# vb000/LookOnceToHear

Hardware: AMD Instinct MI355X
Metric: frames_per_sec (5 s 16 kHz binaural clips, 625 STFT frames each, offline forward) (higher is better)
Workload: dtype f32 via f16x3 split (3x fp16 MFMA per product, fp32 accumulate; ~22-bit operands, un-normalised rows scaled by a power of two before the split: any finite fp32 range); 1 GPU; BASELINE configs[2]: 32 x 5 s 16 kHz binaural clips per GPU, offline forward (configs/tsh.json separator, random-init weights); batch_per_gpu=32, global_batch=32, parallelism=utterance-dp1, gemm_mode=f16x3, tune=, batches_in_flight=1

## Files before the change

### include/lookonce_hip.h

```cpp
#ifndef LOOKONCE_HIP_H
#define LOOKONCE_HIP_H

#ifdef __cplusplus
extern "C" {
#endif

typedef void* lh_stream_t;

enum {
    LH_OK = 0,
    LH_ERR_ARG = 1,
    LH_ERR_UNSUPPORTED = 2,
    LH_ERR_LAUNCH = 3,
    LH_ERR_RANGE = 4
};

int lh_range_status(unsigned* range_flag, lh_stream_t stream);
int lh_range_flag_copy(unsigned* range_flag, void* host_pinned, lh_stream_t stream);
int lh_range_flag_clear(unsigned* range_flag, lh_stream_t stream);
int lh_selftest_fp16_subnormal(lh_stream_t stream);

enum { LH_GEMM_F32 = 0, LH_GEMM_F16X3 = 1 };

int lh_abi_version(void);

int lh_set_tuning(int key, int value);

int lh_check_config(int nfft, int hop, int n_mics, int emb_dim, int n_blocks_unused, int lstm_hidden,
                    int n_heads, int attn_window, int n_srcs, int spk_emb_dim);

int lh_stft_conv_in(const float* x, const float* conv_buf_in, float* conv_buf_out, const void* wfb_pk,
                    const void* wconv_pk, const float* bconv, float* z, int B, int T, int n_samples,
                    lh_stream_t stream);

int lh_embed_proj_ln(const float* emb, const float* w, const float* bias, const float* ln_w, const float* ln_b,
                     float* scratch, float* gain, int B, lh_stream_t stream);

int lh_ln_lstm_intra(const float* x, const float* ln_w, const float* ln_b, const void* w_pk, const float* b_sum,
                     float* h_out, int n_frames , int mode, lh_stream_t stream);

int lh_ln_lstm_inter(const float* x, const float* ln_w, const float* ln_b, const void* w_pk, const float* b_sum,
                     const float* h0, const float* c0, float* hN, float* cN, float* h_out, int B, int T, int mode,
                     lh_stream_t stream);

int lh_intra_stream(const float* x, const void* wih_pk, const float* b_sum, const float* whh, float* h_out,
                    int n_frames, lh_stream_t stream);

int lh_inter_matvec(const float* x, const void* wih_pk, const float* b_sum, const float* whh, const void* wlin_pk,
                    const float* blin, const float* h0, const float* c0, float* hN, float* cN, float* out, int B, int T,
                    lh_stream_t stream);

int lh_intra_block(const float* x, const void* w_pk, const float* b_sum, const void* wlin_pk, const float* blin,
                   float* out, int n_frames, lh_stream_t stream);

int lh_inter_block(const float* x, const void* w_pk, const float* b_sum, const void* wlin_pk, const float* blin,
                   const float* h0, const float* c0, float* hN, float* cN, float* out, int B, int T,
                   lh_stream_t stream);

int lh_linear_res(const float* h, const void* w_pk, const float* bias, const float* res, float* out, int rows,
                  int K, lh_stream_t stream);

#define LH_KV_PAD_ROWS 48

int lh_qkv_proj_ln(const float* y, const void* w_pk, const float* bias, const float* slopes, const float* lnq_w,
                   const float* lnq_b, const float* lnk_w, const float* lnk_b, const float* lnv_w,
                   const float* lnv_b, void* q, void* kx, void* vx, const int* ring_pos, int B, int T,
                   lh_stream_t stream);

int lh_local_attn(const void* q, const void* kx, const void* vx, float* merged, int B, int T, lh_stream_t stream);

int lh_ring_pack(const float* k_buf, const float* v_buf, void* kx, void* vx, int B, int T, lh_stream_t stream);
int lh_ring_unpack(const void* kx, const void* vx, float* k_buf, float* v_buf, int B, int T, lh_stream_t stream);
int lh_ring_advance(int* ring_pos, int modulo, lh_stream_t stream);

int lh_proj_ln_res(const float* merged, const void* w_pk, const float* bias, const float* slope,
                   const float* ln_w, const float* ln_b, const float* y2, const float* gain, float* out, int B,
                   int T, lh_stream_t stream);

int lh_deconv_istft(const float* y, const float* deconv_buf_in, float* deconv_buf_out, const float* istft_buf_in,
                    float* istft_buf_out, const void* wdec_pk, const float* bdec, const void* wfb_dec,
                    float* wave_out, unsigned* range_flag, int keep_nonfinite, int B, int T, lh_stream_t stream);

int lh_intra_block_win(const float* x, const void* w_pk, const float* b_sum, const void* wlin_pk, const float* blin,
                       float* out, int B, int T, int t0, int Tc, lh_stream_t stream);
int lh_inter_block_win(const float* x, const void* w_pk, const float* b_sum, const void* wlin_pk, const float* blin,
                       const float* h0, const float* c0, float* hN, float* cN, float* out, int B, int T, int t0, int Tc,
                       int carry, lh_stream_t stream);
int lh_ln_lstm_intra_win(const float* x, const float* ln_w, const float* ln_b, const void* w_pk, const float* b_sum, float* h_out,
                         int B, int T, int t0, int Tc, lh_stream_t stream);
int lh_linear_res_win(const float* h, const void* w_pk, const float* bias, const float* res, float* out, int B, int T, int t0,
                      int Tc, int K, lh_stream_t stream);
int lh_inter_matvec_win(const float* x, const void* wih_pk, const float* b_sum, const float* whh, const void* wlin_pk,
                        const float* blin, const float* h0, const float* c0, float* hN, float* cN, float* out, int B, int T,
                        int t0, int Tc, int carry, lh_stream_t stream);
int lh_qkv_proj_ln_win(const float* y, const void* w_pk, const float* bias, const float* slopes, const float* lnq_w,
                       const float* lnq_b, const float* lnk_w, const float* lnk_b, const float* lnv_w,
                       const float* lnv_b, void* q, void* kx, void* vx, const int* ring_pos, int B, int T, int t0, int Tc,
                       lh_stream_t stream);
int lh_local_attn_win(const void* q, const void* kx, const void* vx, float* merged, int B, int T, int t0, int Tc,
                      lh_stream_t stream);
int lh_proj_ln_res_win(const float* merged, const void* w_pk, const float* bias, const float* slope, const float* ln_w,
                       const float* ln_b, const float* y2, const float* gain, float* out, int B, int T, int t0, int Tc,
                       lh_stream_t stream);

int lh_ref32_stft_conv_in(const float* x, const float* conv_buf_in, float* conv_buf_out, const float* filters,
                          const float* conv_w, const float* conv_b, float* spec_scratch, float* out, int B, int T,
                          int n_samples, lh_stream_t stream);
int lh_ref32_linear(const float* in, const float* w, const float* bias, const float* slope, const float* res, float* out,
                    int rows, int K, int N, lh_stream_t stream);
int lh_ref32_head_ln(const float* pre, int ncol, int col0, int D, const float* ln_w, const float* ln_b, float* dst,
                     int row0, int rows_per_bh, int B, int T, lh_stream_t stream);
int lh_ref32_local_attn(const float* q, const float* kx, const float* vx, float* merged, int B, int T, lh_stream_t stream);
int lh_ref32_proj_ln_res(const float* merged, const float* w, const float* bias, const float* slope, const float* ln_w,
                         const float* ln_b, const float* y2, const float* gain, float* rows_scratch, float* pre_scratch,
                         float* out, int B, int T, lh_stream_t stream);
int lh_ref32_deconv_istft(const float* y, const float* deconv_buf_in, float* deconv_buf_out, const float* istft_buf_in,
                          float* istft_buf_out, const float* deconv_w, const float* deconv_b, const float* filters,
                          float* sx_scratch, float* wave_out, int B, int T, lh_stream_t stream);

int lh_emb_frontend(const float* x, float* inv_std, const float* wfb_pk, const float* wconv_pk, const float* bconv,
                    const float* gn_w, const float* gn_b, double* gn_part, float* z, void* xsplit_next, int B, int T,
                    int n_samples, lh_stream_t stream);

#ifdef LH_LEGACY
int lh_emb_axis(const float* x, const void* wih_pk, const float* bih, const void* whh_pk, const void* wct_pk,
                const float* bct, void* xsplit, float* gx, float* hbuf, float* out, int B, int T, int inter,
                lh_stream_t stream);
#endif

int lh_emb_axis_fused(const float* x, const void* wrec_pk, const float* brec, const void* wct_pk, const float* bct,
                      void* xsplit, void* hsplit, float* out, int B, int T, int inter, int have_xsplit, int emit_split,
                      lh_stream_t stream);

int lh_emb_axis_mv(const float* x, const void* wih_pk, const float* bih, const float* whh, const void* wct_pk,
                   const float* bct, void* xsplit, void* hsplit, float* out, int B, int T, int have_xsplit, int emit_split,
                   lh_stream_t stream);

int lh_emb_attn_block(const float* y2, const void* wqkv_pk, const float* bqkv, const float* slopes,
                      const float* lnq_w, const float* lnq_b, const float* lnk_w, const float* lnk_b,
                      const float* lnv_w, const float* lnv_b, const void* wproj_pk, const float* bproj,
                      const float* slope_p, const float* lnp_w, const float* lnp_b, void* q, void* k, float* v,
                      void* vt, float* sc, void* p, float* merged, float* out, void* xsplit_next, int B, int T,
                      lh_stream_t stream);

int lh_emb_head(const float* z, const void* w_pk, const float* bias, const float* ln_w, const float* ln_b,
                float* part, float* emb, int B, int T, lh_stream_t stream);

int lh_render_binaural(const float* src, const float* rir, const float* gain, const int* tgt_idx, float* events,
                       unsigned* peak, float* mixture, float* target, int B, int S1, int N, int Lh, lh_stream_t stream);

int lh_metric_sums(const float* outputs, const float* target, const float* mixture, const float* emb,
                   const float* emb_gt, double* scratch, float* rows, double* sums, int B, int n_samples,
                   int emb_dim, lh_stream_t stream);

int lh_binaural_cues(const float* est, const float* gt, double* scratch, double* rows, double* sums, int B, int n_samples,
                     int sr, int frame, double rms_threshold, lh_stream_t stream);

typedef struct { void* base; unsigned long long bytes; } lh_span_t;
enum { LH_SESSION_RESET = 1, LH_SESSION_OPEN = 2, LH_SESSION_CLOSE = 4, LH_SESSION_GEN_SHIFT = 8, LH_SESSION_MAX_SPANS = 32,
       LH_SESSION_MAX_END_SPANS = 8 };
int lh_session_begin(const lh_span_t* spans, int n_spans, const float* chunk_in, float* chunk, const unsigned* cmd,
                     const unsigned* active, int S, lh_stream_t stream);
int lh_session_end(const lh_span_t* spans, int n_spans, const float* chunk_in, float* out, unsigned* cmd, unsigned* active,
                   unsigned* fault, int S, lh_stream_t stream);

int lh_session_move(const lh_span_t* spans, int n_spans, const int* from, unsigned* cmd, unsigned* active, int n_rows, int S,
                    lh_stream_t stream);
int lh_session_begin_rows(const lh_span_t* spans, int n_spans, const float* chunk_in, float* chunk, const unsigned* cmd,
                          const unsigned* active, const int* slot_of, int n_rows, int S, lh_stream_t stream);
int lh_session_end_rows(const lh_span_t* spans, int n_spans, const float* chunk_in, const float* out_rows, float* out,
                        unsigned* cmd, unsigned* active, unsigned* fault, const int* slot_of, const int* row_of, int* from,
                        int n_rows, int S, lh_stream_t stream);

enum { LH_ENROLL_ARM = 1, LH_ENROLL_CANCEL = 2, LH_ENROLL_GEN_SHIFT = 8, LH_ENROLL_FAULT = 0x80000000u };
int lh_session_capture(const float* chunk_in, float* enroll, unsigned* ecmd, unsigned* estate, unsigned* edone, int n_chunks,
                       int S, lh_stream_t stream);

int lh_comm_unique_id(void* id128);
int lh_comm_init(const void* id128, int n_ranks, int rank, void** comm);
int lh_allreduce_f64(void* comm, double* buf, int count, lh_stream_t stream);
int lh_comm_destroy(void* comm);

#ifdef __cplusplus
}
#endif
#endif
```

### lookoncetohear_amd/_cabi.py

```python
from __future__ import annotations

import ctypes
import os
from ctypes import c_double, c_int, c_void_p

_PKG = os.path.dirname(os.path.abspath(__file__))
HIP_LIB_PATH = os.path.join(_PKG, "_lookonce_hip.so")
ABI_VERSION = 18

_P, _I = c_void_p, c_int
SIGNATURES = {
    "lh_abi_version": [],
    "lh_check_config": [_I] * 10,
    "lh_stft_conv_in": [_P] * 7 + [_I] * 3 + [_P],
    "lh_embed_proj_ln": [_P] * 7 + [_I, _P],
    "lh_set_tuning": [_I, _I],
    "lh_ln_lstm_intra": [_P] * 6 + [_I, _I, _P],
    "lh_ln_lstm_inter": [_P] * 10 + [_I, _I, _I, _P],
    "lh_intra_stream": [_P] * 5 + [_I, _P],
    "lh_inter_matvec": [_P] * 11 + [_I, _I, _P],
    "lh_intra_block": [_P] * 6 + [_I, _P],
    "lh_inter_block": [_P] * 10 + [_I, _I, _P],
    "lh_linear_res": [_P] * 5 + [_I, _I, _P],
    "lh_qkv_proj_ln": [_P] * 14 + [_I, _I, _P],
    "lh_local_attn": [_P] * 4 + [_I, _I, _P],
    "lh_ring_pack": [_P] * 4 + [_I, _I, _P],
    "lh_ring_unpack": [_P] * 4 + [_I, _I, _P],
    "lh_ring_advance": [_P, _I, _P],
    "lh_session_begin": [_P, _I, _P, _P, _P, _P, _I, _P],
    "lh_session_end": [_P, _I, _P, _P, _P, _P, _P, _I, _P],
    "lh_session_capture": [_P] * 5 + [_I, _I, _P],
    "lh_session_move": [_P, _I, _P, _P, _P, _I, _I, _P],
    "lh_session_begin_rows": [_P, _I, _P, _P, _P, _P, _P, _I, _I, _P],
    "lh_session_end_rows": [_P, _I] + [_P] * 9 + [_I, _I, _P],
    "lh_proj_ln_res": [_P] * 9 + [_I, _I, _P],
    "lh_deconv_istft": [_P] * 10 + [_I, _I, _I, _P],
    "lh_intra_block_win": [_P] * 6 + [_I, _I, _I, _I, _P],
    "lh_inter_block_win": [_P] * 10 + [_I, _I, _I, _I, _I, _P],
    "lh_ln_lstm_intra_win": [_P] * 6 + [_I, _I, _I, _I, _P],
    "lh_linear_res_win": [_P] * 5 + [_I, _I, _I, _I, _I, _P],
    "lh_inter_matvec_win": [_P] * 11 + [_I, _I, _I, _I, _I, _P],
    "lh_qkv_proj_ln_win": [_P] * 14 + [_I, _I, _I, _I, _P],
    "lh_local_attn_win": [_P] * 4 + [_I, _I, _I, _I, _P],
    "lh_proj_ln_res_win": [_P] * 9 + [_I, _I, _I, _I, _P],
    "lh_emb_frontend": [_P] * 10 + [_I, _I, _I, _P],
    "lh_emb_axis_fused": [_P] * 8 + [_I, _I, _I, _I, _I, _P],
    "lh_emb_axis_mv": [_P] * 9 + [_I, _I, _I, _I, _P],
    "lh_emb_attn_block": [_P] * 24 + [_I, _I, _P],
    "lh_emb_head": [_P] * 7 + [_I, _I, _P],
    "lh_render_binaural": [_P] * 8 + [_I, _I, _I, _I, _P],
    "lh_metric_sums": [_P] * 8 + [_I, _I, _I, _P],
    "lh_binaural_cues": [_P] * 5 + [_I, _I, _I, _I, c_double, _P],
    "lh_range_status": [_P, _P],
    "lh_range_flag_copy": [_P, _P, _P],
    "lh_range_flag_clear": [_P, _P],
    "lh_selftest_fp16_subnormal": [_P],
    "lh_comm_unique_id": [_P],
    "lh_comm_init": [_P, _I, _I, _P],
    "lh_allreduce_f64": [_P, _P, _I, _P],
    "lh_comm_destroy": [_P],
    "lh_ref32_stft_conv_in": [_P] * 8 + [_I, _I, _I, _P],
    "lh_ref32_linear": [_P] * 6 + [_I, _I, _I, _P],
    "lh_ref32_head_ln": [_P, _I, _I, _I, _P, _P, _P, _I, _I, _I, _I, _P],
    "lh_ref32_local_attn": [_P] * 4 + [_I, _I, _P],
    "lh_ref32_proj_ln_res": [_P] * 11 + [_I, _I, _P],
    "lh_ref32_deconv_istft": [_P] * 10 + [_I, _I, _P],
}
LEGACY_SIGNATURES = {
    "lh_emb_axis": [_P] * 10 + [_I, _I, _I, _P],
}
ERRORS = {1: "LH_ERR_ARG", 2: "LH_ERR_UNSUPPORTED", 3: "LH_ERR_LAUNCH", 4: "LH_ERR_RANGE"}


class Lib:

    def __init__(self, path: str):
        if not os.path.exists(path):
            raise RuntimeError(
                f"{path} not found: the HIP extension is not built. Run `python -m lookoncetohear_amd.build` "
                "(hipcc --offload-arch=gfx950). There is no CPU fallback for the product path.")
        self.path = path
        import torch
        self._dll = ctypes.CDLL(path)
        for name, argtypes in SIGNATURES.items():
            fn = getattr(self._dll, name)
            fn.argtypes = argtypes
            fn.restype = c_int
        for name, argtypes in LEGACY_SIGNATURES.items():
            fn = getattr(self._dll, name, None)
            if fn is not None:
                fn.argtypes = argtypes
                fn.restype = c_int
        v = self._dll.lh_abi_version()
        if v != ABI_VERSION:
            raise RuntimeError(f"{path}: ABI version {v}, expected {ABI_VERSION}")

    def call(self, name: str, *args) -> None:
        rc = getattr(self._dll, name)(*args)
        if rc != 0:
            raise RuntimeError(f"{name} failed: {ERRORS.get(rc, rc)}")

    def raw(self, name: str):
        return getattr(self._dll, name)


def device_of(t):
    import torch
    return torch.cuda.device(t.device)


_hip_lib = None
_selftested = set()


class HipHost:
    _host_name = "this module"

    def _lib(self, t) -> "Lib":
        if not t.is_cuda:
            raise RuntimeError(f"lookoncetohear_amd.{self._host_name} runs on an MI355X (ROCm device tensors); there is no "
                               "CPU path. Move the module and its inputs to cuda.")
        lib = load()
        import torch
        selftest_device(lib, t.device.index if t.device.index is not None else torch.cuda.current_device())
        return lib

    def _stream(self, device) -> int:
        import torch
        return torch.cuda.current_stream(device).cuda_stream

    def _device_ctx(self, t):
        return device_of(t)

    def _flag_words(self, device):
        return self._host_words(2, device)

    def _host_words(self, n, device):
        import torch
        return torch.zeros(n, dtype=torch.int32).pin_memory()


def selftest_device(lib: "Lib", device_index: int) -> None:
    if device_index in _selftested:
        return
    import torch
    with torch.cuda.device(device_index):
        rc = lib.raw("lh_selftest_fp16_subnormal")(torch.cuda.current_stream(device_index).cuda_stream)
    if rc != 0:
        raise RuntimeError(f"lh_selftest_fp16_subnormal failed on cuda:{device_index} ({ERRORS.get(rc, rc)}): fp16 subnormal "
                           "MFMA operands are flushed; the split-precision kernels would lose precision silently")
    _selftested.add(device_index)


def load() -> Lib:
    global _hip_lib
    if _hip_lib is None:
        _hip_lib = Lib(os.environ.get("LOOKONCE_HIP_LIB", HIP_LIB_PATH))
        for kv in filter(None, os.environ.get("LOOKONCE_TUNE", "").split(",")):
            k, v = kv.split("=")
            _hip_lib.call("lh_set_tuning", int(k), int(v))
    return _hip_lib
```

### lookoncetohear_amd/csrc/lh_frontend.hip

```cpp
#include "lh_split.h"

namespace lh {

constexpr int FE_NTH = 512;
constexpr int FE_TT = 14;
constexpr int FE_NJ = 16;
constexpr int FE_AP = NFFT + 8;
constexpr int FE_SP = 68;
constexpr int FE_NT = (NK + 15) / 16;
constexpr int FE_KS = NFFT / 32;
constexpr int FE_OP = C + 4;

__global__ void __launch_bounds__(FE_NTH, 1) k_stft_conv_in(const float* __restrict__ x, const float* __restrict__ cbuf_in,
                                                            float* __restrict__ cbuf_out, const _Float16* __restrict__ wfb_pk,
                                                            const _Float16* __restrict__ wc_pk, const float* __restrict__ bc,
                                                            float* __restrict__ z, int B, int T, int n_samples) {
    __shared__ __attribute__((aligned(16))) _Float16 ahi[NMIC * FE_NJ * FE_AP];
    __shared__ __attribute__((aligned(16))) _Float16 alo[NMIC * FE_NJ * FE_AP];
    __shared__ __attribute__((aligned(16))) _Float16 sth[(NF + 2) * FE_SP];
    __shared__ __attribute__((aligned(16))) _Float16 stl[(NF + 2) * FE_SP];
    __shared__ __attribute__((aligned(16))) float outs[2][NF * FE_OP];
    __shared__ float tmax[FE_NTH / 64];
    const int tid = threadIdx.x, lane = tid & 63, wave = wave_id(tid), g4 = lane >> 4, l15 = lane & 15;

    f16x8 wfh[2][FE_KS], wfl[2][FE_KS];
#pragma unroll
    for (int i = 0; i < 2; ++i) load_w<FE_KS>(wfb_pk, min(wave + 8 * i, FE_NT - 1), lane, wfh[i], wfl[i]);
    f16x8 wch[2], wcl[2];
    const int cnt = wave & 3;
    load_w<2>(wc_pk, cnt, lane, wch, wcl);
    const float cbias = bc[cnt * 16 + l15];

    static_assert(((NF + 2) * FE_SP) % 4 == 0, "8-byte zero fill");
    for (int i = tid; i < (NF + 2) * FE_SP / 4; i += FE_NTH) {
        *reinterpret_cast<f16x4*>(&sth[i * 4]) = f16x4{0, 0, 0, 0};
        *reinterpret_cast<f16x4*>(&stl[i * 4]) = f16x4{0, 0, 0, 0};
    }

    const int tiles_per_b = (T + FE_TT - 1) / FE_TT;
    for (int tile = blockIdx.x; tile < B * tiles_per_b; tile += gridDim.x) {
        const int b = tile / tiles_per_b;
        const int t0 = (tile % tiles_per_b) * FE_TT;
        const int nt_out = min(FE_TT, T - t0);
        __syncthreads();
        float tsc, tinv;

        {
            constexpr int NLD = NMIC * FE_NJ * 48 / FE_NTH;
            float4 stg[NLD];
#pragma unroll
            for (int i = 0; i < NLD; ++i) {
                const int e = tid + FE_NTH * i;
                const int m = e / (FE_NJ * 48), j = (e / 48) % FE_NJ, c4 = e % 48;
                const int t = t0 - 2 + j;
                stg[i] = make_float4(0.f, 0.f, 0.f, 0.f);
                if (t >= 0 && t < T)
                    stg[i] = *reinterpret_cast<const float4*>(&x[((long)b * NMIC + m) * n_samples + (long)t * HOP + c4 * 4]);
            }
            float tm = 0.f;
#pragma unroll
            for (int i = 0; i < NLD; ++i) tm = fmaxf(tm, absmax4(stg[i]));
            if (t0 == 0)
                for (int i = tid; i < 4 * 2 * NF; i += FE_NTH) tm = fmaxf(tm, fabsf(cbuf_in[(long)b * 4 * 2 * NF + i]) * (1.0f / 32.0f));
            tm = wave_max(tm);
            if (lane == 0) tmax[wave] = tm;
            __syncthreads();
#pragma unroll
            for (int w = 0; w < FE_NTH / 64; ++w) tm = fmaxf(tm, tmax[w]);
            pow2_scale<9>(tm, tsc, tinv);
#pragma unroll
            for (int i = 0; i < NLD; ++i) {
                const int e = tid + FE_NTH * i;
                const int m = e / (FE_NJ * 48), j = (e / 48) % FE_NJ, c4 = e % 48;
                const float v[4] = {stg[i].x * tsc, stg[i].y * tsc, stg[i].z * tsc, stg[i].w * tsc};
                f16x2_t h01, l01, h23, l23;
                split_pair(v[0], v[1], h01, l01);
                split_pair(v[2], v[3], h23, l23);
                const f16x4 h4 = f16x4{h01[0], h01[1], h23[0], h23[1]}, l4 = f16x4{l01[0], l01[1], l23[0], l23[1]};
                const int idx = (m * FE_NJ + j) * FE_AP + c4 * 4;
                *reinterpret_cast<f16x4*>(&ahi[idx]) = h4;
                *reinterpret_cast<f16x4*>(&alo[idx]) = l4;
            }
        }
        __syncthreads();

#pragma unroll 1
        for (int m = 0; m < NMIC; ++m) {
            f32x4 am[2], ac[2];
#pragma unroll
            for (int i = 0; i < 2; ++i) { am[i] = f32x4{0.f, 0.f, 0.f, 0.f}; ac[i] = f32x4{0.f, 0.f, 0.f, 0.f}; }
            const bool second = wave + 8 < FE_NT;
#pragma unroll
            for (int ks = 0; ks < FE_KS; ++ks) {
                const int idx = (m * FE_NJ + l15) * FE_AP + ks * 32 + g4 * 8;
                const f16x8 fah = *reinterpret_cast<const f16x8*>(&ahi[idx]);
                const f16x8 fal = *reinterpret_cast<const f16x8*>(&alo[idx]);
#pragma unroll
                for (int i = 0; i < 2; ++i) {
                    if (i == 0 || second) {
                        am[i] = __builtin_amdgcn_mfma_f32_16x16x32_f16(fah, wfh[i][ks], am[i], 0, 0, 0);
                        ac[i] = __builtin_amdgcn_mfma_f32_16x16x32_f16(fah, wfl[i][ks], ac[i], 0, 0, 0);
                        ac[i] = __builtin_amdgcn_mfma_f32_16x16x32_f16(fal, wfh[i][ks], ac[i], 0, 0, 0);
                    }
                }
            }
#pragma unroll
            for (int i = 0; i < 2; ++i) {
                const int nt = wave + 8 * i;
                const int k = nt * 16 + l15;
                if (nt < FE_NT && k < NK) {
                    const int ch = (k / NF) * NMIC + m, f = k % NF;
#pragma unroll
                    for (int r = 0; r < 4; ++r) {
                        const int j = g4 * 4 + r, t = t0 - 2 + j;
                        float v = am[i][r] + ac[i][r];
                        if (t < 0) v = cbuf_in[(((long)b * 4 + ch) * 2 + (t + 2)) * NF + f] * tsc;
                        if (t >= T) v = 0.0f;
                        _Float16 h, l;
                        split_hl(v, h, l);
                        sth[(f + 1) * FE_SP + j * 4 + ch] = h;
                        stl[(f + 1) * FE_SP + j * 4 + ch] = l;
                        if (t >= T - 2 && t < T) cbuf_out[(((long)b * 4 + ch) * 2 + (t - (T - 2))) * NF + f] = v * tinv;
                    }
                }
            }
        }
        __syncthreads();

        const int mt0 = wave >> 2;
        const int kf0 = g4 >> 1, cofs = (g4 & 1) * 8;
        for (int jt = 0; jt < nt_out; ++jt) {
            float* ob = outs[jt & 1];
#pragma unroll
            for (int i = 0; i < 4; ++i) {
                const int mt = mt0 + 2 * i;
                if (mt < 7) {
                    const int f = min(mt * 16 + l15, NF - 1);
                    const int a0 = (f + kf0) * FE_SP + jt * 4 + cofs, a1 = (f + 2) * FE_SP + jt * 4 + cofs;
                    f16x8 ah[2], al[2];
                    auto rd8 = [&](const _Float16* base, int idx) -> f16x8 {
                        const f16x4 u = *reinterpret_cast<const f16x4*>(&base[idx]);
                        const f16x4 w = *reinterpret_cast<const f16x4*>(&base[idx + 4]);
                        return f16x8{u[0], u[1], u[2], u[3], w[0], w[1], w[2], w[3]};
                    };
                    ah[0] = rd8(sth, a0); al[0] = rd8(stl, a0);
                    ah[1] = rd8(sth, a1); al[1] = rd8(stl, a1);
                    f32x4 am = f32x4{0.f, 0.f, 0.f, 0.f}, ac = f32x4{0.f, 0.f, 0.f, 0.f};
#pragma unroll
                    for (int ks = 0; ks < 2; ++ks) {
                        am = __builtin_amdgcn_mfma_f32_16x16x32_f16(ah[ks], wch[ks], am, 0, 0, 0);
                        ac = __builtin_amdgcn_mfma_f32_16x16x32_f16(ah[ks], wcl[ks], ac, 0, 0, 0);
                        ac = __builtin_amdgcn_mfma_f32_16x16x32_f16(al[ks], wch[ks], ac, 0, 0, 0);
                    }
#pragma unroll
                    for (int r = 0; r < 4; ++r) {
                        const int fo = mt * 16 + g4 * 4 + r;
                        if (fo < NF) ob[fo * FE_OP + cnt * 16 + l15] = fmaf(am[r] + ac[r], tinv, cbias);
                    }
                }
            }
            __syncthreads();
            float* dst = z + (((long)b * T + t0 + jt) * NF) * C;
            for (int e = tid; e < NF * 16; e += FE_NTH)
                *reinterpret_cast<float4*>(&dst[e * 4]) = *reinterpret_cast<const float4*>(&ob[(e >> 4) * FE_OP + (e & 15) * 4]);
        }
    }
}

constexpr int EP_ROWS = 32, EP_NB = 8;
__global__ void __launch_bounds__(256) k_embed_proj(const float* __restrict__ emb, const float* __restrict__ w,
                                                     const float* __restrict__ bias, float* __restrict__ raw, int B) {
    constexpr int N = C * NF;
    __shared__ __attribute__((aligned(16))) float es[EP_NB][SPK];
    const int tid = threadIdx.x, lane = tid & 63, wave = wave_id(tid);
    const int b0 = blockIdx.y * EP_NB;
    for (int i = tid; i < EP_NB * SPK; i += 256) {
        const int bb = min(b0 + i / SPK, B - 1);
        es[i / SPK][i % SPK] = emb[(long)bb * SPK + (i % SPK)];
    }
    __syncthreads();
    constexpr int RW = EP_ROWS / 4;
    float4 w4[RW];
    float bz[RW];
#pragma unroll
    for (int q = 0; q < RW; ++q) {
        const int r = min((int)blockIdx.x * EP_ROWS + wave + q * 4, N - 1);
        w4[q] = *reinterpret_cast<const float4*>(&w[(long)r * SPK + lane * 4]);
        bz[q] = bias[r];
    }
#pragma unroll
    for (int q = 0; q < RW; ++q) {
        const int r = blockIdx.x * EP_ROWS + wave + q * 4;
        if (r >= N) break;
#pragma unroll
        for (int j = 0; j < EP_NB; ++j) {
            const float4 e4 = *reinterpret_cast<const float4*>(&es[j][lane * 4]);
            float s = wave_sum(w4[q].x * e4.x + w4[q].y * e4.y + w4[q].z * e4.z + w4[q].w * e4.w);
            if (lane == 0 && b0 + j < B) raw[(long)(b0 + j) * N + r] = s + bz[q];
        }
    }
}

__global__ void __launch_bounds__(256) k_embed_ln(const float* __restrict__ raw, const float* __restrict__ lnw,
                                                   const float* __restrict__ lnb, float* __restrict__ gain) {
    constexpr int N = C * NF;
    __shared__ float vals[N];
    __shared__ float red[4];
    const int tid = threadIdx.x;
    const int b = blockIdx.x;
    float s = 0.0f;
    for (int i = tid; i < N; i += 256) { const float v = raw[(long)b * N + i]; vals[i] = v; s += v; }
    const float mean = block_sum_256(s, red) * (1.0f / N);
    float v = 0.0f;
    for (int i = tid; i < N; i += 256) { float d = vals[i] - mean; v += d * d; }
    const float rstd = rsqrtf(block_sum_256(v, red) * (1.0f / N) + LN_EPS);
    for (int oidx = tid; oidx < N; oidx += 256) {
        const int f = oidx / C, c = oidx % C;
        const int i = c * NF + f;
        gain[(long)b * N + oidx] = (vals[i] - mean) * rstd * lnw[i] + lnb[i];
    }
}

}

extern "C" int lh_stft_conv_in(const float* x, const float* conv_buf_in, float* conv_buf_out, const void* wfb_pk,
                               const void* wconv_pk, const float* bconv, float* z, int B, int T, int n_samples,
                               lh_stream_t stream) {
    using namespace lh;
    if (!x || !conv_buf_in || !conv_buf_out || !wfb_pk || !wconv_pk || !bconv || !z || B <= 0 || T <= 0) return LH_ERR_ARG;
    if (conv_buf_in == conv_buf_out || n_samples != T * HOP + (NFFT - HOP)) return LH_ERR_ARG;
    const int tiles = B * ((T + FE_TT - 1) / FE_TT);
    hipLaunchKernelGGL(k_stft_conv_in, dim3(tiles < 256 ? tiles : 256), dim3(FE_NTH), 0, (hipStream_t)stream, x,
                       conv_buf_in, conv_buf_out, (const _Float16*)wfb_pk, (const _Float16*)wconv_pk, bconv, z, B, T,
                       n_samples);
    return check_launch();
}

extern "C" int lh_embed_proj_ln(const float* emb, const float* w, const float* bias, const float* ln_w,
                                const float* ln_b, float* scratch, float* gain, int B, lh_stream_t stream) {
    using namespace lh;
    if (!emb || !w || !bias || !ln_w || !ln_b || !scratch || !gain || B <= 0 || scratch == gain) return LH_ERR_ARG;
    hipLaunchKernelGGL(k_embed_proj, dim3((C * NF + EP_ROWS - 1) / EP_ROWS, (B + EP_NB - 1) / EP_NB), dim3(256), 0,
                       (hipStream_t)stream, emb, w, bias, scratch, B);
    hipLaunchKernelGGL(k_embed_ln, dim3(B), dim3(256), 0, (hipStream_t)stream, scratch, ln_w, ln_b, gain);
    return check_launch();
}

extern "C" int lh_abi_version(void) { return 18; }

extern "C" int lh_check_config(int nfft, int hop, int n_mics, int emb_dim, int n_blocks_unused, int lstm_hidden,
                               int n_heads, int attn_window, int n_srcs, int spk_emb_dim) {
    using namespace lh;
    (void)n_blocks_unused;
    if (nfft != NFFT || hop != HOP || n_mics != NMIC || emb_dim != C || lstm_hidden != H || n_heads != NH ||
        attn_window != WIN || n_srcs != NSRC || spk_emb_dim != SPK)
        return LH_ERR_UNSUPPORTED;
    return LH_OK;
}
```

### lookoncetohear_amd/csrc/lh_lstm.hip

```cpp
#include <type_traits>

#include "lh_common.h"

namespace lh {

constexpr int LS_PAD = 36;

template <int MT>
__global__ void __launch_bounds__(256) k_ln_lstm(const float* __restrict__ x, const float* __restrict__ lnw,
                                                 const float* __restrict__ lnb, const float* __restrict__ w_pk,
                                                 const float* __restrict__ b_sum, const float* __restrict__ h0,
                                                 const float* __restrict__ c0, float* __restrict__ hN,
                                                 float* __restrict__ cN, float* __restrict__ h_out, int nseq,
                                                 int nstep, int sdiv, int so, int si, int ps, int ldh) {
    constexpr int NS = 16 * MT;
    __shared__ __attribute__((aligned(16))) float abuf[2 * 4 * NS * LS_PAD];
    const int tid = threadIdx.x, lane = tid & 63, wave = wave_id(tid);
    const int dir = blockIdx.y;
    const int s0 = blockIdx.x * NS;
    const int g4 = lane >> 4, l15 = lane & 15;

    auto A = [&](int buf, int chunk, int row, int j) -> float* {
        return &abuf[((buf * 4 + chunk) * NS + row) * LS_PAD + j];
    };
// ... 598 lines not shown
    if (nstep >= 2) store_rows(nstep - 2, (nstep - 1) & 1, rr);
    load_base(nstep - 1, rr);
    lin_tile(nstep & 1, nstep & 1);
    __syncthreads();
    store_rows(nstep - 1, nstep & 1, rr);
}

#endif

__global__ void __launch_bounds__(512, 1) k_lstm_lin8p(const float* __restrict__ x, const _Float16* __restrict__ w_pk,
                                                       const float* __restrict__ b_sum, const _Float16* __restrict__ wlin_pk,
                                                       const float* __restrict__ blin, const float* __restrict__ h0,
                                                       const float* __restrict__ c0, float* __restrict__ hN,
                                                       float* __restrict__ cN, float* out, int nseq, int nstep, int sdiv,
                                                       int so, int si, int ps, int dir, int accumulate) {
    constexpr int NS = 16;
    constexpr int LSP = C + 4;
    __shared__ __attribute__((aligned(16))) _Float16 ahi[2 * NS * LH_AP];
    __shared__ __attribute__((aligned(16))) _Float16 alo[2 * NS * LH_AP];
    __shared__ __attribute__((aligned(16))) float ls[2 * NS * LSP];
    __shared__ __attribute__((aligned(16))) float hf[NS * LSP];
    const int tid = threadIdx.x, lane = tid & 63;
    const int wave = __builtin_amdgcn_readfirstlane(tid >> 6);
    const int s0 = blockIdx.x * NS;
    const int g4 = lane >> 4, l15 = lane & 15;
    const bool lin_wave = wave < 4;
    const int q = tid & 15, rrow = (tid & 255) >> 4;
    const int unit0 = 8 * wave + 2 * g4;

    auto row_of0 = [&](int s) -> long { return (long)(s / sdiv) * so + (long)(s % sdiv) * si; };
    const long wg_row0 = row_of0(min(s0, nseq - 1));
    const unsigned voff = (unsigned)((row_of0(min(s0 + rrow, nseq - 1)) - wg_row0) * (C * 4) + q * 16);
    const char* xb = reinterpret_cast<const char*>(x) + wg_row0 * (C * 4);
    char* ob = reinterpret_cast<char*>(out) + wg_row0 * (C * 4);
    const char* bsrc = reinterpret_cast<const char*>(
        accumulate ? reinterpret_cast<unsigned long long>(ob) : reinterpret_cast<unsigned long long>(xb));
    const long step_bytes = (long)ps * (C * 4);
    auto step_pos = [&](int it) -> int { it = min(max(it, 0), nstep - 1); return dir ? (nstep - 1 - it) : it; };

    f16x8 wh[2][4], wl[2][4];
    {
        const _Float16* wp = w_pk + ((long)(dir * 8 + wave) * 8 * 64 + lane) * 16;
#pragma unroll
        for (int m = 0; m < 2; ++m)
#pragma unroll
            for (int ks = 0; ks < 4; ++ks) {
                wh[m][ks] = *reinterpret_cast<const f16x8*>(wp + (long)(m * 4 + ks) * 64 * 16);
                wl[m][ks] = *reinterpret_cast<const f16x8*>(wp + (long)(m * 4 + ks) * 64 * 16 + 8);
            }
    }
    f16x8 lwh[2], lwl[2];
    float lbias = 0.0f;
    if (lin_wave) {
#pragma unroll
        for (int ks = 0; ks < 2; ++ks) {
            lwh[ks] = *reinterpret_cast<const f16x8*>(&wlin_pk[((wave * 2 + ks) * 64 + lane) * 16]);
            lwl[ks] = *reinterpret_cast<const f16x8*>(&wlin_pk[((wave * 2 + ks) * 64 + lane) * 16 + 8]);
        }
        if (!accumulate) lbias = blin[wave * 16 + l15];
    } else {
#pragma unroll
        for (int ks = 0; ks < 2; ++ks) lwh[ks] = lwl[ks] = f16x8{0, 0, 0, 0, 0, 0, 0, 0};
    }
    float bias[2][4];
#pragma unroll
    for (int m = 0; m < 2; ++m)
#pragma unroll
        for (int g = 0; g < 4; ++g) bias[m][g] = b_sum[dir * 256 + g * 64 + unit0 + m];

    const int a_frag = l15 * LH_AP + g4 * 8;
    const int a_cell = l15 * LH_AP + C + unit0;
    const int a_row = rrow * LH_AP + q * 4;
    const int l_row = rrow * LSP + q * 4;
    const int l_lin = (g4 * 4) * LSP + wave * 16 + l15;

    auto store_split4 = [&](int idx, float a, float b, float c, float d) {
        f16x4 h4, l4;
        _Float16 th, tl;
        split_f16(a, th, tl); h4[0] = th; l4[0] = tl;
        split_f16(b, th, tl); h4[1] = th; l4[1] = tl;
        split_f16(c, th, tl); h4[2] = th; l4[2] = tl;
        split_f16(d, th, tl); h4[3] = th; l4[3] = tl;
        *reinterpret_cast<f16x4*>(&ahi[idx]) = h4;
        *reinterpret_cast<f16x4*>(&alo[idx]) = l4;
    };
    auto norm_store_x = [&](int buf, float4 v) {
        const float mean = group16_sum(v.x + v.y + v.z + v.w) * (1.0f / C);
        v.x -= mean; v.y -= mean; v.z -= mean; v.w -= mean;
        const float var = group16_sum(v.x * v.x + v.y * v.y + v.z * v.z + v.w * v.w) * (1.0f / C);
        const float rstd = __builtin_amdgcn_rsqf(var + LN_EPS);
        store_split4(buf * NS * LH_AP + a_row, v.x * rstd, v.y * rstd, v.z * rstd, v.w * rstd);
    };
    auto load_row = [&](const char* base, int it) -> float4 {
        return *reinterpret_cast<const float4*>(base + step_pos(it) * step_bytes + voff);
    };
    auto x_half = [&](int buf, f32x4 (&g)[2]) {
#pragma unroll
        for (int m = 0; m < 2; ++m) g[m] = f32x4{bias[m][0], bias[m][1], bias[m][2], bias[m][3]};
#pragma unroll
        for (int ks = 0; ks < 2; ++ks) {
            const f16x8 xh = *reinterpret_cast<const f16x8*>(&ahi[buf * NS * LH_AP + a_frag + ks * 32]);
            const f16x8 xl = *reinterpret_cast<const f16x8*>(&alo[buf * NS * LH_AP + a_frag + ks * 32]);
#pragma unroll
            for (int m = 0; m < 2; ++m) g[m] = __builtin_amdgcn_mfma_f32_16x16x32_f16(wh[m][ks], xh, g[m], 0, 0, 0);
#pragma unroll
            for (int m = 0; m < 2; ++m) g[m] = __builtin_amdgcn_mfma_f32_16x16x32_f16(wh[m][ks], xl, g[m], 0, 0, 0);
#pragma unroll
            for (int m = 0; m < 2; ++m) g[m] = __builtin_amdgcn_mfma_f32_16x16x32_f16(wl[m][ks], xh, g[m], 0, 0, 0);
        }
    };

    float creg[2], hreg[2];
    float4 carry = make_float4(0.f, 0.f, 0.f, 0.f);
    if (!lin_wave) {
        norm_store_x(0, load_row(xb, 0));
        norm_store_x(1, load_row(xb, 1));
        carry = load_row(xb, 2);
    } else {
        const int s = min(s0 + rrow, nseq - 1);
        float4 hv = make_float4(0.f, 0.f, 0.f, 0.f);
        if (h0) hv = *reinterpret_cast<const float4*>(&h0[(long)s * H + q * 4]);
        store_split4(a_row + C, hv.x, hv.y, hv.z, hv.w);
    }
    {
        const int s = min(s0 + l15, nseq - 1);
#pragma unroll
        for (int m = 0; m < 2; ++m) {
            creg[m] = c0 ? c0[(long)s * H + unit0 + m] : 0.0f;
            hreg[m] = 0.0f;
        }
    }
    __syncthreads();
    f32x4 gx[2];
    x_half(0, gx);
    __syncthreads();

    auto step = [&](int it, auto cur_tag, auto lin_tag) __attribute__((always_inline)) {
        constexpr int cur = decltype(cur_tag)::value, nxt = cur ^ 1;
        constexpr bool LIN = decltype(lin_tag)::value;
        f16x8 bh[2], bl[2];
#pragma unroll
        for (int ks = 0; ks < 2; ++ks) {
            bh[ks] = *reinterpret_cast<const f16x8*>(&ahi[cur * NS * LH_AP + a_frag + (2 + ks) * 32]);
            bl[ks] = *reinterpret_cast<const f16x8*>(&alo[cur * NS * LH_AP + a_frag + (2 + ks) * 32]);
        }
        f32x4 acc[2] = {gx[0], gx[1]};
#pragma unroll
        for (int ks = 0; ks < 2; ++ks) {
#pragma unroll
            for (int m = 0; m < 2; ++m) acc[m] = __builtin_amdgcn_mfma_f32_16x16x32_f16(wh[m][2 + ks], bh[ks], acc[m], 0, 0, 0);
#pragma unroll
            for (int m = 0; m < 2; ++m) acc[m] = __builtin_amdgcn_mfma_f32_16x16x32_f16(wh[m][2 + ks], bl[ks], acc[m], 0, 0, 0);
#pragma unroll
            for (int m = 0; m < 2; ++m) acc[m] = __builtin_amdgcn_mfma_f32_16x16x32_f16(wl[m][2 + ks], bh[ks], acc[m], 0, 0, 0);
        }
        pin_here(carry);
        if (LIN) {
            const float4 pv = *reinterpret_cast<const float4*>(&ls[nxt * NS * LSP + l_row]);
            const float4 done = make_float4(carry.x + pv.x, carry.y + pv.y, carry.z + pv.z, carry.w + pv.w);
            if (it >= 2) *reinterpret_cast<float4*>(ob + step_pos(it - 2) * step_bytes + voff) = done;
            carry = load_row(bsrc, it - 1);
        } else {
            norm_store_x(cur, carry);
            carry = load_row(xb, it + 3);
        }
        __builtin_amdgcn_sched_barrier(0);
        auto cells = [&]() {
#pragma unroll
            for (int m = 0; m < 2; ++m) {
                lstm_cell_pre(acc[m][0], acc[m][1], acc[m][2], acc[m][3], creg[m], hreg[m]);
                _Float16 th, tl;
                split_f16(hreg[m], th, tl);
                ahi[nxt * NS * LH_AP + a_cell + m] = th;
                alo[nxt * NS * LH_AP + a_cell + m] = tl;
            }
        };
        if (LIN) {
            x_half(nxt, gx);
            f32x4 am = f32x4{lbias, lbias, lbias, lbias};
#pragma unroll
            for (int ks = 0; ks < 2; ++ks) {
                am = __builtin_amdgcn_mfma_f32_16x16x32_f16(bh[ks], lwh[ks], am, 0, 0, 0);
                am = __builtin_amdgcn_mfma_f32_16x16x32_f16(bh[ks], lwl[ks], am, 0, 0, 0);
                am = __builtin_amdgcn_mfma_f32_16x16x32_f16(bl[ks], lwh[ks], am, 0, 0, 0);
            }
            __builtin_amdgcn_sched_barrier(0);
            cells();
#pragma unroll
            for (int r = 0; r < 4; ++r) ls[cur * NS * LSP + r * LSP + l_lin] = am[r];
        } else {
            __builtin_amdgcn_sched_barrier(0);
            cells();
            __builtin_amdgcn_sched_barrier(0);
            x_half(nxt, gx);
        }
        __builtin_amdgcn_sched_barrier(0);
        __syncthreads();
    };
    auto run = [&](auto lin_tag) __attribute__((always_inline)) {
        int it = 0;
        for (; it + 1 < nstep; it += 2) {
            step(it, std::integral_constant<int, 0>{}, lin_tag);
            step(it + 1, std::integral_constant<int, 1>{}, lin_tag);
        }
        if (it < nstep) step(it, std::integral_constant<int, 0>{}, lin_tag);
    };
    if (lin_wave) run(std::true_type{});
    else run(std::false_type{});

    const int lastb = nstep & 1;
    if (lin_wave) {
        if (nstep >= 2) {
            const float4 pv = *reinterpret_cast<const float4*>(&ls[(lastb ^ 1) * NS * LSP + l_row]);
            *reinterpret_cast<float4*>(ob + step_pos(nstep - 2) * step_bytes + voff) =
                make_float4(carry.x + pv.x, carry.y + pv.y, carry.z + pv.z, carry.w + pv.w);
        }
        carry = load_row(bsrc, nstep - 1);
        f32x4 am = f32x4{lbias, lbias, lbias, lbias};
#pragma unroll
        for (int ks = 0; ks < 2; ++ks) {
            const f16x8 ah = *reinterpret_cast<const f16x8*>(&ahi[lastb * NS * LH_AP + a_frag + (2 + ks) * 32]);
            const f16x8 al = *reinterpret_cast<const f16x8*>(&alo[lastb * NS * LH_AP + a_frag + (2 + ks) * 32]);
            am = __builtin_amdgcn_mfma_f32_16x16x32_f16(ah, lwh[ks], am, 0, 0, 0);
            am = __builtin_amdgcn_mfma_f32_16x16x32_f16(ah, lwl[ks], am, 0, 0, 0);
            am = __builtin_amdgcn_mfma_f32_16x16x32_f16(al, lwh[ks], am, 0, 0, 0);
        }
#pragma unroll
        for (int r = 0; r < 4; ++r) ls[lastb * NS * LSP + r * LSP + l_lin] = am[r];
    }
    if (hN) {
#pragma unroll
        for (int m = 0; m < 2; ++m) hf[l15 * LSP + unit0 + m] = hreg[m];
    }
    __syncthreads();
    if (lin_wave) {
        const float4 pv = *reinterpret_cast<const float4*>(&ls[lastb * NS * LSP + l_row]);
        *reinterpret_cast<float4*>(ob + step_pos(nstep - 1) * step_bytes + voff) =
            make_float4(carry.x + pv.x, carry.y + pv.y, carry.z + pv.z, carry.w + pv.w);
    } else if (hN && s0 + rrow < nseq) {
        *reinterpret_cast<float4*>(&hN[(long)(s0 + rrow) * H + q * 4]) = *reinterpret_cast<const float4*>(&hf[l_row]);
    }
    if (cN && s0 + l15 < nseq) {
#pragma unroll
        for (int m = 0; m < 2; ++m) cN[(long)(s0 + l15) * H + unit0 + m] = creg[m];
    }
}

#if defined(LH_LEGACY)
static int g_dephase = 1;
template <int MT>
static int launch_lstm_lin(const float* x, const void* w_pk, const float* b_sum, const void* wlin_pk, const float* blin,
                           const float* h0, const float* c0, float* hN, float* cN, float* out, int nseq, int nstep,
                           int sdiv, int so, int si, int ps, int dir, int accumulate, hipStream_t st) {
    constexpr int NS = 16 * MT;
    if (h0 || c0 || hN || cN) return LH_ERR_ARG;
    hipLaunchKernelGGL((k_ln_lstm_lin<MT>), dim3((nseq + NS - 1) / NS), dim3(256), 0, st, x, (const _Float16*)w_pk, b_sum,
                       (const _Float16*)wlin_pk, blin, h0, c0, hN, cN, out, nseq, nstep, sdiv, so, si, ps, dir, accumulate,
                       g_dephase);
    return check_launch();
}

#endif
template <int MT>
static int launch_lstm_h3(const float* x, const float* lnw, const float* lnb, const void* w_pk, const float* b_sum,
                          const float* h0, const float* c0, float* hN, float* cN, float* h_out, int nseq, int nstep,
                          int ndir, int sdiv, int so, int si, int ps, int ldh, hipStream_t st) {
    constexpr int NS = 16 * MT;
    hipLaunchKernelGGL((k_ln_lstm_h3<MT>), dim3((nseq + NS - 1) / NS, ndir), dim3(256), 0, st, x, lnw, lnb,
                       (const _Float16*)w_pk, b_sum, h0, c0, hN, cN, h_out, nseq, nstep, sdiv, so, si, ps, ldh);
    return check_launch();
}

template <int MT>
static int launch_lstm(const float* x, const float* lnw, const float* lnb, const float* w_pk, const float* b_sum,
                       const float* h0, const float* c0, float* hN, float* cN, float* h_out, int nseq, int nstep,
                       int ndir, int sdiv, int so, int si, int ps, int ldh, hipStream_t st) {
    constexpr int NS = 16 * MT;
    hipLaunchKernelGGL((k_ln_lstm<MT>), dim3((nseq + NS - 1) / NS, ndir), dim3(256), 0, st, x, lnw, lnb, w_pk, b_sum,
                       h0, c0, hN, cN, h_out, nseq, nstep, sdiv, so, si, ps, ldh);
    return check_launch();
}

}

namespace lh {
static int cu_count() {
    static int n = 0;
    if (n == 0) {
        int dev = 0, v = 0;
        if (hipGetDevice(&dev) == hipSuccess &&
            hipDeviceGetAttribute(&v, hipDeviceAttributeMultiprocessorCount, dev) == hipSuccess && v > 0)
            n = v;
        else
            n = 256;
    }
    return n;
}
int emb_set(int key, int value);
static int g_tune[8] = {0, 0, 0, 0, 0, 0, 0, 0};
}
namespace lh { int attn_set_mq(int v); }
namespace lh {
int launch_intra_xp(const float* x, const void* w_pk, const float* b_sum, const void* wlin_pk, const float* blin, float* out,
                    int nseq, int nstep, int sdiv, int so, int si, int ps, int dir, int accumulate, hipStream_t st);
int xp_set(int key, int v);
int launch_inter_xp(const float* x, const void* w_pk, const float* b_sum, const void* wlin_pk, const float* blin,
                    const float* h0, const float* c0, float* hN, float* cN, float* out, int nseq, int nstep, int sdiv, int so,
                    int si, int ps, hipStream_t st, int cflags = 0);
}
namespace lh { int backend_set_runs(int v); }
#if defined(LH_PROBE_TRACE)
extern "C" int lh_probe_trace_read(unsigned long long* host_dst) {
    return hipMemcpyFromSymbol(host_dst, HIP_SYMBOL(lh::lh_trace_buf), sizeof(lh::lh_trace_buf)) == hipSuccess ? 0 : 1;
}
#endif
extern "C" int lh_set_tuning(int key, int value) {
    if (key == 4) return lh::attn_set_mq(value);
    if (key == 6) return lh::backend_set_runs(value);
    if (key >= 7 && key < 16) return lh::xp_set(key, value);
    if (key == 16 || key == 17) return lh::emb_set(key, value);
    if (key < 0 || key >= 8) return LH_ERR_ARG;
#if defined(LH_LEGACY)
    if (key == 3) lh::g_dephase = value;
#else
    if (key == 2 && value == 2) return LH_ERR_UNSUPPORTED;
#endif
    lh::g_tune[key] = value;
    return LH_OK;
}

extern "C" int lh_ln_lstm_intra(const float* x, const float* ln_w, const float* ln_b, const void* w_pk,
                                const float* b_sum, float* h_out, int n_frames, int mode, lh_stream_t stream) {
    using namespace lh;
    if (!x || !ln_w || !ln_b || !w_pk || !b_sum || !h_out || n_frames <= 0) return LH_ERR_ARG;
    const int mt = g_tune[0] ? g_tune[0] : (mode == LH_GEMM_F16X3 ? 0 : (n_frames >= 8192 ? 2 : 1));
    if (mode == LH_GEMM_F16X3) {
        hipStream_t st = (hipStream_t)stream;
        if (mt == 2)
            return launch_lstm_h3<2>(x, ln_w, ln_b, w_pk, b_sum, nullptr, nullptr, nullptr, nullptr, h_out, n_frames, NF,
                                     2, 1, NF, 0, 1, 2 * H, st);
        if (mt == 1)
            return launch_lstm_h3<1>(x, ln_w, ln_b, w_pk, b_sum, nullptr, nullptr, nullptr, nullptr, h_out, n_frames, NF,
                                     2, 1, NF, 0, 1, 2 * H, st);
        const int slots = 2 * cu_count();
        const int tiles2 = (n_frames / 32) * 2 / slots * slots / 2;
        const int f2 = tiles2 * 32;
        int rc = LH_OK;
        if (f2 > 0)
            rc = launch_lstm_h3<2>(x, ln_w, ln_b, w_pk, b_sum, nullptr, nullptr, nullptr, nullptr, h_out, f2, NF, 2, 1, NF,
                                   0, 1, 2 * H, st);
        if (rc == LH_OK && n_frames > f2)
            rc = launch_lstm_h3<1>(x + (long)f2 * NF * C, ln_w, ln_b, w_pk, b_sum, nullptr, nullptr, nullptr, nullptr,
                                   h_out + (long)f2 * NF * 2 * H, n_frames - f2, NF, 2, 1, NF, 0, 1, 2 * H, st);
        return rc;
    }
    if (mode != LH_GEMM_F32) return LH_ERR_UNSUPPORTED;
    const float* w_f32 = (const float*)w_pk;
    if (mt == 2)
        return launch_lstm<2>(x, ln_w, ln_b, w_f32, b_sum, nullptr, nullptr, nullptr, nullptr, h_out, n_frames, NF, 2, 1,
                              NF, 0, 1, 2 * H, (hipStream_t)stream);
    return launch_lstm<1>(x, ln_w, ln_b, w_f32, b_sum, nullptr, nullptr, nullptr, nullptr, h_out, n_frames, NF, 2, 1, NF,
                          0, 1, 2 * H, (hipStream_t)stream);
}

extern "C" int lh_ln_lstm_intra_win(const float* x, const float* ln_w, const float* ln_b, const void* w_pk, const float* b_sum,
                                    float* h_out, int B, int T, int t0, int Tc, lh_stream_t stream) {
    using namespace lh;
    if (!x || !ln_w || !ln_b || !w_pk || !b_sum || !h_out || B <= 0 || T <= 0 || t0 < 0 || Tc <= 0 || t0 + Tc > T) return LH_ERR_ARG;
    const long off = (long)t0 * NF;
    return launch_lstm_h3<1>(x + off * C, ln_w, ln_b, w_pk, b_sum, nullptr, nullptr, nullptr, nullptr, h_out + off * 2 * H, B * Tc,
                             NF, 2, Tc, T * NF, NF, 1, 2 * H, (hipStream_t)stream);
}

extern "C" int lh_ln_lstm_inter(const float* x, const float* ln_w, const float* ln_b, const void* w_pk,
                                const float* b_sum, const float* h0, const float* c0, float* hN, float* cN,
                                float* h_out, int B, int T, int mode, lh_stream_t stream) {
    using namespace lh;
    if (!x || !ln_w || !ln_b || !w_pk || !b_sum || !h0 || !c0 || !hN || !cN || !h_out || B <= 0 || T <= 0)
        return LH_ERR_ARG;
    if (h0 == hN || c0 == cN) return LH_ERR_ARG;
    const int nseq = B * NF;
    const int mt = g_tune[1] == 2 ? 2 : 1;
    if (mode == LH_GEMM_F16X3) {
        if (mt == 2)
            return launch_lstm_h3<2>(x, ln_w, ln_b, w_pk, b_sum, h0, c0, hN, cN, h_out, nseq, T, 1, NF, T * NF, 1, NF, H,
                                     (hipStream_t)stream);
        return launch_lstm_h3<1>(x, ln_w, ln_b, w_pk, b_sum, h0, c0, hN, cN, h_out, nseq, T, 1, NF, T * NF, 1, NF, H,
                                 (hipStream_t)stream);
    }
    if (mode != LH_GEMM_F32) return LH_ERR_UNSUPPORTED;
    const float* w_f32 = (const float*)w_pk;
    if (mt == 2)
        return launch_lstm<2>(x, ln_w, ln_b, w_f32, b_sum, h0, c0, hN, cN, h_out, nseq, T, 1, NF, T * NF, 1, NF, H,
                              (hipStream_t)stream);
    return launch_lstm<1>(x, ln_w, ln_b, w_f32, b_sum, h0, c0, hN, cN, h_out, nseq, T, 1, NF, T * NF, 1, NF, H,
                          (hipStream_t)stream);
}

extern "C" int lh_intra_block(const float* x, const void* w_pk, const float* b_sum, const void* wlin_pk,
                              const float* blin, float* out, int n_frames, lh_stream_t stream) {
    using namespace lh;
    if (!x || !w_pk || !b_sum || !wlin_pk || !blin || !out || n_frames <= 0 || x == out) return LH_ERR_ARG;
    hipStream_t st = (hipStream_t)stream;
    int rc = LH_OK;
    for (int dir = 0; dir < 2 && rc == LH_OK; ++dir)
#if defined(LH_LEGACY)
        if (g_tune[2] == 2)
            rc = launch_lstm_lin<1>(x, w_pk, b_sum, (const _Float16*)wlin_pk + (long)dir * 4 * 2 * 64 * 16, blin, nullptr, nullptr,
                                    nullptr, nullptr, out, n_frames, NF, 1, NF, 0, 1, dir, dir, st);
        else
#endif
            rc = launch_intra_xp(x, w_pk, b_sum, (const _Float16*)wlin_pk + (long)dir * 4 * 2 * 64 * 16, blin, out, n_frames,
                                 NF, 1, NF, 0, 1, dir, dir, st);
    return rc;
}

extern "C" int lh_intra_block_win(const float* x, const void* w_pk, const float* b_sum, const void* wlin_pk,
                                  const float* blin, float* out, int B, int T, int t0, int Tc, lh_stream_t stream) {
    using namespace lh;
    if (!x || !w_pk || !b_sum || !wlin_pk || !blin || !out || B <= 0 || T <= 0 || x == out || t0 < 0 || Tc <= 0 || t0 + Tc > T)
        return LH_ERR_ARG;
    const long off = (long)t0 * NF * C;
    int rc = LH_OK;
    for (int dir = 0; dir < 2 && rc == LH_OK; ++dir)
        rc = launch_intra_xp(x + off, w_pk, b_sum, (const _Float16*)wlin_pk + (long)dir * 4 * 2 * 64 * 16, blin, out + off,
                             B * Tc, NF, Tc, T * NF, NF, 1, dir, dir, (hipStream_t)stream);
    return rc;
}

extern "C" int lh_inter_block_win(const float* x, const void* w_pk, const float* b_sum, const void* wlin_pk,
                                  const float* blin, const float* h0, const float* c0, float* hN, float* cN, float* out,
                                  int B, int T, int t0, int Tc, int carry, lh_stream_t stream) {
    using namespace lh;
    if (!x || !w_pk || !b_sum || !wlin_pk || !blin || !h0 || !c0 || !hN || !cN || !out || B <= 0 || T <= 0) return LH_ERR_ARG;
    if (h0 == hN || c0 == cN || x == out || t0 < 0 || Tc < 2 || t0 + Tc > T || (carry & ~3)) return LH_ERR_ARG;
    const long off = (long)t0 * NF * C;
    return launch_inter_xp(x + off, w_pk, b_sum, wlin_pk, blin, h0, c0, hN, cN, out + off, B * NF, Tc, NF, T * NF, 1, NF,
                           (hipStream_t)stream, carry);
}

extern "C" int lh_inter_block(const float* x, const void* w_pk, const float* b_sum, const void* wlin_pk,
                              const float* blin, const float* h0, const float* c0, float* hN, float* cN, float* out,
                              int B, int T, lh_stream_t stream) {
    using namespace lh;
    if (!x || !w_pk || !b_sum || !wlin_pk || !blin || !h0 || !c0 || !hN || !cN || !out || B <= 0 || T <= 0) return LH_ERR_ARG;
    if (h0 == hN || c0 == cN || x == out) return LH_ERR_ARG;
    const int nseq = B * NF;
    if (g_tune[5] != 2 && T >= 2)
        return launch_inter_xp(x, w_pk, b_sum, wlin_pk, blin, h0, c0, hN, cN, out, nseq, T, NF, T * NF, 1, NF,
                               (hipStream_t)stream);
    hipLaunchKernelGGL(k_lstm_lin8p, dim3((nseq + 15) / 16), dim3(512), 0, (hipStream_t)stream, x, (const _Float16*)w_pk,
                           b_sum, (const _Float16*)wlin_pk, blin, h0, c0, hN, cN, out, nseq, T, NF, T * NF, 1, NF, 0, 0);
    return check_launch();
}
```

### lookoncetohear_amd/csrc/lh_recur.hip

```cpp
#include <tuple>
#include <type_traits>
#include <utility>

#include "lh_common.h"

namespace lh {

typedef _Float16 xp_f16x8 __attribute__((ext_vector_type(8)));
typedef _Float16 xp_f16x4 __attribute__((ext_vector_type(4)));
constexpr int XP_AP = 144;
constexpr int XP_LSP = 68;
constexpr float XP_K2 = -2.0f * LOG2E;

template <int NSLOT, class MF, class Ops>
__device__ __forceinline__ void xp_zip(MF& mf, Ops& ops) {
    constexpr int NOPS = (int)std::tuple_size<Ops>::value;
    xp_for<NSLOT>([&](auto s_) {
        constexpr int i = decltype(s_)::value;
        mf(s_);
        constexpr int a = i * NOPS / NSLOT, b = (i + 1) * NOPS / NSLOT;
        xp_for<b - a>([&](auto k_) { std::get<a + decltype(k_)::value>(ops)(); });
#if !defined(XP_NO_FENCE)
        __builtin_amdgcn_sched_barrier(0);
#endif
    });
}

#if defined(XP_X2)
constexpr int XP_XN = 8;
#else
constexpr int XP_XN = 12;
#endif

#if defined(XP_PF1)
constexpr int XP_PF = 1;
#else
constexpr int XP_PF = 2;
#endif

#if defined(XP_TRACE)
__device__ unsigned long long xp_trace_buf[2 * 128 * 4];
__device__ unsigned long long xp_wg_log[4096 * 4];
__device__ unsigned long long xp_trace_inter[2 * 128 * 4];
#define XP_STAMP(k) do { if (tr_on) tr[(it & 127) * 4 + (k)] = __builtin_amdgcn_s_memtime(); } while (0)
#else
#define XP_STAMP(k) do { } while (0)
#endif

__device__ __forceinline__ float xp_exp2(float v) {
#if defined(XP_PROBE_NOTRANS)
    return __builtin_fmaf(v, 0.25f, 0.5f);
#else
    return __builtin_amdgcn_exp2f(v);
#endif
}
__device__ __forceinline__ float xp_rcp(float v) {
#if defined(XP_PROBE_NOTRANS)
    return __builtin_fmaf(v, -0.25f, 1.0f);
#else
    return __builtin_amdgcn_rcpf(v);
#endif
}
#if defined(XP_PROBE_HIHI)
constexpr int XP_NP = 1;
#else
constexpr int XP_NP = 3;
#endif

__global__ void __launch_bounds__(256, 2) k_intra_xp(const float* __restrict__ x, const _Float16* __restrict__ w_pk,
                                                     const float* __restrict__ b_sum, const _Float16* __restrict__ wlin_pk,
                                                     const float* __restrict__ blin, float* out, int nseq, int nstep,
                                                     int sdiv, int so, int si, int ps, int dir, int accumulate, int prio) {
    constexpr int NS = 16;
    __shared__ __attribute__((aligned(16))) _Float16 ahi[2 * NS * XP_AP];
    __shared__ __attribute__((aligned(16))) _Float16 alo[2 * NS * XP_AP];
    __shared__ __attribute__((aligned(16))) float ls[2 * NS * XP_LSP];
    const int tid = threadIdx.x, lane = tid & 63, wave = wave_id(tid);
#if defined(XP_TRACE)
    __shared__ unsigned long long tr[128 * 4];
    const int tr_slot = blockIdx.x == 7 ? 0 : (blockIdx.x == gridDim.x / 2 + 3 ? 1 : -1);
    const bool tr_on = tr_slot >= 0 && threadIdx.x == 0 && dir == 0;
    const unsigned long long wg_t0 = __builtin_amdgcn_s_memtime();
#endif
    if (prio == 1) {
        const unsigned hw_id = __builtin_amdgcn_s_getreg((4 - 1) << 11 | 0 << 6 | 4);
        if (hw_id & 1) __builtin_amdgcn_s_setprio(2);
    }
#if defined(LH_PROBE_INTRA1)
    const int nt1 = (nseq + NS - 1) / NS;
    dir = (int)blockIdx.x >= nt1;
    accumulate = dir;
    wlin_pk += (long)dir * 4 * 2 * 64 * 16;
    const int s0 = ((int)blockIdx.x - dir * nt1) * NS;
#else
    const int s0 = blockIdx.x * NS;
#endif
    const int g4 = lane >> 4, l15 = lane & 15;
    const int q = tid & 15;
    const int unit = wave * 16 + l15;

    auto row_of0 = [&](int s) -> long { return (long)(s / sdiv) * so + (long)(s % sdiv) * si; };
    const long wg_row0 = row_of0(min(s0, nseq - 1));
    const int srow = min(s0 + (tid >> 4), nseq - 1);
    const unsigned voff = (unsigned)((row_of0(srow) - wg_row0) * (C * 4) + q * 16);
    const char* xb = reinterpret_cast<const char*>(x) + wg_row0 * (C * 4);
    char* ob = reinterpret_cast<char*>(out) + wg_row0 * (C * 4);
    const char* bsrc = reinterpret_cast<const char*>(
        accumulate ? reinterpret_cast<unsigned long long>(ob) : reinterpret_cast<unsigned long long>(xb));
    const long step_bytes = (long)ps * (C * 4);
    auto step_pos = [&](int it) -> int { it = min(max(it, 0), nstep - 1); return dir ? (nstep - 1 - it) : it; };

    xp_f16x8 wh[4][4], wl[4][4];
    {
        const _Float16* wp = w_pk + ((long)(dir * 4 + wave) * 16 * 64 + lane) * 16;
#pragma unroll
        for (int g = 0; g < 4; ++g)
#pragma unroll
            for (int ks = 0; ks < 4; ++ks) {
                wh[g][ks] = *reinterpret_cast<const xp_f16x8*>(wp + (long)(g * 4 + ks) * 64 * 16);
                wl[g][ks] = *reinterpret_cast<const xp_f16x8*>(wp + (long)(g * 4 + ks) * 64 * 16 + 8);
            }
    }
    xp_f16x8 lwh[2], lwl[2];
#pragma unroll
    for (int ks = 0; ks < 2; ++ks) {
        lwh[ks] = *reinterpret_cast<const xp_f16x8*>(&wlin_pk[((wave * 2 + ks) * 64 + lane) * 16]);
        lwl[ks] = *reinterpret_cast<const xp_f16x8*>(&wlin_pk[((wave * 2 + ks) * 64 + lane) * 16 + 8]);
    }
    float eb[4];
#pragma unroll
    for (int g = 0; g < 4; ++g)
        eb[g] = __builtin_amdgcn_exp2f(fminf(fmaxf(b_sum[dir * 256 + g * 64 + unit], -100.0f), 100.0f));
    const float lbias = accumulate ? 0.0f : blin[unit];

    const int a_row = (tid >> 4) * XP_AP + q * 4;
    const int l_row = (tid >> 4) * XP_LSP + q * 4;
    const int a_frag = l15 * XP_AP + g4 * 8;
    const int a_cell = (g4 * 4) * XP_AP + C + unit;
    const int l_cell = (g4 * 4) * XP_LSP + unit;

    auto load_x = [&](int it) -> float4 { return *reinterpret_cast<const float4*>(xb + step_pos(it) * step_bytes + voff); };
    auto load_base = [&](int it) -> float4 { return *reinterpret_cast<const float4*>(bsrc + step_pos(it) * step_bytes + voff); };
    auto store_split4 = [&](int idx, float a, float b, float c, float d) {
        f16x2_t h01, l01, h23, l23;
        split_pair(a, b, h01, l01);
        split_pair(c, d, h23, l23);
        const xp_f16x4 h4 = xp_f16x4{h01[0], h01[1], h23[0], h23[1]}, l4 = xp_f16x4{l01[0], l01[1], l23[0], l23[1]};
        *reinterpret_cast<xp_f16x4*>(&ahi[idx]) = h4;
        *reinterpret_cast<xp_f16x4*>(&alo[idx]) = l4;
    };
    auto norm_store_x = [&](int buf, float4 v) {
        const float mean = group16_sum(v.x + v.y + v.z + v.w) * (1.0f / C);
        v.x -= mean; v.y -= mean; v.z -= mean; v.w -= mean;
        const float var = group16_sum(v.x * v.x + v.y * v.y + v.z * v.z + v.w * v.w) * (1.0f / C);
        const float rstd = __builtin_amdgcn_rsqf(var + LN_EPS);
        store_split4(buf * NS * XP_AP + a_row, v.x * rstd, v.y * rstd, v.z * rstd, v.w * rstd);
    };
    auto x_half = [&](int buf, f32x4 (&g)[4]) __attribute__((always_inline)) {
        xp_f16x8 xh[2], xl[2];
#pragma unroll
        for (int ks = 0; ks < 2; ++ks) {
            xh[ks] = *reinterpret_cast<const xp_f16x8*>(&ahi[buf * NS * XP_AP + a_frag + ks * 32]);
            xl[ks] = *reinterpret_cast<const xp_f16x8*>(&alo[buf * NS * XP_AP + a_frag + ks * 32]);
        }
#pragma unroll
        for (int gg = 0; gg < 4; ++gg) g[gg] = f32x4{0.f, 0.f, 0.f, 0.f};
#pragma unroll
        for (int ks = 0; ks < 2; ++ks) {
#pragma unroll
            for (int gg = 0; gg < 4; ++gg) g[gg] = __builtin_amdgcn_mfma_f32_16x16x32_f16(xh[ks], wh[gg][ks], g[gg], 0, 0, 0);
#pragma unroll
            for (int gg = 0; gg < 4; ++gg) g[gg] = __builtin_amdgcn_mfma_f32_16x16x32_f16(xh[ks], wl[gg][ks], g[gg], 0, 0, 0);
#pragma unroll
            for (int gg = 0; gg < 4; ++gg) g[gg] = __builtin_amdgcn_mfma_f32_16x16x32_f16(xl[ks], wh[gg][ks], g[gg], 0, 0, 0);
        }
    };

    float creg[4] = {0.f, 0.f, 0.f, 0.f};
    float4 xr, rr = make_float4(0.f, 0.f, 0.f, 0.f);
    norm_store_x(0, load_x(0));
    norm_store_x(1, load_x(1));
    xr = load_x(2);
    store_split4(a_row + C, 0.f, 0.f, 0.f, 0.f);
    __syncthreads();
    f32x4 gx[4];
    x_half(0, gx);
    __syncthreads();

    auto step = [&](int it, auto cur_tag, auto store_tag) __attribute__((always_inline)) {
        constexpr int cur = decltype(cur_tag)::value, nxt = cur ^ 1;
        constexpr bool STORE = decltype(store_tag)::value;
        if (prio == 2) __builtin_amdgcn_s_setprio(3);
        if (prio == 3) __builtin_amdgcn_s_setprio(0);
        XP_STAMP(0);
        xp_f16x8 hh[2], hl[2];
#pragma unroll
        for (int ks = 0; ks < 2; ++ks) {
            hh[ks] = *reinterpret_cast<const xp_f16x8*>(&ahi[cur * NS * XP_AP + a_frag + (2 + ks) * 32]);
            hl[ks] = *reinterpret_cast<const xp_f16x8*>(&alo[cur * NS * XP_AP + a_frag + (2 + ks) * 32]);
        }
        f32x4 acc[4] = {gx[0], gx[1], gx[2], gx[3]};
        auto h_mfma = [&](auto idx) __attribute__((always_inline)) {
            constexpr int i = decltype(idx)::value, ks = i / 12, p = (i % 12) / 4, g = i % 4;
            if constexpr (p < XP_NP)
            acc[g] = __builtin_amdgcn_mfma_f32_16x16x32_f16(p == 2 ? hl[ks] : hh[ks], p == 1 ? wl[g][2 + ks] : wh[g][2 + ks],
                                                            acc[g], 0, 0, 0);
        };
        float4 v, pv, done, y;
        float s, t, qa, qb, rstd;
        xp_f16x4 h4, l4;
        auto h_ops = std::make_tuple(
            [&] { v = xr; s = v.x + v.y; t = v.z + v.w; },
            [&] { s += t; pv = *reinterpret_cast<const float4*>(&ls[nxt * NS * XP_LSP + l_row]); },
            [&] { s = row_ror_add<8>(s); },
            [&] { s = row_ror_add<4>(s); },
            [&] { s = row_ror_add<2>(s); },
            [&] { s = row_ror_add<1>(s); },
            [&] { v.x = __builtin_fmaf(s, -1.0f / C, v.x); v.y = __builtin_fmaf(s, -1.0f / C, v.y); },
            [&] { v.z = __builtin_fmaf(s, -1.0f / C, v.z); v.w = __builtin_fmaf(s, -1.0f / C, v.w); },
            [&] { qa = v.x * v.x; qb = v.z * v.z; },
            [&] { qa = __builtin_fmaf(v.y, v.y, qa); qb = __builtin_fmaf(v.w, v.w, qb); },
            [&] { qa += qb; done.x = rr.x + pv.x; },
            [&] { qa = row_ror_add<8>(qa); done.y = rr.y + pv.y; },
            [&] { qa = row_ror_add<4>(qa); done.z = rr.z + pv.z; },
            [&] { qa = row_ror_add<2>(qa); done.w = rr.w + pv.w; },
            [&] { qa = row_ror_add<1>(qa); },
            [&] {
                rstd = __builtin_amdgcn_rsqf(__builtin_fmaf(qa, 1.0f / C, LN_EPS));
#if defined(XP_PROBE_NOGLOBAL)
                if (STORE && done.x == 1.2345e30f) *reinterpret_cast<float4*>(ob + step_pos(it - 2) * step_bytes + voff) = done;
#else
                if (STORE) *reinterpret_cast<float4*>(ob + step_pos(it - 2) * step_bytes + voff) = done;
#endif
            },
#if defined(XP_PROBE_NOGLOBAL)
            [&] { if (!STORE) rr = load_base(it - 1); },
#else
            [&] { rr = load_base(it - 1); },
#endif
            [&] { y.x = v.x * rstd; y.y = v.y * rstd; },
            [&] { y.z = v.z * rstd; y.w = v.w * rstd; },
            [&] { f16x2_t a_, b_; split_pair(y.x, y.y, a_, b_); h4[0] = a_[0]; h4[1] = a_[1]; l4[0] = b_[0]; l4[1] = b_[1]; },
            [&] { },
            [&] { f16x2_t a_, b_; split_pair(y.z, y.w, a_, b_); h4[2] = a_[0]; h4[3] = a_[1]; l4[2] = b_[0]; l4[3] = b_[1]; },
            [&] {
                *reinterpret_cast<xp_f16x4*>(&ahi[cur * NS * XP_AP + a_row]) = h4;
                *reinterpret_cast<xp_f16x4*>(&alo[cur * NS * XP_AP + a_row]) = l4;
            },
#if defined(XP_PROBE_NOGLOBAL)
            [&] { if (!STORE) xr = load_x(it + 3); });
#else
            [&] { xr = load_x(it + 3); });
#endif
        xp_zip<24>(h_mfma, h_ops);
        XP_STAMP(1);
        if (prio == 2) __builtin_amdgcn_s_setprio(0);
        if (prio == 3) __builtin_amdgcn_s_setprio(3);
        xp_f16x8 xh[2], xl[2];
        f32x4 am = f32x4{lbias, lbias, lbias, lbias};
        auto c_mfma = [&](auto idx) __attribute__((always_inline)) {
            constexpr int i = decltype(idx)::value;
            if constexpr (i < 6) {
                constexpr int ks = i / 3, p = i % 3;
                if constexpr (p < XP_NP)
                am = __builtin_amdgcn_mfma_f32_16x16x32_f16(p == 2 ? hl[ks] : hh[ks], p == 1 ? lwl[ks] : lwh[ks], am, 0, 0, 0);
            } else {
                constexpr int j = i - 6, ks = j / XP_XN, p = (j % XP_XN) / 4, g = j % 4;
                const f32x4 c0 = j < 4 ? f32x4{0.f, 0.f, 0.f, 0.f} : gx[g];
                if constexpr (p < XP_NP)
                gx[g] = __builtin_amdgcn_mfma_f32_16x16x32_f16(p == 2 ? xl[ks] : xh[ks], p == 1 ? wl[g][ks] : wh[g][ks], c0, 0, 0, 0);
            }
        };
        float tc[4];
        auto cA = [&](auto r_) { constexpr int r = decltype(r_)::value; acc[0][r] = xp_exp2(acc[0][r]); acc[1][r] = xp_exp2(acc[1][r]); };
        auto cB = [&](auto r_) { constexpr int r = decltype(r_)::value; acc[2][r] = xp_exp2(acc[2][r]); acc[3][r] = xp_exp2(acc[3][r]); };
        auto cC = [&](auto r_) {
            constexpr int r = decltype(r_)::value;
#pragma unroll
            for (int g = 0; g < 4; ++g) acc[g][r] = __builtin_fmaf(acc[g][r], eb[g], 1.0f);
        };
        auto cD = [&](auto r_) { constexpr int r = decltype(r_)::value; acc[0][r] = xp_rcp(acc[0][r]); acc[1][r] = xp_rcp(acc[1][r]); };
        auto cE = [&](auto r_) { constexpr int r = decltype(r_)::value; acc[2][r] = xp_rcp(acc[2][r]); acc[3][r] = xp_rcp(acc[3][r]); };
        auto cF = [&](auto r_) {
            constexpr int r = decltype(r_)::value;
            const float g2 = __builtin_fmaf(2.0f * XP_K2, acc[2][r], -XP_K2);
            creg[r] = __builtin_fmaf(acc[1][r], creg[r], acc[0][r] * g2);
        };
        auto cG = [&](auto r_) { constexpr int r = decltype(r_)::value; tc[r] = 1.0f + xp_exp2(creg[r]); };
        auto cH = [&](auto r_) { constexpr int r = decltype(r_)::value; tc[r] = xp_rcp(tc[r]); };
        auto cI = [&](auto r_) {
            constexpr int r = decltype(r_)::value;
            const float hv = acc[3][r] * __builtin_fmaf(2.0f, tc[r], -1.0f);
            _Float16 th, tl;
            split_hl(hv, th, tl);
            ahi[(nxt * NS + r) * XP_AP + a_cell] = th;
            alo[(nxt * NS + r) * XP_AP + a_cell] = tl;
        };
        using R0 = std::integral_constant<int, 0>;
        using R1 = std::integral_constant<int, 1>;
        using R2 = std::integral_constant<int, 2>;
        using R3 = std::integral_constant<int, 3>;
        auto c_ops = std::make_tuple(
            [&] {
                xh[0] = *reinterpret_cast<const xp_f16x8*>(&ahi[nxt * NS * XP_AP + a_frag]);
                xl[0] = *reinterpret_cast<const xp_f16x8*>(&alo[nxt * NS * XP_AP + a_frag]);
            },
            [&] {
                xh[1] = *reinterpret_cast<const xp_f16x8*>(&ahi[nxt * NS * XP_AP + a_frag + 32]);
                xl[1] = *reinterpret_cast<const xp_f16x8*>(&alo[nxt * NS * XP_AP + a_frag + 32]);
            },
            [&] { cA(R0{}); }, [&] { cA(R1{}); }, [&] { cB(R0{}); }, [&] { cB(R1{}); }, [&] { cC(R0{}); }, [&] { cC(R1{}); },
            [&] { cD(R0{}); }, [&] { cD(R1{}); },
            [&] {
#pragma unroll
                for (int r = 0; r < 4; ++r) ls[(cur * NS + r) * XP_LSP + l_cell] = am[r];
            },
            [&] { cE(R0{}); }, [&] { cE(R1{}); }, [&] { cF(R0{}); }, [&] { cF(R1{}); }, [&] { cG(R0{}); }, [&] { cG(R1{}); },
            [&] { cH(R0{}); }, [&] { cH(R1{}); }, [&] { cI(R0{}); }, [&] { cI(R1{}); },
            [&] { cA(R2{}); }, [&] { cA(R3{}); }, [&] { cB(R2{}); }, [&] { cB(R3{}); }, [&] { cC(R2{}); }, [&] { cC(R3{}); },
            [&] { cD(R2{}); }, [&] { cD(R3{}); }, [&] { cE(R2{}); }, [&] { cE(R3{}); }, [&] { cF(R2{}); }, [&] { cF(R3{}); },
            [&] { cG(R2{}); }, [&] { cG(R3{}); }, [&] { cH(R2{}); }, [&] { cH(R3{}); }, [&] { cI(R2{}); }, [&] { cI(R3{}); });
        xp_zip<6 + 2 * XP_XN>(c_mfma, c_ops);
        XP_STAMP(2);
        __syncthreads();
        __builtin_amdgcn_sched_barrier(0);
    };
    {
        using B0 = std::integral_constant<int, 0>;
        using B1 = std::integral_constant<int, 1>;
        step(0, B0{}, std::false_type{});
        if (nstep > 1) step(1, B1{}, std::false_type{});
        int it = 2;
        for (; it + 1 < nstep; it += 2) {
            step(it, B0{}, std::true_type{});
            step(it + 1, B1{}, std::true_type{});
        }
        if (it < nstep) step(it, B0{}, std::true_type{});
    }

#if defined(XP_TRACE)
    if (tr_slot >= 0 && dir == 0 && threadIdx.x < 64)
        for (int i = threadIdx.x; i < 128 * 4; i += 64) xp_trace_buf[tr_slot * 512 + i] = tr[i];
    if (threadIdx.x == 0 && dir == 0 && blockIdx.x < 4096) {
        xp_wg_log[blockIdx.x * 4 + 0] = wg_t0;
        xp_wg_log[blockIdx.x * 4 + 1] = __builtin_amdgcn_s_memtime();
        xp_wg_log[blockIdx.x * 4 + 2] = __builtin_amdgcn_s_getreg((32 - 1) << 11 | 0 << 6 | 4);
        xp_wg_log[blockIdx.x * 4 + 3] = __builtin_amdgcn_s_getreg((32 - 1) << 11 | 0 << 6 | 20);
    }
#endif
    const int lastb = nstep & 1;
    if (nstep >= 2) {
        const float4 pv = *reinterpret_cast<const float4*>(&ls[(lastb ^ 1) * NS * XP_LSP + l_row]);
        *reinterpret_cast<float4*>(ob + step_pos(nstep - 2) * step_bytes + voff) =
            make_float4(rr.x + pv.x, rr.y + pv.y, rr.z + pv.z, rr.w + pv.w);
    }
    rr = load_base(nstep - 1);
    {
        f32x4 am = f32x4{lbias, lbias, lbias, lbias};
#pragma unroll
        for (int ks = 0; ks < 2; ++ks) {
            const xp_f16x8 ah = *reinterpret_cast<const xp_f16x8*>(&ahi[lastb * NS * XP_AP + a_frag + (2 + ks) * 32]);
            const xp_f16x8 al = *reinterpret_cast<const xp_f16x8*>(&alo[lastb * NS * XP_AP + a_frag + (2 + ks) * 32]);
            am = __builtin_amdgcn_mfma_f32_16x16x32_f16(ah, lwh[ks], am, 0, 0, 0);
            am = __builtin_amdgcn_mfma_f32_16x16x32_f16(ah, lwl[ks], am, 0, 0, 0);
            am = __builtin_amdgcn_mfma_f32_16x16x32_f16(al, lwh[ks], am, 0, 0, 0);
        }
#pragma unroll
        for (int r = 0; r < 4; ++r) ls[(lastb * NS + r) * XP_LSP + l_cell] = am[r];
    }
    __syncthreads();
    {
        const float4 pv = *reinterpret_cast<const float4*>(&ls[lastb * NS * XP_LSP + l_row]);
        *reinterpret_cast<float4*>(ob + step_pos(nstep - 1) * step_bytes + voff) =
            make_float4(rr.x + pv.x, rr.y + pv.y, rr.z + pv.z, rr.w + pv.w);
    }
}

template <bool LIN>
struct xp_tag { static constexpr bool value = LIN; };

__global__ void __launch_bounds__(512, 1) k_inter_xp(const float* __restrict__ x, const _Float16* __restrict__ w_pk,
                                                     const float* __restrict__ b_sum, const _Float16* __restrict__ wlin_pk,
                                                     const float* __restrict__ blin, const float* __restrict__ h0,
                                                     const float* __restrict__ c0, float* __restrict__ hN,
                                                     float* __restrict__ cN, float* out, int nseq, int nstep, int sdiv,
                                                     int so, int si, int ps, int dir, int accumulate, int prio, int cflags) {
    constexpr int NS = 16;
    __shared__ __attribute__((aligned(16))) _Float16 ahi[2 * NS * XP_AP];
    __shared__ __attribute__((aligned(16))) _Float16 alo[2 * NS * XP_AP];
    __shared__ __attribute__((aligned(16))) float ls[2 * NS * XP_LSP];
    __shared__ __attribute__((aligned(16))) float hf[NS * XP_LSP];
    const int tid = threadIdx.x, lane = tid & 63;
    const int wave = __builtin_amdgcn_readfirstlane(tid >> 6);
    const bool role_swap = (prio & 16) != 0;
    prio &= 15;
    const bool lin_wave = (wave < 4) != role_swap;
    const int rw = wave & 3;
    if ((prio == 1 && !lin_wave) || (prio == 2 && lin_wave)) __builtin_amdgcn_s_setprio(3);
#if defined(XP_TRACE)
    __shared__ unsigned long long tr_all[2 * 128 * 4];
    const bool tr_on = blockIdx.x == 3 && (threadIdx.x & 255) == 0;
    unsigned long long* const tr = tr_all + (threadIdx.x >> 8) * 512;
#endif
    const int s0 = blockIdx.x * NS;
    const int g4 = lane >> 4, l15 = lane & 15;
    const int q = tid & 15, rrow = (tid & 255) >> 4;
    const int unit0 = 8 * wave + 2 * g4;

    auto row_of0 = [&](int s) -> long { return (long)(s / sdiv) * so + (long)(s % sdiv) * si; };
    const long wg_row0 = row_of0(min(s0, nseq - 1));
    const unsigned voff = (unsigned)((row_of0(min(s0 + rrow, nseq - 1)) - wg_row0) * (C * 4) + q * 16);
    const char* xb = reinterpret_cast<const char*>(x) + wg_row0 * (C * 4);
    char* ob = reinterpret_cast<char*>(out) + wg_row0 * (C * 4);
    const char* bsrc = reinterpret_cast<const char*>(
        accumulate ? reinterpret_cast<unsigned long long>(ob) : reinterpret_cast<unsigned long long>(xb));
    const long step_bytes = (long)ps * (C * 4);
    auto step_pos = [&](int it) -> int { it = min(max(it, 0), nstep - 1); return dir ? (nstep - 1 - it) : it; };

    xp_f16x8 wh[2][4], wl[2][4];
    {
        const _Float16* wp = w_pk + ((long)(dir * 8 + wave) * 8 * 64 + lane) * 16;
#pragma unroll
        for (int m = 0; m < 2; ++m)
#pragma unroll
            for (int ks = 0; ks < 4; ++ks) {
                wh[m][ks] = *reinterpret_cast<const xp_f16x8*>(wp + (long)(m * 4 + ks) * 64 * 16);
                wl[m][ks] = *reinterpret_cast<const xp_f16x8*>(wp + (long)(m * 4 + ks) * 64 * 16 + 8);
            }
    }
    xp_f16x8 lwh[2], lwl[2];
    float lbias = 0.0f;
    if (lin_wave) {
#pragma unroll
        for (int ks = 0; ks < 2; ++ks) {
            lwh[ks] = *reinterpret_cast<const xp_f16x8*>(&wlin_pk[((rw * 2 + ks) * 64 + lane) * 16]);
            lwl[ks] = *reinterpret_cast<const xp_f16x8*>(&wlin_pk[((rw * 2 + ks) * 64 + lane) * 16 + 8]);
        }
        if (!accumulate) lbias = blin[rw * 16 + l15];
    } else {
#pragma unroll
        for (int ks = 0; ks < 2; ++ks) lwh[ks] = lwl[ks] = xp_f16x8{0, 0, 0, 0, 0, 0, 0, 0};
    }
    float eb[2][4];
#pragma unroll
    for (int m = 0; m < 2; ++m)
#pragma unroll
        for (int g = 0; g < 4; ++g)
            eb[m][g] = __builtin_amdgcn_exp2f(fminf(fmaxf(b_sum[dir * 256 + g * 64 + unit0 + m], -100.0f), 100.0f));

    const int a_frag = l15 * XP_AP + g4 * 8;
    const int a_cell = l15 * XP_AP + C + unit0;
    const int a_row = rrow * XP_AP + q * 4;
    const int l_row = rrow * XP_LSP + q * 4;
    const int l_lin = (g4 * 4) * XP_LSP + rw * 16 + l15;

    auto store_split4 = [&](int idx, float a, float b, float c, float d) {
        f16x2_t h01, l01, h23, l23;
        split_pair(a, b, h01, l01);
        split_pair(c, d, h23, l23);
        const xp_f16x4 h4 = xp_f16x4{h01[0], h01[1], h23[0], h23[1]}, l4 = xp_f16x4{l01[0], l01[1], l23[0], l23[1]};
        *reinterpret_cast<xp_f16x4*>(&ahi[idx]) = h4;
        *reinterpret_cast<xp_f16x4*>(&alo[idx]) = l4;
    };
    auto norm_store_x = [&](int buf, float4 v) {
        float s = v.x + v.y, t = v.z + v.w;
        s += t;
        s = group16_sum(s);
        v.x = __builtin_fmaf(s, -1.0f / C, v.x); v.y = __builtin_fmaf(s, -1.0f / C, v.y);
        v.z = __builtin_fmaf(s, -1.0f / C, v.z); v.w = __builtin_fmaf(s, -1.0f / C, v.w);
        float qa = v.x * v.x, qb = v.z * v.z;
        qa = __builtin_fmaf(v.y, v.y, qa); qb = __builtin_fmaf(v.w, v.w, qb);
        qa += qb;
        qa = group16_sum(qa);
        const float rstd = __builtin_amdgcn_rsqf(__builtin_fmaf(qa, 1.0f / C, LN_EPS));
        store_split4(buf * NS * XP_AP + a_row, v.x * rstd, v.y * rstd, v.z * rstd, v.w * rstd);
    };
    auto load_row = [&](const char* base, int it) -> float4 {
        return *reinterpret_cast<const float4*>(base + step_pos(it) * step_bytes + voff);
    };
    auto x_half = [&](int buf, f32x4 (&g)[2]) {
#pragma unroll
        for (int m = 0; m < 2; ++m) g[m] = f32x4{0.f, 0.f, 0.f, 0.f};
#pragma unroll
        for (int ks = 0; ks < 2; ++ks) {
            const xp_f16x8 xh = *reinterpret_cast<const xp_f16x8*>(&ahi[buf * NS * XP_AP + a_frag + ks * 32]);
            const xp_f16x8 xl = *reinterpret_cast<const xp_f16x8*>(&alo[buf * NS * XP_AP + a_frag + ks * 32]);
#pragma unroll
            for (int m = 0; m < 2; ++m) g[m] = __builtin_amdgcn_mfma_f32_16x16x32_f16(wh[m][ks], xh, g[m], 0, 0, 0);
#pragma unroll
            for (int m = 0; m < 2; ++m) g[m] = __builtin_amdgcn_mfma_f32_16x16x32_f16(wh[m][ks], xl, g[m], 0, 0, 0);
#pragma unroll
            for (int m = 0; m < 2; ++m) g[m] = __builtin_amdgcn_mfma_f32_16x16x32_f16(wl[m][ks], xh, g[m], 0, 0, 0);
        }
    };

    float creg[2], hreg[2];
    float4 carryq[2] = {make_float4(0.f, 0.f, 0.f, 0.f), make_float4(0.f, 0.f, 0.f, 0.f)};
    if (!lin_wave) {
        norm_store_x(0, load_row(xb, 0));
        norm_store_x(1, load_row(xb, 1));
        carryq[0] = load_row(xb, 2);
        if (XP_PF == 2) carryq[1] = load_row(xb, 3);
    } else {
        const int s = min(s0 + rrow, nseq - 1);
        float4 hv = make_float4(0.f, 0.f, 0.f, 0.f);
        if (h0) hv = *reinterpret_cast<const float4*>(&h0[(long)s * H + q * 4]);
        store_split4(a_row + C, hv.x, hv.y, hv.z, hv.w);
    }
    {
        const int s = min(s0 + l15, nseq - 1);
#pragma unroll
        for (int m = 0; m < 2; ++m) {
            creg[m] = c0 ? ((cflags & 1) ? 1.0f : XP_K2) * c0[(long)s * H + unit0 + m] : 0.0f;
            hreg[m] = 0.0f;
        }
    }
    __syncthreads();
    f32x4 gx[2];
    x_half(0, gx);
    __syncthreads();

    auto step = [&](int it, auto cur_tag, auto lin_tag, auto store_tag) __attribute__((always_inline)) {
        constexpr int cur = decltype(cur_tag)::value, nxt = cur ^ 1;
        constexpr bool LIN = decltype(lin_tag)::value;
        constexpr bool STORE = decltype(store_tag)::value;
        float4& carry = carryq[XP_PF == 2 ? cur : 0];
        if (prio == 3) __builtin_amdgcn_s_setprio(3);
        if (prio == 4) __builtin_amdgcn_s_setprio(0);
        XP_STAMP(0);
        xp_f16x8 bh[2], bl[2];
#pragma unroll
        for (int ks = 0; ks < 2; ++ks) {
            bh[ks] = *reinterpret_cast<const xp_f16x8*>(&ahi[cur * NS * XP_AP + a_frag + (2 + ks) * 32]);
            bl[ks] = *reinterpret_cast<const xp_f16x8*>(&alo[cur * NS * XP_AP + a_frag + (2 + ks) * 32]);
        }
        f32x4 acc[2] = {gx[0], gx[1]};
        xp_f16x8 xh[2], xl[2];
        auto h_mfma = [&](auto idx) __attribute__((always_inline)) {
            constexpr int i = decltype(idx)::value, ks = i / 6, p = (i % 6) / 2, m = i % 2;
            acc[m] = __builtin_amdgcn_mfma_f32_16x16x32_f16(p == 2 ? wl[m][2 + ks] : wh[m][2 + ks], p == 1 ? bl[ks] : bh[ks],
                                                            acc[m], 0, 0, 0);
        };
        if constexpr (LIN) {
            float4 pv, done;
            auto h_ops = std::make_tuple(
                [&] { pv = *reinterpret_cast<const float4*>(&ls[nxt * NS * XP_LSP + l_row]); },
                [&] {}, [&] {}, [&] {},
                [&] { done.x = carry.x + pv.x; done.y = carry.y + pv.y; },
                [&] { done.z = carry.z + pv.z; done.w = carry.w + pv.w; },
                [&] { if (STORE) *reinterpret_cast<float4*>(ob + step_pos(it - 2) * step_bytes + voff) = done; },
                [&] { carry = load_row(bsrc, it + XP_PF - 2); });
            xp_zip<12>(h_mfma, h_ops);
        } else {
            float4 v, y;
            float s, t, qa, qb, rstd;
            xp_f16x4 h4, l4;
            auto h_ops = std::make_tuple(
                [&] { v = carry; s = v.x + v.y; t = v.z + v.w; },
                [&] { s += t; },
                [&] { s = row_ror_add<8>(s); },
                [&] { s = row_ror_add<4>(s); },
                [&] { s = row_ror_add<2>(s); },
                [&] { s = row_ror_add<1>(s); },
                [&] { v.x = __builtin_fmaf(s, -1.0f / C, v.x); v.y = __builtin_fmaf(s, -1.0f / C, v.y); },
                [&] { v.z = __builtin_fmaf(s, -1.0f / C, v.z); v.w = __builtin_fmaf(s, -1.0f / C, v.w); },
                [&] { qa = v.x * v.x; qb = v.z * v.z; },
                [&] { qa = __builtin_fmaf(v.y, v.y, qa); qb = __builtin_fmaf(v.w, v.w, qb); },
                [&] { qa += qb; },
                [&] { qa = row_ror_add<8>(qa); },
                [&] { qa = row_ror_add<4>(qa); },
                [&] { qa = row_ror_add<2>(qa); },
                [&] { qa = row_ror_add<1>(qa); },
                [&] { rstd = __builtin_amdgcn_rsqf(__builtin_fmaf(qa, 1.0f / C, LN_EPS)); },
                [&] { y.x = v.x * rstd; y.y = v.y * rstd; },
                [&] { y.z = v.z * rstd; y.w = v.w * rstd; },
                [&] { carry = load_row(xb, it + 2 + XP_PF); },
                [&] { f16x2_t a_, b_; split_pair(y.x, y.y, a_, b_); h4[0] = a_[0]; h4[1] = a_[1]; l4[0] = b_[0]; l4[1] = b_[1]; },
                [&] { },
                [&] { f16x2_t a_, b_; split_pair(y.z, y.w, a_, b_); h4[2] = a_[0]; h4[3] = a_[1]; l4[2] = b_[0]; l4[3] = b_[1]; },
                [&] {
                    *reinterpret_cast<xp_f16x4*>(&ahi[cur * NS * XP_AP + a_row]) = h4;
                    *reinterpret_cast<xp_f16x4*>(&alo[cur * NS * XP_AP + a_row]) = l4;
                },
                [&] {
                    xh[0] = *reinterpret_cast<const xp_f16x8*>(&ahi[nxt * NS * XP_AP + a_frag]);
                    xl[0] = *reinterpret_cast<const xp_f16x8*>(&alo[nxt * NS * XP_AP + a_frag]);
                    xh[1] = *reinterpret_cast<const xp_f16x8*>(&ahi[nxt * NS * XP_AP + a_frag + 32]);
                    xl[1] = *reinterpret_cast<const xp_f16x8*>(&alo[nxt * NS * XP_AP + a_frag + 32]);
                });
            xp_zip<12>(h_mfma, h_ops);
        }
        XP_STAMP(1);
        if (prio == 3) __builtin_amdgcn_s_setprio(0);
        if (prio == 4) __builtin_amdgcn_s_setprio(3);
        f32x4 am = f32x4{lbias, lbias, lbias, lbias};
        constexpr int NL = LIN ? 6 : 0;
        auto c_mfma = [&](auto idx) __attribute__((always_inline)) {
            constexpr int i = decltype(idx)::value;
            if constexpr (i < NL) {
                constexpr int ks = i / 3, p = i % 3;
                am = __builtin_amdgcn_mfma_f32_16x16x32_f16(p == 2 ? bl[ks] : bh[ks], p == 1 ? lwl[ks] : lwh[ks], am, 0, 0, 0);
            } else {
                constexpr int j = i - NL, ks = j / 6, p = (j % 6) / 2, m = j % 2;
                const f32x4 c0v = j < 2 ? f32x4{0.f, 0.f, 0.f, 0.f} : gx[m];
                gx[m] = __builtin_amdgcn_mfma_f32_16x16x32_f16(p == 2 ? wl[m][ks] : wh[m][ks], p == 1 ? xl[ks] : xh[ks], c0v, 0, 0, 0);
            }
        };
        float tc[2];
        auto cA = [&](auto m_) { constexpr int m = decltype(m_)::value; acc[m][0] = __builtin_amdgcn_exp2f(acc[m][0]); acc[m][1] = __builtin_amdgcn_exp2f(acc[m][1]); };
        auto cB = [&](auto m_) { constexpr int m = decltype(m_)::value; acc[m][2] = __builtin_amdgcn_exp2f(acc[m][2]); acc[m][3] = __builtin_amdgcn_exp2f(acc[m][3]); };
        auto cC = [&](auto m_) {
            constexpr int m = decltype(m_)::value;
#pragma unroll
            for (int g = 0; g < 4; ++g) acc[m][g] = __builtin_fmaf(acc[m][g], eb[m][g], 1.0f);
        };
        auto cD = [&](auto m_) { constexpr int m = decltype(m_)::value; acc[m][0] = __builtin_amdgcn_rcpf(acc[m][0]); acc[m][1] = __builtin_amdgcn_rcpf(acc[m][1]); };
        auto cE = [&](auto m_) { constexpr int m = decltype(m_)::value; acc[m][2] = __builtin_amdgcn_rcpf(acc[m][2]); acc[m][3] = __builtin_amdgcn_rcpf(acc[m][3]); };
        auto cF = [&](auto m_) {
            constexpr int m = decltype(m_)::value;
            const float g2 = __builtin_fmaf(2.0f * XP_K2, acc[m][2], -XP_K2);
            creg[m] = __builtin_fmaf(acc[m][1], creg[m], acc[m][0] * g2);
        };
        auto cG = [&](auto m_) { constexpr int m = decltype(m_)::value; tc[m] = 1.0f + __builtin_amdgcn_exp2f(creg[m]); };
        auto cH = [&](auto m_) { constexpr int m = decltype(m_)::value; tc[m] = __builtin_amdgcn_rcpf(tc[m]); };
        auto cI = [&](auto m_) {
            constexpr int m = decltype(m_)::value;
            hreg[m] = acc[m][3] * __builtin_fmaf(2.0f, tc[m], -1.0f);
            if constexpr (m == 1) {
                f16x2_t th2, tl2;
                split_pair(hreg[0], hreg[1], th2, tl2);
                *reinterpret_cast<f16x2_t*>(&ahi[nxt * NS * XP_AP + a_cell]) = th2;
                *reinterpret_cast<f16x2_t*>(&alo[nxt * NS * XP_AP + a_cell]) = tl2;
            }
        };
        using M0 = std::integral_constant<int, 0>;
        using M1 = std::integral_constant<int, 1>;
        auto c_ops = std::make_tuple(
            [&] {
                if constexpr (LIN) {
                    xh[0] = *reinterpret_cast<const xp_f16x8*>(&ahi[nxt * NS * XP_AP + a_frag]);
                    xl[0] = *reinterpret_cast<const xp_f16x8*>(&alo[nxt * NS * XP_AP + a_frag]);
                }
            },
            [&] {
                if constexpr (LIN) {
                    xh[1] = *reinterpret_cast<const xp_f16x8*>(&ahi[nxt * NS * XP_AP + a_frag + 32]);
                    xl[1] = *reinterpret_cast<const xp_f16x8*>(&alo[nxt * NS * XP_AP + a_frag + 32]);
                }
            },
            [&] { cA(M0{}); }, [&] { cA(M1{}); }, [&] { cB(M0{}); }, [&] { cB(M1{}); }, [&] { cC(M0{}); }, [&] { cC(M1{}); },
            [&] { cD(M0{}); }, [&] { cD(M1{}); }, [&] { cE(M0{}); }, [&] { cE(M1{}); },
            [&] {
                if constexpr (LIN) {
#pragma unroll
                    for (int r = 0; r < 4; ++r) ls[cur * NS * XP_LSP + r * XP_LSP + l_lin] = am[r];
                }
            },
            [&] { cF(M0{}); }, [&] { cF(M1{}); }, [&] { cG(M0{}); }, [&] { cG(M1{}); }, [&] { cH(M0{}); }, [&] { cH(M1{}); },
            [&] { cI(M0{}); }, [&] { cI(M1{}); });
        xp_zip<12 + NL>(c_mfma, c_ops);
        XP_STAMP(2);
        __syncthreads();
        XP_STAMP(3);
        __builtin_amdgcn_sched_barrier(0);
    };
    auto run = [&](auto lin_tag) __attribute__((always_inline)) {
        using B0 = std::integral_constant<int, 0>;
        using B1 = std::integral_constant<int, 1>;
        step(0, B0{}, lin_tag, std::false_type{});
        step(1, B1{}, lin_tag, std::false_type{});
        int it = 2;
        for (; it + 1 < nstep; it += 2) {
            step(it, B0{}, lin_tag, std::true_type{});
            step(it + 1, B1{}, lin_tag, std::true_type{});
        }
        if (it < nstep) step(it, B0{}, lin_tag, std::true_type{});
    };
    if (lin_wave) run(std::true_type{});
    else run(std::false_type{});

#if defined(XP_TRACE)
    __syncthreads();
    if (blockIdx.x == 3)
        for (int i = threadIdx.x; i < 2 * 128 * 4; i += 512) xp_trace_inter[i] = tr_all[i];
#endif
    const int lastb = nstep & 1;
    float4 carry = XP_PF == 2 ? (lastb ? carryq[1] : carryq[0]) : carryq[0];
    if (lin_wave) {
        if (nstep >= 2) {
            const float4 pv = *reinterpret_cast<const float4*>(&ls[(lastb ^ 1) * NS * XP_LSP + l_row]);
            *reinterpret_cast<float4*>(ob + step_pos(nstep - 2) * step_bytes + voff) =
                make_float4(carry.x + pv.x, carry.y + pv.y, carry.z + pv.z, carry.w + pv.w);
        }
        carry = XP_PF == 2 ? (lastb ? carryq[0] : carryq[1]) : load_row(bsrc, nstep - 1);
        f32x4 am = f32x4{lbias, lbias, lbias, lbias};
#pragma unroll
        for (int ks = 0; ks < 2; ++ks) {
            const xp_f16x8 ah = *reinterpret_cast<const xp_f16x8*>(&ahi[lastb * NS * XP_AP + a_frag + (2 + ks) * 32]);
            const xp_f16x8 al = *reinterpret_cast<const xp_f16x8*>(&alo[lastb * NS * XP_AP + a_frag + (2 + ks) * 32]);
            am = __builtin_amdgcn_mfma_f32_16x16x32_f16(ah, lwh[ks], am, 0, 0, 0);
            am = __builtin_amdgcn_mfma_f32_16x16x32_f16(ah, lwl[ks], am, 0, 0, 0);
            am = __builtin_amdgcn_mfma_f32_16x16x32_f16(al, lwh[ks], am, 0, 0, 0);
        }
#pragma unroll
        for (int r = 0; r < 4; ++r) ls[lastb * NS * XP_LSP + r * XP_LSP + l_lin] = am[r];
    }
    if (hN) {
#pragma unroll
        for (int m = 0; m < 2; ++m) hf[l15 * XP_LSP + unit0 + m] = hreg[m];
    }
    __syncthreads();
    if (lin_wave) {
        const float4 pv = *reinterpret_cast<const float4*>(&ls[lastb * NS * XP_LSP + l_row]);
        *reinterpret_cast<float4*>(ob + step_pos(nstep - 1) * step_bytes + voff) =
            make_float4(carry.x + pv.x, carry.y + pv.y, carry.z + pv.z, carry.w + pv.w);
    } else if (hN && s0 + rrow < nseq) {
        *reinterpret_cast<float4*>(&hN[(long)(s0 + rrow) * H + q * 4]) = *reinterpret_cast<const float4*>(&hf[l_row]);
    }
    if (cN && s0 + l15 < nseq) {
#pragma unroll
        for (int m = 0; m < 2; ++m) cN[(long)(s0 + l15) * H + unit0 + m] = creg[m] * ((cflags & 2) ? 1.0f : 1.0f / XP_K2);
    }
}

static int g_xp_lds_pad = 0;
static int g_xp_prio = 1;
static int g_xp_prio_inter = 3;

int launch_inter_xp(const float* x, const void* w_pk, const float* b_sum, const void* wlin_pk, const float* blin,
                    const float* h0, const float* c0, float* hN, float* cN, float* out, int nseq, int nstep, int sdiv, int so,
                    int si, int ps, hipStream_t st, int cflags) {
    if (nstep < 2) return LH_ERR_ARG;
    hipLaunchKernelGGL(k_inter_xp, dim3((nseq + 15) / 16), dim3(512), 0, st, x, (const _Float16*)w_pk, b_sum,
                       (const _Float16*)wlin_pk, blin, h0, c0, hN, cN, out, nseq, nstep, sdiv, so, si, ps, 0, 0, g_xp_prio_inter,
                       cflags);
    return check_launch();
}
int xp_set(int key, int v) {
    if (key == 7) g_xp_lds_pad = v < 0 ? 0 : v;
    if (key == 8) g_xp_prio = v;
    if (key == 9) g_xp_prio_inter = v;
    return LH_OK;
}

int launch_intra_xp(const float* x, const void* w_pk, const float* b_sum, const void* wlin_pk, const float* blin, float* out,
                    int nseq, int nstep, int sdiv, int so, int si, int ps, int dir, int accumulate, hipStream_t st) {
#if defined(LH_PROBE_INTRA1)
    if (dir == 1) return LH_OK;
    hipLaunchKernelGGL(k_intra_xp, dim3(2 * ((nseq + 15) / 16)), dim3(256), g_xp_lds_pad, st, x, (const _Float16*)w_pk, b_sum,
                       (const _Float16*)wlin_pk, blin, out, nseq, nstep, sdiv, so, si, ps, dir, accumulate, g_xp_prio);
    return check_launch();
#endif
    hipLaunchKernelGGL(k_intra_xp, dim3((nseq + 15) / 16), dim3(256), g_xp_lds_pad, st, x, (const _Float16*)w_pk, b_sum,
                       (const _Float16*)wlin_pk, blin, out, nseq, nstep, sdiv, so, si, ps, dir, accumulate, g_xp_prio);
    return check_launch();
}

}

#if defined(XP_TRACE)
extern "C" int lh_probe_xp_trace_inter_read(unsigned long long* host_dst) {
    return hipMemcpyFromSymbol(host_dst, HIP_SYMBOL(lh::xp_trace_inter), sizeof(lh::xp_trace_inter)) == hipSuccess ? 0 : 1;
}
extern "C" int lh_probe_xp_trace_read(unsigned long long* host_dst) {
    return hipMemcpyFromSymbol(host_dst, HIP_SYMBOL(lh::xp_trace_buf), sizeof(lh::xp_trace_buf)) == hipSuccess ? 0 : 1;
}
extern "C" int lh_probe_xp_wglog_read(unsigned long long* host_dst) {
    return hipMemcpyFromSymbol(host_dst, HIP_SYMBOL(lh::xp_wg_log), sizeof(lh::xp_wg_log)) == hipSuccess ? 0 : 1;
}
#endif
```

### lookoncetohear_amd/net.py

```python
from __future__ import annotations

import ctypes
import math
import os
from typing import Dict, Optional, Tuple

import numpy as np
import torch
import torch.nn as nn
import torch.nn.functional as F

from . import _cabi
from .weights import KV_PAD_ROWS, QK_PAD, pack_all, unsplit_qk, unsplit_v


def mod_pad(x: torch.Tensor, chunk_size: int, pad: Tuple[int, int]):
    mod = 0
    if x.shape[-1] % chunk_size != 0:
        mod = chunk_size - (x.shape[-1] % chunk_size)
    if mod or pad[0] or pad[1]:
        x = F.pad(x, (pad[0], mod + pad[1]))
    return x, mod


def stft_filterbank(n_fft: int, hop: int) -> torch.Tensor:
    nbin = n_fft // 2 + 1
    n = np.arange(n_fft)
    window = np.sqrt(0.5 - 0.5 * np.cos(2 * np.pi * n / n_fft))
    ang = 2 * np.pi * np.arange(nbin)[:, None] * n[None, :] / n_fft
    re, im = np.cos(ang), -np.sin(ang)
    re[0] /= np.sqrt(2)
    re[n_fft // 2] /= np.sqrt(2)
    rows = np.vstack([re, im]) * window[None, :] / (0.5 * np.sqrt(n_fft * n_fft / hop))
    return torch.from_numpy(rows).float().unsqueeze(1)


class _FilterBank(nn.Module):
    def __init__(self, n_fft, hop):
        super().__init__()
        self.register_buffer("_filters", stft_filterbank(n_fft, hop))


class _Coder(nn.Module):
    def __init__(self, n_fft, hop):
        super().__init__()
        self.filterbank = _FilterBank(n_fft, hop)


class _Norm(nn.Module):
    def __init__(self, n, eps):
        super().__init__()
        self.norm = nn.LayerNorm(n, eps=eps)


def _proj(n_in, n_out, n_norm, eps):
    return nn.Sequential(nn.Linear(n_in, n_out), nn.PReLU(), nn.Identity(), _Norm(n_norm, eps))


class _GridNetBlockParams(nn.Module):

    def __init__(self, emb_dim, n_freqs, hidden, n_head, eps):
        super().__init__()
        E = math.ceil(512 * 1.0 / n_freqs)
        self.intra_norm = _Norm(emb_dim, eps)
        self.intra_rnn = nn.LSTM(emb_dim, hidden, 1, batch_first=True, bidirectional=True)
        self.intra_linear = nn.Linear(hidden * 2, emb_dim)
        self.inter_norm = _Norm(emb_dim, eps)
        self.inter_rnn = nn.LSTM(emb_dim, hidden, 1, batch_first=True, bidirectional=False)
        self.inter_linear = nn.Linear(hidden, emb_dim)
        self.attn_conv_Q = _proj(emb_dim, E * n_head, n_freqs * E, eps)
        self.attn_conv_K = _proj(emb_dim, E * n_head, n_freqs * E, eps)
        self.attn_conv_V = _proj(emb_dim, (emb_dim // n_head) * n_head, n_freqs * (emb_dim // n_head), eps)
        self.attn_concat_proj = _proj(emb_dim, emb_dim, n_freqs * emb_dim, eps)


class _TFGridNetParams(nn.Module):

    def __init__(self, n_fft, stride, n_imics, n_srcs, emb_dim, n_layers, hidden, n_head, spk_emb_dim, eps=1.0e-5):
        super().__init__()
        n_freqs = n_fft // 2 + 1
        self.enc = _Coder(n_fft, stride)
        self.dec = _Coder(n_fft, stride)
        self.conv = nn.Sequential(nn.Conv2d(2 * n_imics, emb_dim, (3, 3), padding=(0, 1)))
        self.blocks = nn.ModuleList(
            [_GridNetBlockParams(emb_dim, n_freqs, hidden, n_head, eps) for _ in range(n_layers)])
        self.embed_to_feats_proj = nn.Sequential(nn.Linear(spk_emb_dim, emb_dim * n_freqs),
                                                 nn.LayerNorm(emb_dim * n_freqs))
        self.deconv = nn.ConvTranspose2d(emb_dim, n_srcs * 2, (3, 3), padding=(2, 1))


class _Lanes:
    serial = False

    def __init__(self, dev, side_streams):
        self.dev = dev
        self.main = torch.cuda.current_stream(dev)
        self.streams = [self.main] + list(side_streams)

    def fork(self):
        ev = torch.cuda.Event()
        ev.record(self.main)
        for s_ in self.streams[1:]:
            s_.wait_event(ev)

    def on(self, k):
        return torch.cuda.stream(self.streams[k])

    def signal(self, k):
        ev = torch.cuda.Event()
        ev.record(self.streams[k])
        return ev

    def wait(self, k, ev):
        self.streams[k].wait_event(ev)

    def join(self):
        for s_ in self.streams[1:]:
            self.main.wait_stream(s_)


class _EnrollSide:

    def __init__(self, dev, low_priority: bool = False):
        self.dev = dev
        self._hip, self._raw = None, None
        if low_priority:
            hip = self._hip = _cabi.load()._dll
            least, greatest, raw = ctypes.c_int(0), ctypes.c_int(0), ctypes.c_void_p()
            with torch.cuda.device(dev):
                if (hip.hipDeviceGetStreamPriorityRange(ctypes.byref(least), ctypes.byref(greatest)) != 0 or
                        hip.hipStreamCreateWithPriority(ctypes.byref(raw), 1, least.value) != 0):
                    raise RuntimeError("could not create a low-priority HIP stream")
            self._raw = raw
            self.stream = torch.cuda.ExternalStream(raw.value, device=dev)
        else:
            self.stream = torch.cuda.Stream(device=dev)

    def __del__(self):
        if self._raw is not None:
            self._hip.hipStreamDestroy(self._raw)

    def run(self, fn):
        ev = torch.cuda.Event()
        ev.record(torch.cuda.current_stream(self.dev))
        self.stream.wait_event(ev)
        with torch.cuda.stream(self.stream):
            out = fn()
        done = torch.cuda.Event()
        done.record(self.stream)
        return out, done

    def finished(self, done) -> bool:
        return done.query()

    def hand_over(self, done, out: torch.Tensor):
        main = torch.cuda.current_stream(self.dev)
        main.wait_event(done)
        out.record_stream(main)


class Net(_cabi.HipHost, nn.Module):
    _host_name = "Net"
    enroll_low_priority = False

    def __init__(self, stft_chunk_size=160, stft_pad_size=120, embed_dim=256,
                 num_ch=2, D=64, B=6, I=1, J=1, L=0, H=128,
                 use_attn=False, lookahead=True, local_atten_len=100,
                 chunk_causal=False, num_src=2):
        super().__init__()
        self.ctor_params = dict(stft_chunk_size=stft_chunk_size, stft_pad_size=stft_pad_size, embed_dim=embed_dim,
                                num_ch=num_ch, D=D, B=B, I=I, J=J, L=L, H=H, use_attn=use_attn, lookahead=lookahead,
                                local_atten_len=local_atten_len, chunk_causal=chunk_causal, num_src=num_src)
        self.stft_chunk_size = stft_chunk_size
        self.stft_pad_size = stft_pad_size
        self.num_ch = num_ch
        self.lookahead = lookahead
        self.nfft = stft_chunk_size + stft_pad_size
        self.n_blocks, self.emb_dim, self.hidden, self.n_head = B, D, H, L
        self.n_freqs = self.nfft // 2 + 1
        self.local_atten_len = local_atten_len
        self.n_srcs = num_src
        self.spk_emb_dim = embed_dim
        if not (use_attn and chunk_causal):
            raise NotImplementedError("only the chunk-causal attention mode of configs/tsh.json is implemented")
        shape = (self.nfft, stft_chunk_size, num_ch, D, H, L, local_atten_len, num_src, embed_dim)
        if shape != (192, 128, 2, 64, 64, 4, 50, 2, 256):
            raise NotImplementedError(
                f"the gfx950 kernels are specialised on the configs/tsh.json shapes; got (nfft, hop, mics, D, H, L, "
                f"window, srcs, embed_dim) = {shape}")
        self.E = math.ceil(512 * 1.0 / self.n_freqs)
        self.V_dim = D // L
        self.tfgridnet = _TFGridNetParams(self.nfft, stft_chunk_size, num_ch, num_src, D, B, H, L, embed_dim)
        self.gemm_mode = os.environ.get("LOOKONCE_GEMM", "f16x3")
        self._check_gemm_mode()
        rc = os.environ.get("LOOKONCE_RANGE_CHECK", "1")
        self.range_check = False if rc == "0" else ("sync" if rc == "sync" else True)
        self._range_flags: Dict[str, torch.Tensor] = {}
        self.fuse_linear = os.environ.get("LOOKONCE_FUSE", "1") != "0"
        self.fuse_intra_min_frames = int(os.environ.get("LOOKONCE_FUSE_INTRA_MIN_FRAMES", "6000"))
        self.inter_matvec_max_seqs = int(os.environ.get("LOOKONCE_MATVEC_MAX_SEQS", "256"))
        self.stream_intra_max_frames = 128
        self.n_cus = 256
        self.time_chunks = int(os.environ.get("LOOKONCE_TIME_CHUNKS", "0"))
        self.time_chunks_small = int(os.environ.get("LOOKONCE_TIME_CHUNKS_SMALL", "0"))
        self.chunk_min_frames = 64
        self._chunk_streams: Dict[str, list] = {}
        self._pack_key = None
        self._packed = None
        self._ws: Dict[tuple, dict] = {}
        self._zeros: Dict[tuple, dict] = {}
        self._blob = None
        self._debug_taps: Optional[dict] = None
        self._prof: Optional[list] = None
        self._prof_only: Optional[set] = None
        self._prof_stride: int = 1
        self._prof_count: dict = {}
        self._register_load_state_dict_pre_hook(self._drop_foreign_filterbank_keys)

    @staticmethod
    def _drop_foreign_filterbank_keys(state_dict, prefix, *_):
        for k in [k for k in state_dict if k.startswith(prefix) and ".filterbank." in k and not k.endswith("._filters")]:
            state_dict.pop(k)

    def init_buffers(self, batch_size, device):
        z = lambda *s: torch.zeros(*s, device=device)
        F_, C_, L_ = self.n_freqs, self.emb_dim, self.local_atten_len
        bufs = {}
        for i in range(self.n_blocks):
            bufs[f"buf{i}"] = dict(K_buf=z(batch_size * self.n_head, L_ - 1, self.E * F_),
                                   V_buf=z(batch_size * self.n_head, L_ - 1, self.V_dim * F_),
                                   c0=z(1, batch_size * F_, self.hidden),
                                   h0=z(1, batch_size * F_, self.hidden))
        return dict(conv_buf=z(batch_size, self.num_ch * 2, 2, F_), deconv_buf=z(batch_size, C_, 2, F_),
                    istft_buf=z(batch_size, self.n_srcs, F_ * 2, 1), gridnet_bufs=bufs)

    def predict(self, x, embed, input_state, pad=True, want_state=True):
        mod = 0
        if pad:
            pad_size = (0, self.stft_pad_size) if self.lookahead else (0, 0)
            x, mod = mod_pad(x, chunk_size=self.stft_chunk_size, pad=pad_size)
        x, next_state = self._separate(x, embed, input_state, want_state)
        if mod != 0:
            x = x[:, :, :-mod]
        return x, next_state

    def forward(self, x, embeds, input_state=None, pad=True):
        embeds = embeds[:, 0]
        x, next_state = self.predict(x, embeds, input_state, pad, want_state=input_state is not None)
        return x

    def make_streamer(self, batch_size: int, device, use_graph: bool = True):
        return Streamer(self, batch_size, device, use_graph)

    def make_session_streamer(self, n_slots: int, device, use_graph: bool = True, enroll_chunks: int = 0,
                              compact: bool = False, row_buckets=None):
        return SessionStreamer(self, n_slots, device, use_graph, enroll_chunks, compact, row_buckets)

    def _enroll_side(self, dev) -> _EnrollSide:
        return _EnrollSide(dev, self.enroll_low_priority)

    @classmethod
    def from_packed(cls, path: str, device) -> "Net":
        from . import checkpoint
        meta, flat = checkpoint.import_packed(path, device)
        if meta["model"] != "separator":
            raise ValueError(f"{path}: holds a {meta['model']!r} blob")
        if meta["abi_version"] != _cabi.ABI_VERSION:
            raise ValueError(f"{path}: packed for ABI v{meta['abi_version']}, library is v{_cabi.ABI_VERSION}")
        net = cls(**meta["params"]).eval()
        net.tfgridnet = None
        tree: dict = {"blocks": [dict() for _ in range(net.n_blocks)]}
        for name, t in flat.items():
            if name.startswith("blocks."):
                _, i, key = name.split(".", 2)
                tree["blocks"][int(i)][key] = t
            else:
                tree[name] = t
        net._blob = (next(iter(flat.values())).device, tree)
        return net

    def _weights(self, device) -> dict:
        if self._blob is not None:
            if torch.device(device) != self._blob[0]:
                raise RuntimeError(f"packed weights live on {self._blob[0]}, input on {device}")
            return self._blob[1]
        tensors = list(self.parameters()) + list(self.buffers())
        key = (str(device),) + tuple((t.data_ptr(), t._version) for t in tensors)
        if key != self._pack_key:
            sd = {k: v for k, v in self.state_dict(keep_vars=True).items()}
            for k, v in sd.items():
                if v.device != device:
                    raise RuntimeError(f"parameter {k} lives on {v.device}, input on {device}")
            with torch.no_grad():
                self._packed = pack_all(sd, self.n_blocks)
            self._pack_key = key
        return self._packed

    def _workspace(self, B, T, device) -> dict:
        key = (B, T, str(device))
        ws = self._ws.get(key)
        if ws is None:
            if len(self._ws) > 4:
                self._ws.clear()
            F_, C_, nh = self.n_freqs, self.emb_dim, self.n_head
            e = lambda *s: torch.empty(*s, device=device, dtype=torch.float32)
            hist = self.local_atten_len - 1
            z16 = lambda *s: torch.zeros(*s, device=device, dtype=torch.float16)
            ws = dict(xa=e(B, T, F_, C_), xb=e(B, T, F_, C_), xc=e(B, T, F_, C_), hbuf=e(B * T * F_, 2 * self.hidden),
                      q=z16(B * nh, T, 2 * QK_PAD), kx=z16(B * nh, T + hist + KV_PAD_ROWS, 2 * QK_PAD),
                      vx=z16(B * nh, T + hist + KV_PAD_ROWS, 2 * self.V_dim * F_), gain=e(B, F_, C_),
                      gain_raw=e(B, F_ * C_), hist_dirty=False)
            self._ws[key] = ws
        return ws

    @staticmethod
    def _dev_key(device) -> str:
        dev = torch.device(device)
        if dev.type == "cuda" and dev.index is None:
            dev = torch.device("cuda", torch.cuda.current_device())
        return str(dev)

    def _range_flag(self, device) -> torch.Tensor:
        key = self._dev_key(device)
        if key not in self._range_flags:
            self._range_flags[key] = self._flag_words(torch.device(key))
        return self._range_flags[key]

    def range_status(self, device=None) -> bool:
        if device is None:
            keys = list(self._range_flags)
        else:
            keys = [self._dev_key(device)]
        bad = False
        for key in keys:
            dev = torch.device(key)
            flag = self._range_flag(dev)
            self._sync(dev)
            if int(flag[0]) != 0:
                flag.zero_()
                bad = True
        return bad

    def _sync(self, dev):
        torch.cuda.current_stream(dev).synchronize()

    _RANGE_MSG = ("LH_ERR_RANGE: {} produced non-finite samples. The frame kernels scale every row by a power of "
                  "two before the fp16 hi + lo split, so this means inf / NaN in the input or the state, or an activation "
                  "beyond the fp32 range itself (include/lookonce_hip.h, range contract).")

    def _zero_state(self, B, device) -> dict:
        key = (B, str(device))
        if key not in self._zeros:
            if len(self._zeros) > 4:
                self._zeros.clear()
            self._zeros[key] = self.init_buffers(B, device)
        return self._zeros[key]

    def _separate(self, x: torch.Tensor, embed: torch.Tensor, state: Optional[dict], want_state: bool = True):
        if self.training and torch.is_grad_enabled():
            raise RuntimeError("lookoncetohear_amd.Net is an inference-only drop-in (forward kernels, no autograd): call "
                               ".eval() and/or run under torch.no_grad(); training stays on the reference model")
        self._check_gemm_mode()
        if self.gemm_mode == "f32all":
            return self._separate_ref32(x, embed, state, want_state)
        lib = self._lib(x)
        dev = x.device
        if self.range_check and int(self._range_flag(dev)[0]) != 0:
            self._range_flag(dev).zero_()
            raise RuntimeError(self._RANGE_MSG.format("an earlier forward of this Net"))
        hop, nfft = self.stft_chunk_size, self.nfft
        assert x.dim() == 3 and x.shape[1] == self.num_ch, "input must be [B, num_ch, N]"
        Bn, _, n = x.shape
        from_zero = state is None and not want_state
        if state is None:
            state = self._zero_state(Bn, dev) if from_zero else self.init_buffers(Bn, dev)
        T = (n - nfft) // hop + 1
        if T < 1:
            raise ValueError(f"need at least {nfft} samples, got {n}")
        ns = (T - 1) * hop + nfft
        x = x[..., :ns].contiguous().float()
        embed = embed.contiguous().float()
        F_, C_, nh, H_ = self.n_freqs, self.emb_dim, self.n_head, self.hidden
        hist = self.local_atten_len - 1
        with torch.no_grad(), self._device_ctx(x):
            pk = self._weights(dev)
            ws = self._workspace(Bn, T, dev)
            st = self._stream(dev)
            P = lambda t: t.data_ptr()
            new = lambda t: torch.empty_like(t, dtype=torch.float32)
            c32 = lambda t: t.contiguous().float()
            taps = self._debug_taps
            xa, xb, xc, hbuf = ws["xa"], ws["xb"], ws["xc"], ws["hbuf"]
            prof = self._prof
            only = self._prof_only
            stride, count = self._prof_stride, self._prof_count

            class _Timed:
                @staticmethod
                def call(fn, *args):
                    name = fn[:-4] if fn.endswith("_win") else fn
                    if prof is None or (only is not None and name not in only):
                        return lib_.call(fn, *args)
                    if stride > 1:
                        n = count.get(name, 0)
                        count[name] = n + 1
                        if n % stride:
                            return lib_.call(fn, *args)
                    e0, e1 = torch.cuda.Event(enable_timing=True), torch.cuda.Event(enable_timing=True)
                    e0.record()
                    lib_.call(fn, *args)
                    e1.record()
                    prof.append((name, e0, e1))

            lib_, lib = lib, _Timed

            conv_in = c32(state["conv_buf"]); conv_out = new(conv_in)
            lib.call("lh_stft_conv_in", P(x), P(conv_in), P(conv_out), P(pk["wfb_t"]), P(pk["conv_w"]),
                     P(pk["conv_b"]), P(xa), Bn, T, ns, st)
            lib.call("lh_embed_proj_ln", P(embed), P(pk["emb_w"]), P(pk["emb_b"]), P(pk["emb_ln_w"]),
                     P(pk["emb_ln_b"]), P(ws["gain_raw"]), P(ws["gain"]), Bn, st)
            if taps is not None:
                taps["Z0"], taps["G"] = xa.clone(), ws["gain"].clone()

            rows = Bn * T * F_
            mode = 1 if self.gemm_mode == "f16x3" else 0
            wkey, bkey = ("_w16", "_b16") if mode else ("_w", "_b")
            K = self._n_time_chunks(Bn, T, mode)
            if K > 1:
                self._blocks_chunked(lib, pk, ws, state, Bn, T, dev, from_zero, want_state, K)
            for i in range(self.n_blocks if K == 1 else 0):
                bp = pk["blocks"][i]
                bs = state["gridnet_bufs"][f"buf{i}"]
                h0, c0 = c32(bs["h0"]), c32(bs["c0"])
                hN, cN = new(h0), new(c0)
                fuse = mode == 1 and self.fuse_linear
                if fuse and Bn * T >= self.fuse_intra_min_frames:
                    lib.call("lh_intra_block", P(xa), P(bp["intra_w16"]), P(bp["intra_b16"]), P(bp["intra_lin_w2"]),
                             P(bp["intra_lin_b"]), P(xb), Bn * T, st)
                elif mode == 1 and Bn * T <= self.stream_intra_max_frames:
                    lib.call("lh_intra_stream", P(xa), P(bp["intra_s_wih"]), P(bp["intra_s_b"]), P(bp["intra_s_whh"]),
                             P(hbuf), Bn * T, st)
                    lib.call("lh_linear_res", P(hbuf), P(bp["intra_lin_w"]), P(bp["intra_lin_b"]), P(xa), P(xb), rows,
                             2 * H_, st)
                else:
                    lib.call("lh_ln_lstm_intra", P(xa), P(bp["intra_ln_w"]), P(bp["intra_ln_b"]), P(bp["intra" + wkey]),
                             P(bp["intra" + bkey]), P(hbuf), Bn * T, mode, st)
                    lib.call("lh_linear_res", P(hbuf), P(bp["intra_lin_w"]), P(bp["intra_lin_b"]), P(xa), P(xb), rows,
                             2 * H_, st)
                if fuse and Bn * F_ <= self.inter_matvec_max_seqs and T >= 32:
                    lib.call("lh_inter_matvec", P(xb), P(bp["inter_s_wih"]), P(bp["inter_s_b"]), P(bp["inter_s_whh"]),
                             P(bp["inter_lin_w"]), P(bp["inter_lin_b"]), P(h0), P(c0), P(hN), P(cN), P(xc), Bn, T, st)
                elif fuse:
                    lib.call("lh_inter_block", P(xb), P(bp["inter_w8"]), P(bp["inter_b16"]), P(bp["inter_lin_wu"]),
                             P(bp["inter_lin_b"]), P(h0), P(c0), P(hN), P(cN), P(xc), Bn, T, st)
                else:
                    lib.call("lh_ln_lstm_inter", P(xb), P(bp["inter_ln_w"]), P(bp["inter_ln_b"]), P(bp["inter" + wkey]),
                             P(bp["inter" + bkey]), P(h0), P(c0), P(hN), P(cN), P(hbuf), Bn, T, mode, st)
                    lib.call("lh_linear_res", P(hbuf), P(bp["inter_lin_w"]), P(bp["inter_lin_b"]), P(xb), P(xc), rows,
                             H_, st)
                if not from_zero:
                    lib.call("lh_ring_pack", P(c32(bs["K_buf"])), P(c32(bs["V_buf"])), P(ws["kx"]), P(ws["vx"]), Bn, T, st)
                    ws["hist_dirty"] = True
                elif ws["hist_dirty"]:
                    ws["kx"][:, :hist].zero_()
                    ws["vx"][:, :hist].zero_()
                    ws["hist_dirty"] = False
                lib.call("lh_qkv_proj_ln", P(xc), P(bp["qkv_w"]), P(bp["qkv_b"]), P(bp["qkv_slopes"]), P(bp["lnq_w"]),
                         P(bp["lnq_b"]), P(bp["lnk_w"]), P(bp["lnk_b"]), P(bp["lnv_w"]), P(bp["lnv_b"]), P(ws["q"]),
                         P(ws["kx"]), P(ws["vx"]), None, Bn, T, st)
                lib.call("lh_local_attn", P(ws["q"]), P(ws["kx"]), P(ws["vx"]), P(xb), Bn, T, st)
                if taps is not None:
                    taps[f"blocks.{i}.attn"] = xb.clone()
                gain = ws["gain"] if (i == 0 and self.n_blocks > 1) else None
                lib.call("lh_proj_ln_res", P(xb), P(bp["proj_w"]), P(bp["proj_b"]), P(bp["proj_slope"]),
                         P(bp["proj_ln_w"]), P(bp["proj_ln_b"]), P(xc), P(gain) if gain is not None else None, P(xa),
                         Bn, T, st)
                if want_state:
                    bs["h0"], bs["c0"] = hN, cN
                    bs["K_buf"] = torch.empty(Bn * nh, hist, self.E * F_, device=dev, dtype=torch.float32)
                    bs["V_buf"] = torch.empty(Bn * nh, hist, self.V_dim * F_, device=dev, dtype=torch.float32)
                    lib.call("lh_ring_unpack", P(ws["kx"]), P(ws["vx"]), P(bs["K_buf"]), P(bs["V_buf"]), Bn, T, st)
                if taps is not None:
                    taps[f"blocks.{i}.Y2"] = xc.clone()
                    taps[f"blocks.{i}.Q"] = unsplit_qk(ws["q"], self.E * F_)
                    taps[f"blocks.{i}.K"] = unsplit_qk(ws["kx"][:, hist:hist + T], self.E * F_)
                    taps[f"blocks.{i}.V"] = unsplit_v(ws["vx"][:, hist:hist + T])
                    taps[f"blocks.{i}.out"] = xa.clone()

            dec_in, ist_in = c32(state["deconv_buf"]), c32(state["istft_buf"])
            dec_out, ist_out = new(dec_in), new(ist_in)
            y = torch.empty(Bn, self.n_srcs, hop * T, device=dev, dtype=torch.float32)
            flag = self._range_flag(dev)
            lib.call("lh_deconv_istft", P(xa), P(dec_in), P(dec_out), P(ist_in), P(ist_out), P(pk["deconv_w"]),
                     P(pk["deconv_b"]), P(pk["wfb_dec"]), P(y), P(flag), 1, Bn, T, st)
            if want_state:
                state["conv_buf"], state["deconv_buf"], state["istft_buf"] = conv_out, dec_out, ist_out
            if self.range_check == "sync" and not self._capturing():
                if self.range_status(dev):
                    raise RuntimeError(self._RANGE_MSG.format("this forward"))
        return y, (state if want_state else None)

    def _n_time_chunks(self, Bn: int, T: int, mode: int) -> int:
        if mode != 1 or not self.fuse_linear or self._debug_taps is not None:
            return 1
        if Bn * self.n_freqs <= self.inter_matvec_max_seqs and T < 32:
            return 1
        if Bn * T < self.fuse_intra_min_frames:
            if Bn * T <= self.stream_intra_max_frames:
                return 1
            K = int(self.time_chunks_small)
            if K == 0:
                nseq = Bn * self.n_freqs
                K = 3
                if nseq <= self.inter_matvec_max_seqs:
                    tail = nseq % self.n_cus or self.n_cus
                    K = 1 if tail >= 0.6 * self.n_cus else (2 if nseq <= self.n_cus else 3)
        else:
            K = int(self.time_chunks)
            if K == 0:
                tiles = (Bn * self.n_freqs + 15) // 16
                K = 2 if tiles < 0.7 * self.n_cus else 1
            while K > 1 and Bn * (T // K) < self.fuse_intra_min_frames // 2:
                K -= 1
        return max(min(K, T // max(self.chunk_min_frames, 1)), 1)

    def _window_bounds(self, Bn: int, T: int, K: int) -> list:
        bh8 = (Bn * self.n_head + 7) // 8 * 8
        align = 40 if bh8 * ((T + 31) // 32) > 512 else 32
        if Bn * self.n_freqs <= self.inter_matvec_max_seqs:
            align = 64
        cuts = [(k * T) // K for k in range(K + 1)]
        if T // K >= 2 * align or (align == 64 and T // K >= 64):
            cuts = [0] + [int(round(k * T / K / align)) * align for k in range(1, K)] + [T]
        return cuts

    def _lanes(self, dev, K) -> _Lanes:
        pool = self._chunk_streams.setdefault(str(dev), [])
        while len(pool) < K - 1:
            pool.append(torch.cuda.Stream(device=dev))
        if self.chunk_min_frames < self.local_atten_len - 1:
            raise ValueError("chunk_min_frames must cover the attention history (49 frames) on concurrent streams")
        return _Lanes(dev, pool[:K - 1])

    def _blocks_chunked(self, lib, pk, ws, state, Bn, T, dev, from_zero, want_state, K):
        F_, nh, hist = self.n_freqs, self.n_head, self.local_atten_len - 1
        P = lambda t: t.data_ptr()
        c32 = lambda t: t.contiguous().float()
        xa, xb, xc = ws["xa"], ws["xb"], ws["xc"]
        lanes = self._lanes(dev, K)
        unfused_intra = Bn * T < self.fuse_intra_min_frames
        matvec_inter = Bn * F_ <= self.inter_matvec_max_seqs
        if "kxb" not in ws:
            z16 = lambda *s_: torch.zeros(*s_, device=dev, dtype=torch.float16)
            ws["kxb"] = [ws["kx"]] + [z16(*ws["kx"].shape) for _ in range(self.n_blocks - 1)]
            ws["vxb"] = [ws["vx"]] + [z16(*ws["vx"].shape) for _ in range(self.n_blocks - 1)]
            ws["hist_dirty_b"] = [False] * self.n_blocks
        bounds = self._window_bounds(Bn, T, K)
        hs, cs = [], []
        for i in range(self.n_blocks):
            bs = state["gridnet_bufs"][f"buf{i}"]
            h0, c0 = c32(bs["h0"]).reshape(-1, self.hidden), c32(bs["c0"]).reshape(-1, self.hidden)
            hs.append([h0] + [torch.empty_like(h0) for _ in range(K)])
            cs.append([c0] + [torch.empty_like(c0) for _ in range(K)])
            kx, vx = ws["kxb"][i], ws["vxb"][i]
            if not from_zero:
                lib.call("lh_ring_pack", P(c32(bs["K_buf"])), P(c32(bs["V_buf"])), P(kx), P(vx), Bn, T, self._stream(dev))
                ws["hist_dirty_b"][i] = True
                if i == 0:
                    ws["hist_dirty"] = True
            elif ws["hist_dirty_b"][i] or (i == 0 and ws["hist_dirty"]):
                kx[:, :hist].zero_()
                vx[:, :hist].zero_()
                ws["hist_dirty_b"][i] = False
                if i == 0:
                    ws["hist_dirty"] = False
        lanes.fork()
        for i in range(self.n_blocks):
            bp = pk["blocks"][i]
            kx, vx = ws["kxb"][i], ws["vxb"][i]
            gain = ws["gain"] if (i == 0 and self.n_blocks > 1) else None
            ev_r = ev_q = None
            for k in range(K):
                t0, Tc = bounds[k], bounds[k + 1] - bounds[k]
                carry = (1 if k > 0 else 0) | (2 if k + 1 < K else 0)
                with lanes.on(k):
                    st = self._stream(dev)
                    if unfused_intra:
                        lib.call("lh_ln_lstm_intra_win", P(xa), P(bp["intra_ln_w"]), P(bp["intra_ln_b"]), P(bp["intra_w16"]),
                                 P(bp["intra_b16"]), P(ws["hbuf"]), Bn, T, t0, Tc, st)
                        lib.call("lh_linear_res_win", P(ws["hbuf"]), P(bp["intra_lin_w"]), P(bp["intra_lin_b"]), P(xa), P(xb),
                                 Bn, T, t0, Tc, 2 * self.hidden, st)
                    else:
                        lib.call("lh_intra_block_win", P(xa), P(bp["intra_w16"]), P(bp["intra_b16"]), P(bp["intra_lin_w2"]),
                                 P(bp["intra_lin_b"]), P(xb), Bn, T, t0, Tc, st)
                    if k > 0:
                        lanes.wait(k, ev_r)
                    if matvec_inter:
                        lib.call("lh_inter_matvec_win", P(xb), P(bp["inter_s_wih"]), P(bp["inter_s_b"]), P(bp["inter_s_whh"]),
                                 P(bp["inter_lin_w"]), P(bp["inter_lin_b"]), P(hs[i][k]), P(cs[i][k]), P(hs[i][k + 1]),
                                 P(cs[i][k + 1]), P(xc), Bn, T, t0, Tc, carry, st)
                    else:
                        lib.call("lh_inter_block_win", P(xb), P(bp["inter_w8"]), P(bp["inter_b16"]), P(bp["inter_lin_wu"]),
                                 P(bp["inter_lin_b"]), P(hs[i][k]), P(cs[i][k]), P(hs[i][k + 1]), P(cs[i][k + 1]), P(xc), Bn, T,
                                 t0, Tc, carry, st)
                    if k + 1 < K:
                        ev_r = lanes.signal(k)
                    lib.call("lh_qkv_proj_ln_win", P(xc), P(bp["qkv_w"]), P(bp["qkv_b"]), P(bp["qkv_slopes"]), P(bp["lnq_w"]),
                             P(bp["lnq_b"]), P(bp["lnk_w"]), P(bp["lnk_b"]), P(bp["lnv_w"]), P(bp["lnv_b"]), P(ws["q"]),
                             P(kx), P(vx), None, Bn, T, t0, Tc, st)
                    ev_prev = ev_q
                    if k + 1 < K:
                        ev_q = lanes.signal(k)
                    if k > 0:
                        lanes.wait(k, ev_prev)
                    lib.call("lh_local_attn_win", P(ws["q"]), P(kx), P(vx), P(xb), Bn, T, t0, Tc, st)
                    lib.call("lh_proj_ln_res_win", P(xb), P(bp["proj_w"]), P(bp["proj_b"]), P(bp["proj_slope"]),
                             P(bp["proj_ln_w"]), P(bp["proj_ln_b"]), P(xc), P(gain) if gain is not None else None, P(xa),
                             Bn, T, t0, Tc, st)
        lanes.join()
        if want_state:
            for i in range(self.n_blocks):
                bs = state["gridnet_bufs"][f"buf{i}"]
                bs["h0"], bs["c0"] = hs[i][K].reshape(1, -1, self.hidden), cs[i][K].reshape(1, -1, self.hidden)
                bs["K_buf"] = torch.empty(Bn * nh, hist, self.E * F_, device=dev, dtype=torch.float32)
                bs["V_buf"] = torch.empty(Bn * nh, hist, self.V_dim * F_, device=dev, dtype=torch.float32)
                lib.call("lh_ring_unpack", P(ws["kxb"][i]), P(ws["vxb"][i]), P(bs["K_buf"]), P(bs["V_buf"]), Bn, T,
                         self._stream(dev))

    def _check_gemm_mode(self):
        if self.gemm_mode not in ("f32rec", "f32all", "f16x3"):
            raise ValueError(f"gemm_mode / LOOKONCE_GEMM must be 'f16x3', 'f32rec' or 'f32all', got {self.gemm_mode!r}"
                             + (" ('f32' was the pre-round-5 spelling of 'f32rec')" if self.gemm_mode == "f32" else ""))

    def _capturing(self) -> bool:
        return torch.cuda.is_current_stream_capturing()

    def _separate_ref32(self, x: torch.Tensor, embed: torch.Tensor, state: Optional[dict], want_state: bool = True):
        if self._blob is not None:
            raise RuntimeError("gemm_mode='f32all' reads the parameter tree; a `from_packed` Net has none")
        lib = self._lib(x)
        dev = x.device
        hop, nfft = self.stft_chunk_size, self.nfft
        assert x.dim() == 3 and x.shape[1] == self.num_ch, "input must be [B, num_ch, N]"
        Bn, _, n = x.shape
        if state is None:
            state = self.init_buffers(Bn, dev)
        T = (n - nfft) // hop + 1
        if T < 1:
            raise ValueError(f"need at least {nfft} samples, got {n}")
        ns = (T - 1) * hop + nfft
        x = x[..., :ns].contiguous().float()
        embed = embed.contiguous().float()
        F_, C_, nh, H_ = self.n_freqs, self.emb_dim, self.n_head, self.hidden
        hist = self.local_atten_len - 1
        rows = Bn * T * F_
        with torch.no_grad(), self._device_ctx(x):
            pk = self._weights(dev)
            sd = {k: v.detach().float().contiguous() for k, v in self.tfgridnet.state_dict().items()}
            st = self._stream(dev)
            P = lambda t: t.data_ptr()
            e = lambda *s: torch.empty(*s, device=dev, dtype=torch.float32)
            c32 = lambda t: t.contiguous().float()
            xa, xb, xc, hbuf = e(Bn, T, F_, C_), e(Bn, T, F_, C_), e(Bn, T, F_, C_), e(rows, 2 * H_)
            gain_raw, gain = e(Bn, F_ * C_), e(Bn, F_, C_)
            conv_in = c32(state["conv_buf"]); conv_out = torch.empty_like(conv_in)
            spec_s, sx_s = e(Bn, 2 * self.num_ch, T + 2, F_), e(Bn, self.n_srcs, T + 1, 2 * F_)
            lib.call("lh_ref32_stft_conv_in", P(x), P(conv_in), P(conv_out), P(sd["enc.filterbank._filters"]),
                     P(sd["conv.0.weight"]), P(sd["conv.0.bias"]), P(spec_s), P(xa), Bn, T, ns, st)
            lib.call("lh_embed_proj_ln", P(embed), P(pk["emb_w"]), P(pk["emb_b"]), P(pk["emb_ln_w"]), P(pk["emb_ln_b"]),
                     P(gain_raw), P(gain), Bn, st)
            taps = self._debug_taps
            if taps is not None:
                taps["Z0"], taps["G"] = xa.clone(), gain.clone()
            pre, rows_s, pre_s = e(rows, 112), e(rows, C_), e(rows, C_)
            q = e(Bn * nh, T, self.E * F_)
            for i in range(self.n_blocks):
                bp, bs, g = pk["blocks"][i], state["gridnet_bufs"][f"buf{i}"], f"blocks.{i}."
                h0, c0 = c32(bs["h0"]), c32(bs["c0"])
                hN, cN = torch.empty_like(h0), torch.empty_like(c0)
                lib.call("lh_ln_lstm_intra", P(xa), P(bp["intra_ln_w"]), P(bp["intra_ln_b"]), P(bp["intra_w"]), P(bp["intra_b"]),
                         P(hbuf), Bn * T, 0, st)
                lib.call("lh_ref32_linear", P(hbuf), P(sd[g + "intra_linear.weight"]), P(sd[g + "intra_linear.bias"]), None,
                         P(xa), P(xb), rows, 2 * H_, C_, st)
                lib.call("lh_ln_lstm_inter", P(xb), P(bp["inter_ln_w"]), P(bp["inter_ln_b"]), P(bp["inter_w"]), P(bp["inter_b"]),
                         P(h0), P(c0), P(hN), P(cN), P(hbuf), Bn, T, 0, st)
                lib.call("lh_ref32_linear", P(hbuf), P(sd[g + "inter_linear.weight"]), P(sd[g + "inter_linear.bias"]), None,
                         P(xb), P(xc), rows, H_, C_, st)
                kx, vx = e(Bn * nh, T + hist, self.E * F_), e(Bn * nh, T + hist, self.V_dim * F_)
                kx[:, :hist] = bs["K_buf"].float()
                vx[:, :hist] = bs["V_buf"].float()
                for nm, D, dst, row0, rpb in (("Q", self.E, q, 0, T), ("K", self.E, kx, hist, T + hist),
                                              ("V", self.V_dim, vx, hist, T + hist)):
                    a = g + f"attn_conv_{nm}."
                    ncol = nh * D
                    lib.call("lh_ref32_linear", P(xc), P(sd[a + "0.weight"]), P(sd[a + "0.bias"]), P(sd[a + "1.weight"]), None,
                             P(pre), rows, C_, ncol, st)
                    lib.call("lh_ref32_head_ln", P(pre), ncol, 0, D, P(sd[a + "3.norm.weight"]), P(sd[a + "3.norm.bias"]),
                             P(dst), row0, rpb, Bn, T, st)
                lib.call("lh_ref32_local_attn", P(q), P(kx), P(vx), P(xb), Bn, T, st)
                a = g + "attn_concat_proj."
                gn = gain if (i == 0 and self.n_blocks > 1) else None
                lib.call("lh_ref32_proj_ln_res", P(xb), P(sd[a + "0.weight"]), P(sd[a + "0.bias"]), P(sd[a + "1.weight"]),
                         P(sd[a + "3.norm.weight"]), P(sd[a + "3.norm.bias"]), P(xc), P(gn) if gn is not None else None,
                         P(rows_s), P(pre_s), P(xa), Bn, T, st)
                if want_state:
                    bs["h0"], bs["c0"] = hN, cN
                    bs["K_buf"], bs["V_buf"] = kx[:, T:T + hist].clone(), vx[:, T:T + hist].clone()
                if taps is not None:
                    taps[f"blocks.{i}.Y2"], taps[f"blocks.{i}.Q"] = xc.clone(), q.clone()
                    taps[f"blocks.{i}.K"], taps[f"blocks.{i}.V"] = kx[:, hist:].clone(), vx[:, hist:].clone()
                    taps[f"blocks.{i}.out"] = xa.clone()
            dec_in, ist_in = c32(state["deconv_buf"]), c32(state["istft_buf"])
            dec_out, ist_out = torch.empty_like(dec_in), torch.empty_like(ist_in)
            y = e(Bn, self.n_srcs, hop * T)
            lib.call("lh_ref32_deconv_istft", P(xa), P(dec_in), P(dec_out), P(ist_in), P(ist_out), P(sd["deconv.weight"]),
                     P(sd["deconv.bias"]), P(sd["dec.filterbank._filters"]), P(sx_s), P(y), Bn, T, st)
            if want_state:
                state["conv_buf"], state["deconv_buf"], state["istft_buf"] = conv_out, dec_out, ist_out
        return y, (state if want_state else None)

    def _speaker_gain(self, embed: torch.Tensor, gain_raw: torch.Tensor, gain: torch.Tensor):
        lib = self._lib(embed)
        pk = self._weights(embed.device)
        st = self._stream(embed.device)
        P = lambda t: t.data_ptr()
        with self._device_ctx(embed):
            lib.call("lh_embed_proj_ln", P(embed), P(pk["emb_w"]), P(pk["emb_b"]), P(pk["emb_ln_w"]), P(pk["emb_ln_b"]),
                     P(gain_raw), P(gain), embed.shape[0], st)

    def _stream_chunk(self, x, gain, sin: dict, sout: dict, rings, pos, y, pk: dict, ws: dict, flag=None,
                      keep_nonfinite: int = 0):
        lib = self._lib(x)
        dev = x.device
        hop, nfft = self.stft_chunk_size, self.nfft
        Bn, _, n = x.shape
        T = (n - nfft) // hop + 1
        assert T == 1 and n == nfft, "the streaming path takes chunks of stft_chunk_size + stft_pad_size samples"
        F_, H_ = self.n_freqs, self.hidden
        st = self._stream(dev)
        P = lambda t: t.data_ptr()
        xa, xb, xc, hbuf = ws["xa"], ws["xb"], ws["xc"], ws["hbuf"]
        lib.call("lh_stft_conv_in", P(x), P(sin["conv_buf"]), P(sout["conv_buf"]), P(pk["wfb_t"]), P(pk["conv_w"]),
                 P(pk["conv_b"]), P(xa), Bn, T, n, st)
        for i in range(self.n_blocks):
            bp = pk["blocks"][i]
            kx, vx = rings[i]
            lib.call("lh_intra_stream", P(xa), P(bp["intra_s_wih"]), P(bp["intra_s_b"]), P(bp["intra_s_whh"]), P(hbuf),
                     Bn * T, st)
            lib.call("lh_linear_res", P(hbuf), P(bp["intra_lin_w"]), P(bp["intra_lin_b"]), P(xa), P(xb), Bn * T * F_,
                     2 * H_, st)
            lib.call("lh_inter_block", P(xb), P(bp["inter_w8"]), P(bp["inter_b16"]), P(bp["inter_lin_wu"]),
                     P(bp["inter_lin_b"]), P(sin["h"][i]), P(sin["c"][i]), P(sout["h"][i]), P(sout["c"][i]), P(xc), Bn, T, st)
            lib.call("lh_qkv_proj_ln", P(xc), P(bp["qkv_w"]), P(bp["qkv_b"]), P(bp["qkv_slopes"]), P(bp["lnq_w"]),
                     P(bp["lnq_b"]), P(bp["lnk_w"]), P(bp["lnk_b"]), P(bp["lnv_w"]), P(bp["lnv_b"]), P(ws["q"]),
                     P(kx), P(vx), P(pos), Bn, T, st)
            lib.call("lh_local_attn", P(ws["q"]), P(kx), P(vx), P(xb), Bn, T, st)
            g = gain if (i == 0 and self.n_blocks > 1) else None
            lib.call("lh_proj_ln_res", P(xb), P(bp["proj_w"]), P(bp["proj_b"]), P(bp["proj_slope"]),
                     P(bp["proj_ln_w"]), P(bp["proj_ln_b"]), P(xc), P(g) if g is not None else None, P(xa), Bn, T, st)
        lib.call("lh_deconv_istft", P(xa), P(sin["deconv_buf"]), P(sout["deconv_buf"]), P(sin["istft_buf"]),
                 P(sout["istft_buf"]), P(pk["deconv_w"]), P(pk["deconv_b"]), P(pk["wfb_dec"]), P(y),
                 P(flag) if flag is not None else None, keep_nonfinite, Bn, T, st)



class Streamer:

    def __init__(self, net: Net, batch_size: int, device, use_graph: bool = True):
        if net.gemm_mode != "f16x3" or not net.fuse_linear:
            raise ValueError("Streamer runs the split-precision fused kernels (LOOKONCE_GEMM=f16x3, LOOKONCE_FUSE=1)")
        self.net = net
        self.B = B = batch_size
        self.device = dev = torch.device(device)
        n = net.stft_chunk_size + net.stft_pad_size
        z = lambda *s, **k: torch.zeros(*s, device=dev, **k)
        self.chunk = z(B, net.num_ch, n)
        self.embed = z(B, net.spk_emb_dim)
        self.out = z(B, net.n_srcs, net.stft_chunk_size)
        F_, C_, nh, H_ = net.n_freqs, net.emb_dim, net.n_head, net.hidden
        mk = lambda: dict(conv_buf=z(B, net.num_ch * 2, 2, F_), deconv_buf=z(B, C_, 2, F_),
                          istft_buf=z(B, net.n_srcs, F_ * 2, 1),
                          h=[z(1, B * F_, H_) for _ in range(net.n_blocks)], c=[z(1, B * F_, H_) for _ in range(net.n_blocks)])
        self.sets = [mk(), mk()]
        rows = 1 + net.local_atten_len - 1 + KV_PAD_ROWS
        self.rings = [(z(B * nh, rows, 2 * QK_PAD, dtype=torch.float16), z(B * nh, rows, 2 * net.V_dim * F_, dtype=torch.float16))
                      for _ in range(net.n_blocks)]
        self.pos = z(1, dtype=torch.int32)
        self.gain = z(B, F_, C_)
        self.gain_raw = z(B, F_ * C_)
        self.range_flag = net._flag_words(dev)
        self.parity = 0
        self.graphs = None
        self.graph = None
        with torch.no_grad(), net._device_ctx(self.chunk):
            self._pk = net._weights(dev)
            self._pack_key = net._pack_key
            self._n_steps = 0
            self._versions = [] if net._blob is not None else [(t, t._version) for t in list(net.parameters()) + list(net.buffers())]
            self._vpos = 0
            self._ws = net._workspace(B, 1, dev)
            net._ws.pop((B, 1, str(dev)), None)
        if use_graph:
            self.graphs = self._capture(self._body, dev)
            self.graph = self.graphs[0]
            self.reset()

    @staticmethod
    def _capture(body, dev) -> list:
        side = torch.cuda.Stream(device=dev)
        side.wait_stream(torch.cuda.current_stream(dev))
        with torch.cuda.stream(side):
            for k in (0, 1):
                body(k)
        torch.cuda.current_stream(dev).wait_stream(side)
        graphs = []
        for k in (0, 1):
            g = torch.cuda.CUDAGraph()
            with torch.cuda.graph(g):
                body(k)
            graphs.append(g)
        return graphs

    def _body(self, k: int):
        with self.net._device_ctx(self.chunk):
            self.net._stream_chunk(self.chunk, self.gain, self.sets[k], self.sets[k ^ 1], self.rings, self.pos, self.out,
                                   self._pk, self._ws, self.range_flag)
            st = self.net._stream(self.device)
            self.net._lib(self.pos).call("lh_ring_advance", self.pos.data_ptr(), self.net.local_atten_len, st)

    def reset(self):
        for st in self.sets:
            for t in [st["conv_buf"], st["deconv_buf"], st["istft_buf"]] + st["h"] + st["c"]:
                t.zero_()
        for kx, vx in self.rings:
            kx.zero_()
            vx.zero_()
        self.pos.zero_()
        self.range_flag.zero_()
        self.parity = 0

    def set_embedding(self, embed: torch.Tensor):
        self.embed.copy_(embed.reshape(self.B, -1))
        with torch.no_grad():
            self.net._speaker_gain(self.embed, self.gain_raw, self.gain)

    def step(self, chunk: torch.Tensor) -> torch.Tensor:
        self._check_repacked()
        if self.net.range_check and int(self.range_flag[0]) != 0:
            self.range_flag.zero_()
            raise RuntimeError("LH_ERR_RANGE: an earlier chunk produced non-finite samples, emitted as zeros (inf / NaN in "
                               "the input or in the carried state); reset() the streamer")
        self._check_versions()
        self.chunk.copy_(chunk)
        with torch.no_grad():
            if self.graphs is not None:
                self.graphs[self.parity].replay()
            else:
                self._body(self.parity)
        self.parity ^= 1
        return self.out

    def _check_repacked(self):
        net = self.net
        cur = net._blob[1] if net._blob is not None else net._packed
        if cur is not self._pk:
            raise RuntimeError("the Net's parameters changed after this Streamer was built (its HIP graphs hold pointers "
                               "into the old packed weights): create a new streamer with net.make_streamer(...)")

    def _check_versions(self):
        self._n_steps += 1
        for _ in range(3 if self._versions else 0):
            t, v = self._versions[self._vpos]
            self._vpos = (self._vpos + 1) % len(self._versions)
            if t._version != v:
                raise RuntimeError("a parameter of the Net was modified in place after this Streamer was built: create a new "
                                   "streamer with net.make_streamer(...)")


class _Span(ctypes.Structure):
    _fields_ = [("base", ctypes.c_void_p), ("bytes", ctypes.c_ulonglong)]


class SessionStreamer:
    RESET, OPEN, CLOSE, GEN_SHIFT, MAX_SPANS, GEN_MASK = 1, 2, 4, 8, 32, 0x7fffff
    ARM, CANCEL, ENROLL_FAULT = 1, 2, 0x80000000

    def __init__(self, net: Net, n_slots: int, device, use_graph: bool = True, enroll_chunks: int = 0, compact: bool = False,
                 row_buckets=None):
        if n_slots < 1:
            raise ValueError("n_slots must be positive")
        if row_buckets is not None and not compact:
            raise ValueError("row_buckets are the launch sizes of a compacting streamer: compact=True")
        if compact:
            if row_buckets is None:
                row_buckets = [1 << i for i in range(n_slots.bit_length()) if 1 << i < n_slots] + [n_slots]
            row_buckets = tuple(int(b) for b in row_buckets)
            if not row_buckets or row_buckets[0] < 1 or row_buckets[-1] != n_slots or \
                    any(a >= b for a, b in zip(row_buckets, row_buckets[1:])):
                raise ValueError(f"row_buckets must ascend from >= 1 to n_slots = {n_slots}, got {row_buckets}")
        if enroll_chunks < 0 or enroll_chunks == 1:
            raise ValueError("enroll_chunks must be 0 (no enrollment) or >= 2: the embedder needs 4 STFT frames at stride 64, "
                             "192 samples, and a chunk records 128")
# ... 323 lines not shown
```

Measured before the change: 2.905 million frames/s.

## Compute inter-LSTM LayerNorm stats in intra kernel epilogue and reuse them

The fused intra-block kernel gets a stats variant. Its second-direction pass, which finalises the residual output, also computes each row's mean and rstd and writes them to a small stats buffer. The inter-block kernel gets a variant that reads these precomputed stats, so it no longer runs the row reductions for LayerNorm inside its latency-bound recurrent loop. The cost is extra work and an extra store in the intra kernel, a new per-frame stats buffer, and more kernel variants and ABI entries.

Result: slower. 2.873 million frames/s (-1.1%).

```diff
diff --git a/include/lookonce_hip.h b/include/lookonce_hip.h
--- a/include/lookonce_hip.h
+++ b/include/lookonce_hip.h
@@ -86,6 +86,16 @@
 int lh_inter_block_win(const float* x, const void* w_pk, const float* b_sum, const void* wlin_pk, const float* blin,
                        const float* h0, const float* c0, float* hN, float* cN, float* out, int B, int T, int t0, int Tc,
                        int carry, lh_stream_t stream);
+int lh_intra_block_stats(const float* x, const void* w_pk, const float* b_sum, const void* wlin_pk, const float* blin,
+                         float* out, float* stats, int n_frames, lh_stream_t stream);
+int lh_intra_block_stats_win(const float* x, const void* w_pk, const float* b_sum, const void* wlin_pk, const float* blin,
+                             float* out, float* stats, int B, int T, int t0, int Tc, lh_stream_t stream);
+int lh_inter_block_stats(const float* x, const float* stats, const void* w_pk, const float* b_sum, const void* wlin_pk,
+                         const float* blin, const float* h0, const float* c0, float* hN, float* cN, float* out, int B, int T,
+                         lh_stream_t stream);
+int lh_inter_block_stats_win(const float* x, const float* stats, const void* w_pk, const float* b_sum, const void* wlin_pk,
+                             const float* blin, const float* h0, const float* c0, float* hN, float* cN, float* out, int B,
+                             int T, int t0, int Tc, int carry, lh_stream_t stream);
 int lh_ln_lstm_intra_win(const float* x, const float* ln_w, const float* ln_b, const void* w_pk, const float* b_sum, float* h_out,
                          int B, int T, int t0, int Tc, lh_stream_t stream);
 int lh_linear_res_win(const float* h, const void* w_pk, const float* bias, const float* res, float* out, int B, int T, int t0,
diff --git a/lookoncetohear_amd/_cabi.py b/lookoncetohear_amd/_cabi.py
--- a/lookoncetohear_amd/_cabi.py
+++ b/lookoncetohear_amd/_cabi.py
@@ -6,7 +6,7 @@
 
 _PKG = os.path.dirname(os.path.abspath(__file__))
 HIP_LIB_PATH = os.path.join(_PKG, "_lookonce_hip.so")
-ABI_VERSION = 18
+ABI_VERSION = 19
 
 _P, _I = c_void_p, c_int
 SIGNATURES = {
@@ -37,6 +37,10 @@
     "lh_deconv_istft": [_P] * 10 + [_I, _I, _I, _P],
     "lh_intra_block_win": [_P] * 6 + [_I, _I, _I, _I, _P],
     "lh_inter_block_win": [_P] * 10 + [_I, _I, _I, _I, _I, _P],
+    "lh_intra_block_stats": [_P] * 7 + [_I, _P],
+    "lh_intra_block_stats_win": [_P] * 7 + [_I, _I, _I, _I, _P],
+    "lh_inter_block_stats": [_P] * 11 + [_I, _I, _P],
+    "lh_inter_block_stats_win": [_P] * 11 + [_I, _I, _I, _I, _I, _P],
     "lh_ln_lstm_intra_win": [_P] * 6 + [_I, _I, _I, _I, _P],
     "lh_linear_res_win": [_P] * 5 + [_I, _I, _I, _I, _I, _P],
     "lh_inter_matvec_win": [_P] * 11 + [_I, _I, _I, _I, _I, _P],
diff --git a/lookoncetohear_amd/csrc/lh_frontend.hip b/lookoncetohear_amd/csrc/lh_frontend.hip
--- a/lookoncetohear_amd/csrc/lh_frontend.hip
+++ b/lookoncetohear_amd/csrc/lh_frontend.hip
@@ -246,7 +246,7 @@
     return check_launch();
 }
 
-extern "C" int lh_abi_version(void) { return 18; }
+extern "C" int lh_abi_version(void) { return 19; }
 
 extern "C" int lh_check_config(int nfft, int hop, int n_mics, int emb_dim, int n_blocks_unused, int lstm_hidden,
                                int n_heads, int attn_window, int n_srcs, int spk_emb_dim) {
diff --git a/lookoncetohear_amd/csrc/lh_lstm.hip b/lookoncetohear_amd/csrc/lh_lstm.hip
--- a/lookoncetohear_amd/csrc/lh_lstm.hip
+++ b/lookoncetohear_amd/csrc/lh_lstm.hip
@@ -924,11 +924,12 @@
 namespace lh { int attn_set_mq(int v); }
 namespace lh {
 int launch_intra_xp(const float* x, const void* w_pk, const float* b_sum, const void* wlin_pk, const float* blin, float* out,
-                    int nseq, int nstep, int sdiv, int so, int si, int ps, int dir, int accumulate, hipStream_t st);
+                    int nseq, int nstep, int sdiv, int so, int si, int ps, int dir, int accumulate, hipStream_t st,
+                    float* stats = nullptr);
 int xp_set(int key, int v);
 int launch_inter_xp(const float* x, const void* w_pk, const float* b_sum, const void* wlin_pk, const float* blin,
                     const float* h0, const float* c0, float* hN, float* cN, float* out, int nseq, int nstep, int sdiv, int so,
-                    int si, int ps, hipStream_t st, int cflags = 0);
+                    int si, int ps, hipStream_t st, int cflags = 0, const float* stats = nullptr);
 }
 namespace lh { int backend_set_runs(int v); }
 #if defined(LH_PROBE_TRACE)
@@ -1075,3 +1076,55 @@
                            b_sum, (const _Float16*)wlin_pk, blin, h0, c0, hN, cN, out, nseq, T, NF, T * NF, 1, NF, 0, 0);
     return check_launch();
 }
+
+extern "C" int lh_intra_block_stats(const float* x, const void* w_pk, const float* b_sum, const void* wlin_pk,
+                                    const float* blin, float* out, float* stats, int n_frames, lh_stream_t stream) {
+    using namespace lh;
+    if (!x || !w_pk || !b_sum || !wlin_pk || !blin || !out || !stats || n_frames <= 0 || x == out) return LH_ERR_ARG;
+    int rc = LH_OK;
+    for (int dir = 0; dir < 2 && rc == LH_OK; ++dir)
+        rc = launch_intra_xp(x, w_pk, b_sum, (const _Float16*)wlin_pk + (long)dir * 4 * 2 * 64 * 16, blin, out, n_frames,
+                             NF, 1, NF, 0, 1, dir, dir, (hipStream_t)stream, stats);
+    return rc;
+}
+
+extern "C" int lh_intra_block_stats_win(const float* x, const void* w_pk, const float* b_sum, const void* wlin_pk,
+                                        const float* blin, float* out, float* stats, int B, int T, int t0, int Tc,
+                                        lh_stream_t stream) {
+    using namespace lh;
+    if (!x || !w_pk || !b_sum || !wlin_pk || !blin || !out || !stats || B <= 0 || T <= 0 || x == out || t0 < 0 || Tc <= 0 ||
+        t0 + Tc > T)
+        return LH_ERR_ARG;
+    const long off = (long)t0 * NF;
+    int rc = LH_OK;
+    for (int dir = 0; dir < 2 && rc == LH_OK; ++dir)
+        rc = launch_intra_xp(x + off * C, w_pk, b_sum, (const _Float16*)wlin_pk + (long)dir * 4 * 2 * 64 * 16, blin, out + off * C,
+                             B * Tc, NF, Tc, T * NF, NF, 1, dir, dir, (hipStream_t)stream, stats + off * 2);
+    return rc;
+}
+
+extern "C" int lh_inter_block_stats_win(const float* x, const float* stats, const void* w_pk, const float* b_sum,
+                                        const void* wlin_pk, const float* blin, const float* h0, const float* c0, float* hN,
+                                        float* cN, float* out, int B, int T, int t0, int Tc, int carry, lh_stream_t stream) {
+    using namespace lh;
+    if (!x || !stats || !w_pk || !b_sum || !wlin_pk || !blin || !h0 || !c0 || !hN || !cN || !out || B <= 0 || T <= 0)
+        return LH_ERR_ARG;
+    if (h0 == hN || c0 == cN || x == out || t0 < 0 || Tc < 2 || t0 + Tc > T || (carry & ~3)) return LH_ERR_ARG;
+    const long off = (long)t0 * NF;
+    return launch_inter_xp(x + off * C, w_pk, b_sum, wlin_pk, blin, h0, c0, hN, cN, out + off * C, B * NF, Tc, NF, T * NF, 1, NF,
+                           (hipStream_t)stream, carry, stats + off * 2);
+}
+
+extern "C" int lh_inter_block_stats(const float* x, const float* stats, const void* w_pk, const float* b_sum,
+                                    const void* wlin_pk, const float* blin, const float* h0, const float* c0, float* hN,
+                                    float* cN, float* out, int B, int T, lh_stream_t stream) {
+    using namespace lh;
+    if (!stats) return LH_ERR_ARG;
+    if (g_tune[5] != 2 && T >= 2) {
+        if (!x || !w_pk || !b_sum || !wlin_pk || !blin || !h0 || !c0 || !hN || !cN || !out || B <= 0) return LH_ERR_ARG;
+        if (h0 == hN || c0 == cN || x == out) return LH_ERR_ARG;
+        return launch_inter_xp(x, w_pk, b_sum, wlin_pk, blin, h0, c0, hN, cN, out, B * NF, T, NF, T * NF, 1, NF,
+                               (hipStream_t)stream, 0, stats);
+    }
+    return lh_inter_block(x, w_pk, b_sum, wlin_pk, blin, h0, c0, hN, cN, out, B, T, stream);
+}
diff --git a/lookoncetohear_amd/csrc/lh_recur.hip b/lookoncetohear_amd/csrc/lh_recur.hip
--- a/lookoncetohear_amd/csrc/lh_recur.hip
+++ b/lookoncetohear_amd/csrc/lh_recur.hip
@@ -67,10 +67,12 @@
 constexpr int XP_NP = 3;
 #endif
 
-__global__ void __launch_bounds__(256, 2) k_intra_xp(const float* __restrict__ x, const _Float16* __restrict__ w_pk,
-                                                     const float* __restrict__ b_sum, const _Float16* __restrict__ wlin_pk,
-                                                     const float* __restrict__ blin, float* out, int nseq, int nstep,
-                                                     int sdiv, int so, int si, int ps, int dir, int accumulate, int prio) {
+template <bool STATS>
+__device__ __forceinline__ void intra_xp_body(const float* __restrict__ x, const _Float16* __restrict__ w_pk,
+                                              const float* __restrict__ b_sum, const _Float16* __restrict__ wlin_pk,
+                                              const float* __restrict__ blin, float* out, int nseq, int nstep,
+                                              int sdiv, int so, int si, int ps, int dir, int accumulate, int prio,
+                                              float* stats) {
     constexpr int NS = 16;
     __shared__ __attribute__((aligned(16))) _Float16 ahi[2 * NS * XP_AP];
     __shared__ __attribute__((aligned(16))) _Float16 alo[2 * NS * XP_AP];
@@ -109,6 +111,23 @@
         accumulate ? reinterpret_cast<unsigned long long>(ob) : reinterpret_cast<unsigned long long>(xb));
     const long step_bytes = (long)ps * (C * 4);
     auto step_pos = [&](int it) -> int { it = min(max(it, 0), nstep - 1); return dir ? (nstep - 1 - it) : it; };
+    char* sb = STATS ? reinterpret_cast<char*>(stats) + wg_row0 * 8 : nullptr;
+    const unsigned svoff = (voff >> 8) * 8;
+    auto store_stats = [&](int it, float s, float rstd) {
+        if (q == 0) *reinterpret_cast<float2*>(sb + step_pos(it) * (step_bytes >> 5) + svoff) = make_float2(s, rstd);
+    };
+    auto row_stats = [&](int it, float4 d) {
+        float s = d.x + d.y, t = d.z + d.w;
+        s += t;
+        s = group16_sum(s);
+        d.x = __builtin_fmaf(s, -1.0f / C, d.x); d.y = __builtin_fmaf(s, -1.0f / C, d.y);
+        d.z = __builtin_fmaf(s, -1.0f / C, d.z); d.w = __builtin_fmaf(s, -1.0f / C, d.w);
+        float qa = d.x * d.x, qb = d.z * d.z;
+        qa = __builtin_fmaf(d.y, d.y, qa); qb = __builtin_fmaf(d.w, d.w, qb);
+        qa += qb;
+        qa = group16_sum(qa);
+        store_stats(it, s, __builtin_amdgcn_rsqf(__builtin_fmaf(qa, 1.0f / C, LN_EPS)));
+    };
 
     xp_f16x8 wh[4][4], wl[4][4];
     {
@@ -209,50 +228,112 @@
         float4 v, pv, done, y;
         float s, t, qa, qb, rstd;
         xp_f16x4 h4, l4;
-        auto h_ops = std::make_tuple(
-            [&] { v = xr; s = v.x + v.y; t = v.z + v.w; },
-            [&] { s += t; pv = *reinterpret_cast<const float4*>(&ls[nxt * NS * XP_LSP + l_row]); },
-            [&] { s = row_ror_add<8>(s); },
-            [&] { s = row_ror_add<4>(s); },
-            [&] { s = row_ror_add<2>(s); },
-            [&] { s = row_ror_add<1>(s); },
-            [&] { v.x = __builtin_fmaf(s, -1.0f / C, v.x); v.y = __builtin_fmaf(s, -1.0f / C, v.y); },
-            [&] { v.z = __builtin_fmaf(s, -1.0f / C, v.z); v.w = __builtin_fmaf(s, -1.0f / C, v.w); },
-            [&] { qa = v.x * v.x; qb = v.z * v.z; },
-            [&] { qa = __builtin_fmaf(v.y, v.y, qa); qb = __builtin_fmaf(v.w, v.w, qb); },
-            [&] { qa += qb; done.x = rr.x + pv.x; },
-            [&] { qa = row_ror_add<8>(qa); done.y = rr.y + pv.y; },
-            [&] { qa = row_ror_add<4>(qa); done.z = rr.z + pv.z; },
-            [&] { qa = row_ror_add<2>(qa); done.w = rr.w + pv.w; },
-            [&] { qa = row_ror_add<1>(qa); },
-            [&] {
-                rstd = __builtin_amdgcn_rsqf(__builtin_fmaf(qa, 1.0f / C, LN_EPS));
+        if constexpr (!STATS) {
+            auto h_ops = std::make_tuple(
+                [&] { v = xr; s = v.x + v.y; t = v.z + v.w; },
+                [&] { s += t; pv = *reinterpret_cast<const float4*>(&ls[nxt * NS * XP_LSP + l_row]); },
+                [&] { s = row_ror_add<8>(s); },
+                [&] { s = row_ror_add<4>(s); },
+                [&] { s = row_ror_add<2>(s); },
+                [&] { s = row_ror_add<1>(s); },
+                [&] { v.x = __builtin_fmaf(s, -1.0f / C, v.x); v.y = __builtin_fmaf(s, -1.0f / C, v.y); },
+                [&] { v.z = __builtin_fmaf(s, -1.0f / C, v.z); v.w = __builtin_fmaf(s, -1.0f / C, v.w); },
+                [&] { qa = v.x * v.x; qb = v.z * v.z; },
+                [&] { qa = __builtin_fmaf(v.y, v.y, qa); qb = __builtin_fmaf(v.w, v.w, qb); },
+                [&] { qa += qb; done.x = rr.x + pv.x; },
+                [&] { qa = row_ror_add<8>(qa); done.y = rr.y + pv.y; },
+                [&] { qa = row_ror_add<4>(qa); done.z = rr.z + pv.z; },
+                [&] { qa = row_ror_add<2>(qa); done.w = rr.w + pv.w; },
+                [&] { qa = row_ror_add<1>(qa); },
+                [&] {
+                    rstd = __builtin_amdgcn_rsqf(__builtin_fmaf(qa, 1.0f / C, LN_EPS));
 #if defined(XP_PROBE_NOGLOBAL)
-                if (STORE && done.x == 1.2345e30f) *reinterpret_cast<float4*>(ob + step_pos(it - 2) * step_bytes + voff) = done;
+                    if (STORE && done.x == 1.2345e30f) *reinterpret_cast<float4*>(ob + step_pos(it - 2) * step_bytes + voff) = done;
 #else
-                if (STORE) *reinterpret_cast<float4*>(ob + step_pos(it - 2) * step_bytes + voff) = done;
-#endif
-            },
+                    if (STORE) *reinterpret_cast<float4*>(ob + step_pos(it - 2) * step_bytes + voff) = done;
+#endif
+                },
 #if defined(XP_PROBE_NOGLOBAL)
-            [&] { if (!STORE) rr = load_base(it - 1); },
+                [&] { if (!STORE) rr = load_base(it - 1); },
 #else
-            [&] { rr = load_base(it - 1); },
-#endif
-            [&] { y.x = v.x * rstd; y.y = v.y * rstd; },
-            [&] { y.z = v.z * rstd; y.w = v.w * rstd; },
-            [&] { f16x2_t a_, b_; split_pair(y.x, y.y, a_, b_); h4[0] = a_[0]; h4[1] = a_[1]; l4[0] = b_[0]; l4[1] = b_[1]; },
-            [&] { },
-            [&] { f16x2_t a_, b_; split_pair(y.z, y.w, a_, b_); h4[2] = a_[0]; h4[3] = a_[1]; l4[2] = b_[0]; l4[3] = b_[1]; },
-            [&] {
-                *reinterpret_cast<xp_f16x4*>(&ahi[cur * NS * XP_AP + a_row]) = h4;
-                *reinterpret_cast<xp_f16x4*>(&alo[cur * NS * XP_AP + a_row]) = l4;
-            },
+                [&] { rr = load_base(it - 1); },
+#endif
+                [&] { y.x = v.x * rstd; y.y = v.y * rstd; },
+                [&] { y.z = v.z * rstd; y.w = v.w * rstd; },
+                [&] { f16x2_t a_, b_; split_pair(y.x, y.y, a_, b_); h4[0] = a_[0]; h4[1] = a_[1]; l4[0] = b_[0]; l4[1] = b_[1]; },
+                [&] { },
+                [&] { f16x2_t a_, b_; split_pair(y.z, y.w, a_, b_); h4[2] = a_[0]; h4[3] = a_[1]; l4[2] = b_[0]; l4[3] = b_[1]; },
+                [&] {
+                    *reinterpret_cast<xp_f16x4*>(&ahi[cur * NS * XP_AP + a_row]) = h4;
+                    *reinterpret_cast<xp_f16x4*>(&alo[cur * NS * XP_AP + a_row]) = l4;
+                },
 #if defined(XP_PROBE_NOGLOBAL)
-            [&] { if (!STORE) xr = load_x(it + 3); });
+                [&] { if (!STORE) xr = load_x(it + 3); });
 #else
-            [&] { xr = load_x(it + 3); });
-#endif
-        xp_zip<24>(h_mfma, h_ops);
+                [&] { xr = load_x(it + 3); });
+#endif
+            xp_zip<24>(h_mfma, h_ops);
+        } else {
+            float4 dv;
+            float ds, dt, dqa, dqb, drstd;
+            auto h_ops = std::make_tuple(
+                [&] { v = xr; s = v.x + v.y; t = v.z + v.w; pv = *reinterpret_cast<const float4*>(&ls[nxt * NS * XP_LSP + l_row]); },
+                [&] { s += t; },
+                [&] { s = row_ror_add<8>(s); },
+                [&] { s = row_ror_add<4>(s); done.x = rr.x + pv.x; done.y = rr.y + pv.y; },
+                [&] { s = row_ror_add<2>(s); done.z = rr.z + pv.z; done.w = rr.w + pv.w; },
+                [&] { s = row_ror_add<1>(s); if constexpr (STORE) { ds = done.x + done.y; dt = done.z + done.w; } },
+                [&] {
+                    v.x = __builtin_fmaf(s, -1.0f / C, v.x); v.y = __builtin_fmaf(s, -1.0f / C, v.y);
+                    if constexpr (STORE) ds += dt;
+                },
+                [&] {
+                    v.z = __builtin_fmaf(s, -1.0f / C, v.z); v.w = __builtin_fmaf(s, -1.0f / C, v.w);
+                    if constexpr (STORE) ds = row_ror_add<8>(ds);
+                },
+                [&] { qa = v.x * v.x; qb = v.z * v.z; if constexpr (STORE) ds = row_ror_add<4>(ds); },
+                [&] {
+                    qa = __builtin_fmaf(v.y, v.y, qa); qb = __builtin_fmaf(v.w, v.w, qb);
+                    if constexpr (STORE) ds = row_ror_add<2>(ds);
+                },
+                [&] { qa += qb; if constexpr (STORE) ds = row_ror_add<1>(ds); },
+                [&] {
+                    qa = row_ror_add<8>(qa);
+                    if constexpr (STORE) { dv.x = __builtin_fmaf(ds, -1.0f / C, done.x); dv.y = __builtin_fmaf(ds, -1.0f / C, done.y); }
+                },
+                [&] {
+                    qa = row_ror_add<4>(qa);
+                    if constexpr (STORE) { dv.z = __builtin_fmaf(ds, -1.0f / C, done.z); dv.w = __builtin_fmaf(ds, -1.0f / C, done.w); }
+                },
+                [&] { qa = row_ror_add<2>(qa); if constexpr (STORE) { dqa = dv.x * dv.x; dqb = dv.z * dv.z; } },
+                [&] {
+                    qa = row_ror_add<1>(qa);
+                    if constexpr (STORE) { dqa = __builtin_fmaf(dv.y, dv.y, dqa); dqb = __builtin_fmaf(dv.w, dv.w, dqb); }
+                },
+                [&] {
+                    rstd = __builtin_amdgcn_rsqf(__builtin_fmaf(qa, 1.0f / C, LN_EPS));
+                    if constexpr (STORE) {
+                        *reinterpret_cast<float4*>(ob + step_pos(it - 2) * step_bytes + voff) = done;
+                        dqa += dqb;
+                    }
+                },
+                [&] { rr = load_base(it - 1); if constexpr (STORE) dqa = row_ror_add<8>(dqa); },
+                [&] { y.x = v.x * rstd; y.y = v.y * rstd; if constexpr (STORE) dqa = row_ror_add<4>(dqa); },
+                [&] { y.z = v.z * rstd; y.w = v.w * rstd; if constexpr (STORE) dqa = row_ror_add<2>(dqa); },
+                [&] {
+                    f16x2_t a_, b_; split_pair(y.x, y.y, a_, b_); h4[0] = a_[0]; h4[1] = a_[1]; l4[0] = b_[0]; l4[1] = b_[1];
+                    if constexpr (STORE) dqa = row_ror_add<1>(dqa);
+                },
+                [&] { if constexpr (STORE) drstd = __builtin_amdgcn_rsqf(__builtin_fmaf(dqa, 1.0f / C, LN_EPS)); },
+                [&] { f16x2_t a_, b_; split_pair(y.z, y.w, a_, b_); h4[2] = a_[0]; h4[3] = a_[1]; l4[2] = b_[0]; l4[3] = b_[1]; },
+                [&] {
+                    *reinterpret_cast<xp_f16x4*>(&ahi[cur * NS * XP_AP + a_row]) = h4;
+                    *reinterpret_cast<xp_f16x4*>(&alo[cur * NS * XP_AP + a_row]) = l4;
+                    if constexpr (STORE) store_stats(it - 2, ds, drstd);
+                },
+                [&] { xr = load_x(it + 3); });
+            xp_zip<24>(h_mfma, h_ops);
+        }
         XP_STAMP(1);
         if (prio == 2) __builtin_amdgcn_s_setprio(0);
         if (prio == 3) __builtin_amdgcn_s_setprio(3);
@@ -351,8 +432,9 @@
     const int lastb = nstep & 1;
     if (nstep >= 2) {
         const float4 pv = *reinterpret_cast<const float4*>(&ls[(lastb ^ 1) * NS * XP_LSP + l_row]);
-        *reinterpret_cast<float4*>(ob + step_pos(nstep - 2) * step_bytes + voff) =
-            make_float4(rr.x + pv.x, rr.y + pv.y, rr.z + pv.z, rr.w + pv.w);
+        const float4 done = make_float4(rr.x + pv.x, rr.y + pv.y, rr.z + pv.z, rr.w + pv.w);
+        *reinterpret_cast<float4*>(ob + step_pos(nstep - 2) * step_bytes + voff) = done;
+        if constexpr (STATS) row_stats(nstep - 2, done);
     }
     rr = load_base(nstep - 1);
     {
@@ -371,20 +453,37 @@
     __syncthreads();
     {
         const float4 pv = *reinterpret_cast<const float4*>(&ls[lastb * NS * XP_LSP + l_row]);
-        *reinterpret_cast<float4*>(ob + step_pos(nstep - 1) * step_bytes + voff) =
-            make_float4(rr.x + pv.x, rr.y + pv.y, rr.z + pv.z, rr.w + pv.w);
-    }
+        const float4 done = make_float4(rr.x + pv.x, rr.y + pv.y, rr.z + pv.z, rr.w + pv.w);
+        *reinterpret_cast<float4*>(ob + step_pos(nstep - 1) * step_bytes + voff) = done;
+        if constexpr (STATS) row_stats(nstep - 1, done);
+    }
+}
+
+__global__ void __launch_bounds__(256, 2) k_intra_xp(const float* __restrict__ x, const _Float16* __restrict__ w_pk,
+                                                     const float* __restrict__ b_sum, const _Float16* __restrict__ wlin_pk,
+                                                     const float* __restrict__ blin, float* out, int nseq, int nstep,
+                                                     int sdiv, int so, int si, int ps, int dir, int accumulate, int prio) {
+    intra_xp_body<false>(x, w_pk, b_sum, wlin_pk, blin, out, nseq, nstep, sdiv, so, si, ps, dir, accumulate, prio, nullptr);
+}
+__global__ void __launch_bounds__(256, 2) k_intra_xp_stats(const float* __restrict__ x, const _Float16* __restrict__ w_pk,
+                                                           const float* __restrict__ b_sum, const _Float16* __restrict__ wlin_pk,
+                                                           const float* __restrict__ blin, float* out, int nseq, int nstep,
+                                                           int sdiv, int so, int si, int ps, int dir, int accumulate, int prio,
+                                                           float* stats) {
+    intra_xp_body<true>(x, w_pk, b_sum, wlin_pk, blin, out, nseq, nstep, sdiv, so, si, ps, dir, accumulate, prio, stats);
 }
 
 template <bool LIN>
 struct xp_tag { static constexpr bool value = LIN; };
 
-__global__ void __launch_bounds__(512, 1) k_inter_xp(const float* __restrict__ x, const _Float16* __restrict__ w_pk,
-                                                     const float* __restrict__ b_sum, const _Float16* __restrict__ wlin_pk,
-                                                     const float* __restrict__ blin, const float* __restrict__ h0,
-                                                     const float* __restrict__ c0, float* __restrict__ hN,
-                                                     float* __restrict__ cN, float* out, int nseq, int nstep, int sdiv,
-                                                     int so, int si, int ps, int dir, int accumulate, int prio, int cflags) {
+template <bool STATS>
+__device__ __forceinline__ void inter_xp_body(const float* __restrict__ x, const _Float16* __restrict__ w_pk,
+                                              const float* __restrict__ b_sum, const _Float16* __restrict__ wlin_pk,
+                                              const float* __restrict__ blin, const float* __restrict__ h0,
+                                              const float* __restrict__ c0, float* __restrict__ hN,
+                                              float* __restrict__ cN, float* out, int nseq, int nstep, int sdiv,
+                                              int so, int si, int ps, int dir, int accumulate, int prio, int cflags,
+                                              const float* __restrict__ stats) {
     constexpr int NS = 16;
     __shared__ __attribute__((aligned(16))) _Float16 ahi[2 * NS * XP_AP];
     __shared__ __attribute__((aligned(16))) _Float16 alo[2 * NS * XP_AP];
@@ -478,6 +577,16 @@
     auto load_row = [&](const char* base, int it) -> float4 {
         return *reinterpret_cast<const float4*>(base + step_pos(it) * step_bytes + voff);
     };
+    const char* sb = STATS ? reinterpret_cast<const char*>(stats) + wg_row0 * 8 : nullptr;
+    const unsigned svoff = (voff >> 8) * 8;
+    auto load_stats = [&](int it) -> float2 {
+        return *reinterpret_cast<const float2*>(sb + step_pos(it) * (step_bytes >> 5) + svoff);
+    };
+    auto norm_store_x_stats = [&](int buf, float4 v, float2 sr) {
+        v.x = __builtin_fmaf(sr.x, -1.0f / C, v.x); v.y = __builtin_fmaf(sr.x, -1.0f / C, v.y);
+        v.z = __builtin_fmaf(sr.x, -1.0f / C, v.z); v.w = __builtin_fmaf(sr.x, -1.0f / C, v.w);
+        store_split4(buf * NS * XP_AP + a_row, v.x * sr.y, v.y * sr.y, v.z * sr.y, v.w * sr.y);
+    };
     auto x_half = [&](int buf, f32x4 (&g)[2]) {
 #pragma unroll
         for (int m = 0; m < 2; ++m) g[m] = f32x4{0.f, 0.f, 0.f, 0.f};
@@ -496,9 +605,17 @@
 
     float creg[2], hreg[2];
     float4 carryq[2] = {make_float4(0.f, 0.f, 0.f, 0.f), make_float4(0.f, 0.f, 0.f, 0.f)};
+    float2 statq[2] = {make_float2(0.f, 0.f), make_float2(0.f, 0.f)};
     if (!lin_wave) {
-        norm_store_x(0, load_row(xb, 0));
-        norm_store_x(1, load_row(xb, 1));
+        if constexpr (STATS) {
+            norm_store_x_stats(0, load_row(xb, 0), load_stats(0));
+            norm_store_x_stats(1, load_row(xb, 1), load_stats(1));
+            statq[0] = load_stats(2);
+            if (XP_PF == 2) statq[1] = load_stats(3);
+        } else {
+            norm_store_x(0, load_row(xb, 0));
+            norm_store_x(1, load_row(xb, 1));
+        }
         carryq[0] = load_row(xb, 2);
         if (XP_PF == 2) carryq[1] = load_row(xb, 3);
     } else {
@@ -550,6 +667,30 @@
                 [&] { done.z = carry.z + pv.z; done.w = carry.w + pv.w; },
                 [&] { if (STORE) *reinterpret_cast<float4*>(ob + step_pos(it - 2) * step_bytes + voff) = done; },
                 [&] { carry = load_row(bsrc, it + XP_PF - 2); });
+            xp_zip<12>(h_mfma, h_ops);
+        } else if constexpr (STATS) {
+            float2& sc = statq[XP_PF == 2 ? cur : 0];
+            float4 v, y;
+            xp_f16x4 h4, l4;
+            auto h_ops = std::make_tuple(
+                [&] { v = carry; v.x = __builtin_fmaf(sc.x, -1.0f / C, v.x); v.y = __builtin_fmaf(sc.x, -1.0f / C, v.y); },
+                [&] { v.z = __builtin_fmaf(sc.x, -1.0f / C, v.z); v.w = __builtin_fmaf(sc.x, -1.0f / C, v.w); },
+                [&] { y.x = v.x * sc.y; y.y = v.y * sc.y; },
+                [&] { y.z = v.z * sc.y; y.w = v.w * sc.y; },
+                [&] { carry = load_row(xb, it + 2 + XP_PF); sc = load_stats(it + 2 + XP_PF); },
+                [&] { f16x2_t a_, b_; split_pair(y.x, y.y, a_, b_); h4[0] = a_[0]; h4[1] = a_[1]; l4[0] = b_[0]; l4[1] = b_[1]; },
+                [&] { },
+                [&] { f16x2_t a_, b_; split_pair(y.z, y.w, a_, b_); h4[2] = a_[0]; h4[3] = a_[1]; l4[2] = b_[0]; l4[3] = b_[1]; },
+                [&] {
+                    *reinterpret_cast<xp_f16x4*>(&ahi[cur * NS * XP_AP + a_row]) = h4;
+                    *reinterpret_cast<xp_f16x4*>(&alo[cur * NS * XP_AP + a_row]) = l4;
+                },
+                [&] {
+                    xh[0] = *reinterpret_cast<const xp_f16x8*>(&ahi[nxt * NS * XP_AP + a_frag]);
+                    xl[0] = *reinterpret_cast<const xp_f16x8*>(&alo[nxt * NS * XP_AP + a_frag]);
+                    xh[1] = *reinterpret_cast<const xp_f16x8*>(&ahi[nxt * NS * XP_AP + a_frag + 32]);
+                    xl[1] = *reinterpret_cast<const xp_f16x8*>(&alo[nxt * NS * XP_AP + a_frag + 32]);
+                });
             xp_zip<12>(h_mfma, h_ops);
         } else {
             float4 v, y;
@@ -723,14 +864,44 @@
     }
 }
 
+__global__ void __launch_bounds__(512, 1) k_inter_xp(const float* __restrict__ x, const _Float16* __restrict__ w_pk,
+                                                     const float* __restrict__ b_sum, const _Float16* __restrict__ wlin_pk,
+                                                     const float* __restrict__ blin, const float* __restrict__ h0,
+                                                     const float* __restrict__ c0, float* __restrict__ hN,
+                                                     float* __restrict__ cN, float* out, int nseq, int nstep, int sdiv,
+                                                     int so, int si, int ps, int dir, int accumulate, int prio, int cflags) {
+    inter_xp_body<false>(x, w_pk, b_sum, wlin_pk, blin, h0, c0, hN, cN, out, nseq, nstep, sdiv, so, si, ps, dir, accumulate, prio,
+                         cflags, nullptr);
+}
+__global__ void __launch_bounds__(512, 1) k_inter_xp_stats(const float* __restrict__ x, const _Float16* __restrict__ w_pk,
+                                                           const float* __restrict__ b_sum, const _Float16* __restrict__ wlin_pk,
+                                                           const float* __restrict__ blin, const float* __restrict__ h0,
+                                                           const float* __restrict__ c0, float* __restrict__ hN,
+                                                           float* __restrict__ cN, float* out, int nseq, int nstep, int sdiv,
+                                                           int so, int si, int ps, int dir, int accumulate, int prio, int cflags,
+                                                           const float* __restrict__ stats) {
+    inter_xp_body<true>(x, w_pk, b_sum, wlin_pk, blin, h0, c0, hN, cN, out, nseq, nstep, sdiv, so, si, ps, dir, accumulate, prio,
+                        cflags, stats);
+}
+
 static int g_xp_lds_pad = 0;
 static int g_xp_prio = 1;
+#if !defined(LH_XP_STATS_DEFAULT)
+#define LH_XP_STATS_DEFAULT 1
+#endif
+static int g_xp_stats = LH_XP_STATS_DEFAULT;
 static int g_xp_prio_inter = 3;
 
 int launch_inter_xp(const float* x, const void* w_pk, const float* b_sum, const void* wlin_pk, const float* blin,
                     const float* h0, const float* c0, float* hN, float* cN, float* out, int nseq, int nstep, int sdiv, int so,
-                    int si, int ps, hipStream_t st, int cflags) {
+                    int si, int ps, hipStream_t st, int cflags, const float* stats) {
     if (nstep < 2) return LH_ERR_ARG;
+    if (stats && g_xp_stats) {
+        hipLaunchKernelGGL(k_inter_xp_stats, dim3((nseq + 15) / 16), dim3(512), 0, st, x, (const _Float16*)w_pk, b_sum,
+                           (const _Float16*)wlin_pk, blin, h0, c0, hN, cN, out, nseq, nstep, sdiv, so, si, ps, 0, 0,
+                           g_xp_prio_inter, cflags, stats);
+        return check_launch();
+    }
     hipLaunchKernelGGL(k_inter_xp, dim3((nseq + 15) / 16), dim3(512), 0, st, x, (const _Float16*)w_pk, b_sum,
                        (const _Float16*)wlin_pk, blin, h0, c0, hN, cN, out, nseq, nstep, sdiv, so, si, ps, 0, 0, g_xp_prio_inter,
                        cflags);
@@ -740,11 +911,17 @@
     if (key == 7) g_xp_lds_pad = v < 0 ? 0 : v;
     if (key == 8) g_xp_prio = v;
     if (key == 9) g_xp_prio_inter = v;
+    if (key == 10) g_xp_stats = v != 0;
     return LH_OK;
 }
 
 int launch_intra_xp(const float* x, const void* w_pk, const float* b_sum, const void* wlin_pk, const float* blin, float* out,
-                    int nseq, int nstep, int sdiv, int so, int si, int ps, int dir, int accumulate, hipStream_t st) {
+                    int nseq, int nstep, int sdiv, int so, int si, int ps, int dir, int accumulate, hipStream_t st, float* stats) {
+    if (stats && g_xp_stats && accumulate) {
+        hipLaunchKernelGGL(k_intra_xp_stats, dim3((nseq + 15) / 16), dim3(256), g_xp_lds_pad, st, x, (const _Float16*)w_pk, b_sum,
+                           (const _Float16*)wlin_pk, blin, out, nseq, nstep, sdiv, so, si, ps, dir, accumulate, g_xp_prio, stats);
+        return check_launch();
+    }
 #if defined(LH_PROBE_INTRA1)
     if (dir == 1) return LH_OK;
     hipLaunchKernelGGL(k_intra_xp, dim3(2 * ((nseq + 15) / 16)), dim3(256), g_xp_lds_pad, st, x, (const _Float16*)w_pk, b_sum,
diff --git a/lookoncetohear_amd/net.py b/lookoncetohear_amd/net.py
--- a/lookoncetohear_amd/net.py
+++ b/lookoncetohear_amd/net.py
@@ -309,7 +309,8 @@
             ws = dict(xa=e(B, T, F_, C_), xb=e(B, T, F_, C_), xc=e(B, T, F_, C_), hbuf=e(B * T * F_, 2 * self.hidden),
                       q=z16(B * nh, T, 2 * QK_PAD), kx=z16(B * nh, T + hist + KV_PAD_ROWS, 2 * QK_PAD),
                       vx=z16(B * nh, T + hist + KV_PAD_ROWS, 2 * self.V_dim * F_), gain=e(B, F_, C_),
-                      gain_raw=e(B, F_ * C_), hist_dirty=False)
+                      gain_raw=e(B, F_ * C_), hist_dirty=False,
+                      stats=e(B * T * F_, 2))
             self._ws[key] = ws
         return ws
 
@@ -399,6 +400,7 @@
                 @staticmethod
                 def call(fn, *args):
                     name = fn[:-4] if fn.endswith("_win") else fn
+                    name = name[:-6] if name.endswith("_stats") else name
                     if prof is None or (only is not None and name not in only):
                         return lib_.call(fn, *args)
                     if stride > 1:
@@ -434,7 +436,13 @@
                 h0, c0 = c32(bs["h0"]), c32(bs["c0"])
                 hN, cN = new(h0), new(c0)
                 fuse = mode == 1 and self.fuse_linear
-                if fuse and Bn * T >= self.fuse_intra_min_frames:
+                fuse_intra = fuse and Bn * T >= self.fuse_intra_min_frames
+                matvec_inter = fuse and Bn * F_ <= self.inter_matvec_max_seqs and T >= 32
+                hand_stats = fuse_intra and not matvec_inter
+                if hand_stats:
+                    lib.call("lh_intra_block_stats", P(xa), P(bp["intra_w16"]), P(bp["intra_b16"]), P(bp["intra_lin_w2"]),
+                             P(bp["intra_lin_b"]), P(xb), P(ws["stats"]), Bn * T, st)
+                elif fuse_intra:
                     lib.call("lh_intra_block", P(xa), P(bp["intra_w16"]), P(bp["intra_b16"]), P(bp["intra_lin_w2"]),
                              P(bp["intra_lin_b"]), P(xb), Bn * T, st)
                 elif mode == 1 and Bn * T <= self.stream_intra_max_frames:
@@ -447,9 +455,12 @@
                              P(bp["intra" + bkey]), P(hbuf), Bn * T, mode, st)
                     lib.call("lh_linear_res", P(hbuf), P(bp["intra_lin_w"]), P(bp["intra_lin_b"]), P(xa), P(xb), rows,
                              2 * H_, st)
-                if fuse and Bn * F_ <= self.inter_matvec_max_seqs and T >= 32:
+                if matvec_inter:
                     lib.call("lh_inter_matvec", P(xb), P(bp["inter_s_wih"]), P(bp["inter_s_b"]), P(bp["inter_s_whh"]),
                              P(bp["inter_lin_w"]), P(bp["inter_lin_b"]), P(h0), P(c0), P(hN), P(cN), P(xc), Bn, T, st)
+                elif hand_stats:
+                    lib.call("lh_inter_block_stats", P(xb), P(ws["stats"]), P(bp["inter_w8"]), P(bp["inter_b16"]),
+                             P(bp["inter_lin_wu"]), P(bp["inter_lin_b"]), P(h0), P(c0), P(hN), P(cN), P(xc), Bn, T, st)
                 elif fuse:
                     lib.call("lh_inter_block", P(xb), P(bp["inter_w8"]), P(bp["inter_b16"]), P(bp["inter_lin_wu"]),
                              P(bp["inter_lin_b"]), P(h0), P(c0), P(hN), P(cN), P(xc), Bn, T, st)
@@ -550,6 +561,7 @@
         lanes = self._lanes(dev, K)
         unfused_intra = Bn * T < self.fuse_intra_min_frames
         matvec_inter = Bn * F_ <= self.inter_matvec_max_seqs
+        hand_stats = not unfused_intra and not matvec_inter
         if "kxb" not in ws:
             z16 = lambda *s_: torch.zeros(*s_, device=dev, dtype=torch.float16)
             ws["kxb"] = [ws["kx"]] + [z16(*ws["kx"].shape) for _ in range(self.n_blocks - 1)]
@@ -590,6 +602,9 @@
                                  P(bp["intra_b16"]), P(ws["hbuf"]), Bn, T, t0, Tc, st)
                         lib.call("lh_linear_res_win", P(ws["hbuf"]), P(bp["intra_lin_w"]), P(bp["intra_lin_b"]), P(xa), P(xb),
                                  Bn, T, t0, Tc, 2 * self.hidden, st)
+                    elif hand_stats:
+                        lib.call("lh_intra_block_stats_win", P(xa), P(bp["intra_w16"]), P(bp["intra_b16"]),
+                                 P(bp["intra_lin_w2"]), P(bp["intra_lin_b"]), P(xb), P(ws["stats"]), Bn, T, t0, Tc, st)
                     else:
                         lib.call("lh_intra_block_win", P(xa), P(bp["intra_w16"]), P(bp["intra_b16"]), P(bp["intra_lin_w2"]),
                                  P(bp["intra_lin_b"]), P(xb), Bn, T, t0, Tc, st)
@@ -598,6 +613,10 @@
                     if matvec_inter:
                         lib.call("lh_inter_matvec_win", P(xb), P(bp["inter_s_wih"]), P(bp["inter_s_b"]), P(bp["inter_s_whh"]),
                                  P(bp["inter_lin_w"]), P(bp["inter_lin_b"]), P(hs[i][k]), P(cs[i][k]), P(hs[i][k + 1]),
+                                 P(cs[i][k + 1]), P(xc), Bn, T, t0, Tc, carry, st)
+                    elif hand_stats:
+                        lib.call("lh_inter_block_stats_win", P(xb), P(ws["stats"]), P(bp["inter_w8"]), P(bp["inter_b16"]),
+                                 P(bp["inter_lin_wu"]), P(bp["inter_lin_b"]), P(hs[i][k]), P(cs[i][k]), P(hs[i][k + 1]),
                                  P(cs[i][k + 1]), P(xc), Bn, T, t0, Tc, carry, st)
                     else:
                         lib.call("lh_inter_block_win", P(xb), P(bp["inter_w8"]), P(bp["inter_b16"]), P(bp["inter_lin_wu"]),
```
